# PaullyMac/routest

Hardware: AMD Instinct MI355X
Metric: ETA preds/sec (whole node) + p50 /predict latency, 3-layer MLP bf16 (higher is better)
Workload: dtype bf16

## Files before the change

csrc/cch.hip:

```cpp
#include <chrono>
#include <cstdio>
#include <cstdlib>
#include <cstring>
#include <string>

#include "cch_dev.h"
#include "cch_gpu.h"

namespace rt {

using namespace cchd;

CchMetricDev::~CchMetricDev() {
  int cur = 0;
  (void)hipGetDevice(&cur);
  (void)hipSetDevice(device);
  dfree(cost);
  dfree(sub_up);
  dfree(sub_dn);
  dfree(len_up);
  dfree(len_dn);
  dfree(cnt_up);
  dfree(cnt_dn);
  dfree(f_ptr);
  dfree(b_ptr);
  dfree(f_rec);
  dfree(b_rec);
  (void)hipSetDevice(cur);
}

CchGpu::CchGpu(rcch::Topology T, const float* length, const uint8_t* road_class, const uint8_t* base_traffic,
               int device)
    : T_(std::move(T)), dev_(device) {
  int cur = 0;
  (void)hipGetDevice(&cur);
  if (hipSetDevice(dev_) != hipSuccess) throw std::runtime_error("CchGpu: bad device");
  const int N = T_.N;
  const int64_t M = T_.M, E = T_.E;
  if (M >= (int64_t)1 << 31 || E >= (int64_t)1 << 31) throw std::runtime_error("CchGpu: graph too large");
  std::vector<int32_t> up_ptr32(N + 1);
  for (int r = 0; r <= N; ++r) up_ptr32[r] = (int32_t)T_.up_ptr[r];
  bofs_.assign(N + 1, 0);
  pofs_.assign(N + 1, 0);
  aofs_.assign(N + 1, 0);
  for (int i = 0; i < N; ++i) {
    const int64_t kb = T_.up_ptr[T_.hlev_nodes[i] + 1] - T_.up_ptr[T_.hlev_nodes[i]];
    bofs_[i + 1] = bofs_[i] + kb * (kb + 1) / 2;
    const int64_t kp = T_.up_ptr[T_.dlev_nodes[i] + 1] - T_.up_ptr[T_.dlev_nodes[i]];
    pofs_[i + 1] = pofs_[i] + kp * (kp - 1);
    aofs_[i + 1] = aofs_[i] + kp;
  }
  plev_kmax_.assign((size_t)T_.max_depth + 1, 0);
  for (int d = 0; d <= T_.max_depth; ++d)
    for (int64_t i = T_.dlev_ptr[d]; i < T_.dlev_ptr[d + 1]; ++i) {
      const int x = T_.dlev_nodes[i];
      plev_kmax_[d] = std::max(plev_kmax_[d], (int)(T_.up_ptr[x + 1] - T_.up_ptr[x]));
    }
  hipError_t e = hipSuccess;
  auto ck = [&](hipError_t x) {
    if (x != hipSuccess && e == hipSuccess) e = x;
  };
  ck(up_copy(d_up_ptr, up_ptr32.data(), N + 1));
  ck(up_copy(d_up_head, T_.up_head.data(), M));
  ck(up_copy(d_arc_lo, T_.arc_lo.data(), M));
  ck(up_copy(d_parent, T_.parent.data(), N));
  ck(up_copy(d_depth, T_.depth.data(), N));
  ck(up_copy(d_rank, T_.rank.data(), N));
  ck(up_copy(d_node, T_.node.data(), N));
  ck(up_copy(d_edge_arc, T_.edge_arc.data(), E));
  ck(up_copy(d_edge_dir, T_.edge_dir.data(), E));
  ck(up_copy(d_length, length, E));
  if (road_class) ck(up_copy(d_class, road_class, E));
  if (base_traffic) ck(up_copy(d_base_traffic, base_traffic, E));
  ck(up_copy(d_hnodes, T_.hlev_nodes.data(), N));
  ck(up_copy(d_dnodes, T_.dlev_nodes.data(), N));
  {
    std::vector<int32_t> dlev32(T_.dlev_ptr.begin(), T_.dlev_ptr.end());
    ck(up_copy(d_dlev_ptr, dlev32.data(), dlev32.size()));
  }
  ck(up_copy(d_bofs, bofs_.data(), N + 1));
  ck(up_copy(d_pofs, pofs_.data(), N + 1));

  ck(alloc_scratch(cs0_));
  if (builder_max_wg_.load() < 0) builder_max_wg_.store(M >= 20000000LL ? 512 : 0);
  if (e == hipSuccess) build_tables();
  (void)hipSetDevice(cur);
  if (e != hipSuccess) throw std::runtime_error(std::string("CchGpu: ") + hipGetErrorString(e));
  if (const char* gb = std::getenv("ROUTEST_CCH_CACHE_GB")) cache_gb_ = std::atof(gb);
}

CchGpu::~CchGpu() {
  {
    std::lock_guard<std::mutex> lk(bmu_);
    bstop_ = true;
    bq_.clear();
  }
  bcv_.notify_all();
  for (auto& t : bths_)
    if (t.joinable()) t.join();
  for (auto& x : bscr_) free_scratch(*x);
  {
    std::lock_guard<std::mutex> lk(mu_);
    cache_.clear();
  }
  int cur = 0;
  (void)hipGetDevice(&cur);
  (void)hipSetDevice(dev_);
  dfree(d_up_ptr);
  dfree(d_up_head);
  dfree(d_arc_lo);
  dfree(d_parent);
  dfree(d_depth);
  dfree(d_rank);
  dfree(d_node);
  dfree(d_edge_arc);
  dfree(d_edge_dir);
  dfree(d_length);
  dfree(d_class);
  dfree(d_base_traffic);
  dfree(d_hnodes);
  dfree(d_dnodes);
  dfree(d_dlev_ptr);
  dfree(d_bofs);
  dfree(d_pofs);
  free_tables();
  free_geometry();
  free_scratch(cs0_);
  (void)hipSetDevice(cur);
}

void CchGpu::set_eta(const void* blob, int H, const NormParams& np, int variant, int num_cus) {
  std::lock_guard<std::mutex> lk(mu_cust_);
  eta_blob_ = blob;
  eta_H_ = H;
  eta_np_ = np;
  eta_variant_ = variant;
  eta_cus_ = num_cus;
}

hipError_t CchGpu::metric_from_costs(uint64_t key, const float* d_cost, hipStream_t s,
                                     std::shared_ptr<CchMetricDev>& out) {
  auto m = std::make_shared<CchMetricDev>();
  m->key = key;
  hipError_t e = customize(d_cost, *m, s);
  if (e != hipSuccess) return e;
  {
    std::lock_guard<std::mutex> lk(mu_);
    for (auto it = cache_.begin(); it != cache_.end(); ++it)
      if ((*it)->key == key) {
        cache_.erase(it);
        break;
      }
  }
  insert_cached(m);
  out = m;
  return hipSuccess;
}

static int64_t metric_device_bytes(const CchMetricDev& m, int64_t N, int64_t M, int64_t E) {
  return E * 4 + M * (8 + 8 + 4 + 4 + 4 + 4) + (N + 1) * 8 + (m.kept_f + m.kept_b) * 16;
}

void CchGpu::insert_cached(const std::shared_ptr<CchMetricDev>& m) {
  const int64_t b = metric_device_bytes(*m, T_.N, T_.M, T_.E);
  metric_bytes_.store(b);
  std::lock_guard<std::mutex> lk(mu_);
  if (cache_gb_ > 0.0 && b > 0) capacity_ = (int)std::max<int64_t>(4, (int64_t)(cache_gb_ * 1073741824.0 / (double)b));
  cache_.push_front(m);
  if (m->avoid) {
    const int cap = std::max(1, capacity_ / 4);
    int n = 0;
    for (const auto& x : cache_) n += x->avoid != nullptr;
    for (auto it = cache_.end(); n > cap && it != cache_.begin();) {
      --it;
      if ((*it)->avoid) {
        it = cache_.erase(it);
        --n;
      }
    }
  }
  while ((int)cache_.size() > capacity_) cache_.pop_back();
}

static bool same_avoid(const std::shared_ptr<const std::vector<int32_t>>& a,
                       const std::shared_ptr<const std::vector<int32_t>>& b) {
  return a == b || (a && b && *a == *b);
}

bool CchGpu::avoid_clash(const CchContext& c) {
  const uint64_t key = c.key();
  std::lock_guard<std::mutex> lk(mu_);
  for (const auto& m : cache_)
    if (m->key == key) return !same_avoid(m->avoid, c.avoid);
  return false;
}

void CchGpu::set_cache_gb(double gb) {
  std::lock_guard<std::mutex> lk(mu_);
  cache_gb_ = gb > 0.0 ? gb : 0.0;
  const int64_t b = metric_bytes_.load();
  if (cache_gb_ > 0.0 && b > 0) capacity_ = (int)std::max<int64_t>(4, (int64_t)(cache_gb_ * 1073741824.0 / (double)b));
  while ((int)cache_.size() > capacity_) cache_.pop_back();
}

void CchGpu::request_build(const CchContext& c, bool urgent) {
  const uint64_t key = c.key();
  std::shared_ptr<CchMetricDev> m;
  if (cached_metric(key, m)) {
    notify_built(key, same_avoid(m->avoid, c.avoid));
    return;
  }
  {
    std::lock_guard<std::mutex> lk(bmu_);
    if (bstop_ || !bpending_.insert(key).second) return;
    if (urgent) bq_.push_front(c);
    else bq_.push_back(c);
    start_builders_locked();
  }
  n_bqueued_.fetch_add(1, std::memory_order_relaxed);
  bcv_.notify_one();
}

void CchGpu::start_builders_locked() {
  if (!bths_.empty() || bstop_) return;
  static const int nb = [] {
    const char* v = std::getenv("ROUTEST_CCH_BUILDERS");
    const int k = v ? std::atoi(v) : 3;
    return k < 1 ? 1 : (k > 8 ? 8 : k);
  }();
  for (int i = 0; i < nb; ++i) bths_.emplace_back([this, i] { builder_loop(i); });
}

void CchGpu::start_builders() {
  std::lock_guard<std::mutex> lk(bmu_);
  start_builders_locked();
}

int CchGpu::add_build_listener(std::function<void(uint64_t, bool)> cb) {
  std::lock_guard<std::mutex> lk(lmu_);
  listeners_.emplace_back(next_listener_, std::move(cb));
  return next_listener_++;
}

void CchGpu::remove_build_listener(int id) {
  std::lock_guard<std::mutex> lk(lmu_);
  for (auto it = listeners_.begin(); it != listeners_.end(); ++it)
    if (it->first == id) {
      listeners_.erase(it);
      break;
    }
}

void CchGpu::notify_built(uint64_t key, bool ok) {
  std::lock_guard<std::mutex> lk(lmu_);
  for (auto& l : listeners_) l.second(key, ok);
}

CchGpu::AsyncStats CchGpu::async_stats() {
  AsyncStats a;
  a.queued = n_bqueued_.load();
  a.built = n_bbuilt_.load();
  a.failed = n_bfailed_.load();
  a.build_ms = us_build_.load() / 1e3;
  a.alloc_ms = us_alloc_.load() / 1e3;
  a.hostcopy_ms = us_hostcopy_.load() / 1e3;
  a.paced = n_paced_.load();
  std::lock_guard<std::mutex> lk(bmu_);
  a.pending = (int)bpending_.size();
  return a;
}

void CchGpu::builder_loop(int idx) {
  (void)idx;
  if (hipSetDevice(dev_) != hipSuccess) return;
  CustScratch* xs = nullptr;
  {
    auto x = std::make_unique<CustScratch>();
    if (alloc_scratch(*x) == hipSuccess) {
      xs = x.get();
      std::lock_guard<std::mutex> lk(bmu_);
      bscr_.push_back(std::move(x));
    } else {
      free_scratch(*x);
      (void)hipGetLastError();
    }
  }
  hipStream_t s = nullptr;
  static const int share = [] {
    const char* v = std::getenv("ROUTEST_CCH_BUILDER_CU_SHARE");
    const int k = v ? std::atoi(v) : 4;
    return k < 1 ? 1 : k;
  }();
  if (share > 1) {
    int cus = 0;
    if (hipDeviceGetAttribute(&cus, hipDeviceAttributeMultiprocessorCount, dev_) != hipSuccess || cus <= 0) cus = 256;
    std::vector<uint32_t> mask((size_t)(cus + 31) / 32, 0u);
    for (int c = share - 1; c < cus; c += share) mask[(size_t)c / 32] |= 1u << (c % 32);
    if (hipExtStreamCreateWithCUMask(&s, (uint32_t)mask.size(), mask.data()) != hipSuccess) {
      (void)hipGetLastError();
      s = nullptr;
    }
  }
  if (s == nullptr) {
    int least = 0, greatest = 0;
    if (hipDeviceGetStreamPriorityRange(&least, &greatest) != hipSuccess ||
        hipStreamCreateWithPriority(&s, hipStreamNonBlocking, least) != hipSuccess) {
      (void)hipGetLastError();
      if (hipStreamCreateWithFlags(&s, hipStreamNonBlocking) != hipSuccess) s = nullptr;
    }
  }
  while (true) {
    CchContext c;
    {
      std::unique_lock<std::mutex> lk(bmu_);
      bcv_.wait(lk, [&] { return bstop_ || !bq_.empty(); });
      if (bstop_) break;
      c = bq_.front();
      bq_.pop_front();
    }
    std::shared_ptr<CchMetricDev> m;
    bool fresh = false;
    const auto tb = std::chrono::steady_clock::now();
    const bool ok = s != nullptr && metric_for(c, s, m, &fresh, xs) == hipSuccess;
    if (ok && fresh && m) {
      us_build_.fetch_add((long long)(std::chrono::duration<double, std::micro>(std::chrono::steady_clock::now() - tb).count()));
      us_alloc_.fetch_add((long long)(m->alloc_ms * 1e3));
      us_hostcopy_.fetch_add((long long)(m->hostcopy_ms * 1e3));
    }
    if (!ok) (void)hipGetLastError();
    (ok ? n_bbuilt_ : n_bfailed_).fetch_add(1, std::memory_order_relaxed);
    {
      std::lock_guard<std::mutex> lk(bmu_);
      bpending_.erase(c.key());
    }
    notify_built(c.key(), ok);
  }
  if (s) (void)hipStreamDestroy(s);
}

bool CchGpu::cached_metric(uint64_t key, std::shared_ptr<CchMetricDev>& out) {
  std::lock_guard<std::mutex> lk(mu_);
  for (auto it = cache_.begin(); it != cache_.end(); ++it)
    if ((*it)->key == key) {
      out = *it;
      cache_.splice(cache_.begin(), cache_, it);
      return true;
    }
  return false;
}

hipError_t CchGpu::metric_for(const CchContext& c, hipStream_t s, std::shared_ptr<CchMetricDev>& out, bool* fresh,
                              CustScratch* cs) {
  const uint64_t key = c.key();
  if (fresh) *fresh = false;
  auto lookup = [&]() -> bool { return cached_metric(key, out); };
  auto checked = [&]() -> hipError_t {
    if (same_avoid(out->avoid, c.avoid)) return hipSuccess;
    out.reset();
    return hipErrorInvalidValue;
  };
  if (lookup()) return checked();
  {
    std::unique_lock<std::mutex> lk(mu_inflight_);
    cv_inflight_.wait(lk, [&] { return inflight_.count(key) == 0; });
    if (lookup()) return checked();
    inflight_.insert(key);
  }
  struct Done {
    CchGpu* g;
    uint64_t k;
    ~Done() {
      {
        std::lock_guard<std::mutex> lk(g->mu_inflight_);
        g->inflight_.erase(k);
      }
      g->cv_inflight_.notify_all();
    }
  } done{this, key};
  auto m = std::make_shared<CchMetricDev>();
  m->key = key;
  m->device = dev_;
  m->avoid = c.avoid;
  const auto ta = std::chrono::steady_clock::now();
  hipError_t e = dmalloc(m->cost, T_.E);
  m->alloc_ms = std::chrono::duration<double, std::milli>(std::chrono::steady_clock::now() - ta).count();
  if (e != hipSuccess) return e;
  auto t0 = std::chrono::steady_clock::now();
  e = context_costs(c, m->cost, s, cs);
  if (e == hipSuccess) e = hipStreamSynchronize(s);
  if (e != hipSuccess) return e;
  m->cost_ms = std::chrono::duration<double, std::milli>(std::chrono::steady_clock::now() - t0).count();
  e = customize(m->cost, *m, s, cs);
  if (e != hipSuccess) return e;
  insert_cached(m);
  out = m;
  if (fresh) *fresh = true;
  return hipSuccess;
}

}
```

csrc/cch_all.hip:

```cpp
#include <algorithm>
#include <cstdlib>

#include "cch_dev.h"
#include "cch_gpu.h"

namespace rt {

using namespace cchd;

namespace {

constexpr int ALL_FUSED_THREADS = 1024;
constexpr int ALL_FUSE_MAX = ALL_FUSED_THREADS / 64;
constexpr int ALL_ROWS = 16;
constexpr int ALL_PRE = 64 / ALL_ROWS;

__device__ __forceinline__ bool label_less(float s1, float m1, float s0, float m0) {
  return s1 < s0 || (s1 == s0 && m1 < m0);
}

__global__ __launch_bounds__(256) void cch_all_fill_kernel(float4* __restrict__ sec, float4* __restrict__ met,
                                                           long long n4) {
  const long long g = blockIdx.x * (long long)blockDim.x + threadIdx.x;
  if (g >= n4) return;
  const float4 v = make_float4(F_INF, F_INF, F_INF, F_INF);
  sec[g] = v;
  met[g] = v;
}

__global__ __launch_bounds__(64) void cch_all_up_kernel(const int* __restrict__ src, int cnt,
                                                        const int32_t* __restrict__ rank,
                                                        const int32_t* __restrict__ parent,
                                                        const int32_t* __restrict__ depth,
                                                        const int32_t* __restrict__ ptr, const int4* __restrict__ rec,
                                                        const float* __restrict__ len, int N, int stride,
                                                        float* __restrict__ wsec, float* __restrict__ wmet) {
  extern __shared__ unsigned char smem[];
  float* sd = reinterpret_cast<float*>(smem);
  float* sm = sd + stride;
  int32_t* sn = reinterpret_cast<int32_t*>(sm + stride);
  const int j = blockIdx.x;
  if (j >= cnt) return;
  const int lane = threadIdx.x;
  const int node = src[j];
  if (node < 0 || node >= N) return;
  const int r = rank[node];
  const int D = depth[r];
  if (D >= stride) return;
  for (int d = lane; d <= D; d += 64) {
    sd[d] = F_INF;
    sm[d] = F_INF;
    sn[d] = -1;
  }
  __syncthreads();
  if (lane == 0) {
    sd[D] = 0.f;
    sm[D] = 0.f;
  }
  __syncthreads();
  int x = r;
  for (int d = D; d >= 0 && x >= 0; --d) {
    const int par = parent[x];
    const int kb = ptr[x], ke = ptr[x + 1];
    if (lane == 0) sn[d] = x;
    const float dx = sd[d], mx = sm[d];
    if (dx < F_INF) {
      for (int k = kb + lane; k < ke; k += 64) {
        const int4 rc = rec[k];
        const int hd = rc.y;
        const float cs = dx + __int_as_float(rc.x);
        const float cm = mx + len[rc.z];
        if (hd >= 0 && hd < d && label_less(cs, cm, sd[hd], sm[hd])) {
          sd[hd] = cs;
          sm[hd] = cm;
        }
      }
    }
    __syncthreads();
    x = par;
  }
  const size_t base = (size_t)(j >> 6) * (size_t)N * 64 + (size_t)(j & 63);
  for (int d = lane; d <= D; d += 64) {
    const int y = sn[d];
    if (y < 0) continue;
    wsec[base + (size_t)y * 64] = sd[d];
    wmet[base + (size_t)y * 64] = sm[d];
  }
}

__device__ __forceinline__ void pull_rows(int n, int l0, int w_l, int u_l, int m_l, size_t base, const float* wsec,
                                          const float* wmet, float& bs, float& bm) {
  float ls[ALL_ROWS], lm[ALL_ROWS];
#pragma unroll
  for (int q = 0; q < ALL_ROWS; ++q) {
    const int u = __builtin_amdgcn_readlane(u_l, l0 + (q < n ? q : n - 1));
    ls[q] = wsec[base + (size_t)u * 64];
    lm[q] = wmet[base + (size_t)u * 64];
  }
#pragma unroll
  for (int q = 0; q < ALL_ROWS; ++q) {
    const int ii = l0 + (q < n ? q : n - 1);
    const float cs = ls[q] + __int_as_float(__builtin_amdgcn_readlane(w_l, ii));
    const float cm = lm[q] + __int_as_float(__builtin_amdgcn_readlane(m_l, ii));
    if (ls[q] < F_INF && label_less(cs, cm, bs, bm)) {
      bs = cs;
      bm = cm;
    }
  }
}

__device__ __forceinline__ int chunk_record(int kb, int part, int parts, int t0, int lane) {
  return kb + ALL_ROWS * (part + parts * (t0 + lane / ALL_ROWS)) + lane % ALL_ROWS;
}

__device__ __forceinline__ void pull_chunks(int kb, int ke, int part, int parts, int t0, int w_l, int u_l, int m_l,
                                            size_t base, const float* wsec, const float* wmet, float& bs, float& bm) {
#pragma unroll
  for (int t = 0; t < ALL_PRE; ++t) {
    const int left = ke - (kb + ALL_ROWS * (part + parts * (t0 + t)));
    if (left > 0) pull_rows(left < ALL_ROWS ? left : ALL_ROWS, ALL_ROWS * t, w_l, u_l, m_l, base, wsec, wmet, bs, bm);
  }
}

__device__ __forceinline__ void pull_part(int kb, int ke, int part, int parts, int t0, size_t base, int lane,
                                          const int4* __restrict__ rec, const int32_t* __restrict__ up_head,
                                          const float* __restrict__ len, const float* wsec, const float* wmet,
                                          float& bs, float& bm) {
  for (; kb + ALL_ROWS * (part + parts * t0) < ke; t0 += ALL_PRE) {
    const int k = chunk_record(kb, part, parts, t0, lane);
    int w_l = 0, u_l = 0, m_l = 0;
    if (k < ke) {
      const int4 rc = rec[k];
      w_l = rc.x;
      u_l = up_head[rc.z];
      m_l = __float_as_int(len[rc.z]);
    }
    pull_chunks(kb, ke, part, parts, t0, w_l, u_l, m_l, base, wsec, wmet, bs, bm);
  }
}

template <int WAVES>
__global__ __launch_bounds__(64 * WAVES) void cch_all_pull_kernel(
    const int32_t* __restrict__ dnodes, int lb, int cnt, int nblk, int N, const int32_t* __restrict__ ptr,
    const int4* __restrict__ rec, const int32_t* __restrict__ up_head, const float* __restrict__ len, float* wsec,
    float* wmet) {
  __shared__ float red_s[WAVES][64], red_m[WAVES][64];
  const int wave = __builtin_amdgcn_readfirstlane(threadIdx.x >> 6), lane = threadIdx.x & 63;
  const int ni = blockIdx.x / nblk, b = blockIdx.x % nblk;
  if (ni >= cnt) return;
  const int v = dnodes[lb + ni];
  const int kb = ptr[v], ke = ptr[v + 1];
  if (ke <= kb) return;
  const size_t base = (size_t)b * (size_t)N * 64 + (size_t)lane;
  const size_t row = base + (size_t)v * 64;
  float bs = F_INF, bm = F_INF;
  if (wave == 0) {
    bs = wsec[row];
    bm = wmet[row];
  }
  pull_part(kb, ke, wave, WAVES, 0, base, lane, rec, up_head, len, wsec, wmet, bs, bm);
  if (WAVES > 1) {
    red_s[wave][lane] = bs;
    red_m[wave][lane] = bm;
    __syncthreads();
    if (wave != 0) return;
#pragma unroll
    for (int p = 1; p < WAVES; ++p)
      if (label_less(red_s[p][lane], red_m[p][lane], bs, bm)) {
        bs = red_s[p][lane];
        bm = red_m[p][lane];
      }
  }
  wsec[row] = bs;
  wmet[row] = bm;
}

__global__ __launch_bounds__(ALL_FUSED_THREADS) void cch_all_pull_fused_kernel(
    const int32_t* __restrict__ dlev_ptr, const int32_t* __restrict__ dnodes, int d0, int d1, int N,
    const int32_t* __restrict__ ptr, const int4* __restrict__ rec, const int32_t* __restrict__ up_head,
    const float* __restrict__ len, float* wsec, float* wmet) {
  constexpr int NW = ALL_FUSED_THREADS / 64;
  __shared__ float red_s[NW][64], red_m[NW][64];
  const int wave = __builtin_amdgcn_readfirstlane(threadIdx.x >> 6), lane = threadIdx.x & 63;
  const size_t base = (size_t)blockIdx.x * (size_t)N * 64 + (size_t)lane;
  int lb1 = 0, width1 = 0;
  int act2 = 0, part2 = 0, parts2 = 1, v2 = 0;
  int act3 = 0, part3 = 0, parts3 = 1, v3 = 0, kb3 = 0, ke3 = 0;
  int act4 = 0, part4 = 0, parts4 = 1, v4 = 0, kb4 = 0, ke4 = 0, n4 = 0;
  int4 rc4 = make_int4(0, 0, 0, 0);
  int act5 = 0, part5 = 0, parts5 = 1, v5 = 0, kb5 = 0, ke5 = 0;
  int w5 = 0, u5 = 0, m5 = 0;
  for (int d = d0 - 5; d < d1; ++d) {
    const int act = act5, part = part5, parts = parts5, v = v5, kb = kb5, ke = ke5;
    const int w_l = w5, u_l = u5, m_l = m5;
    act5 = act4, part5 = part4, parts5 = parts4, v5 = v4, kb5 = kb4, ke5 = ke4;
    w5 = rc4.x;
    u5 = m5 = 0;
    if (n4) {
      u5 = up_head[rc4.z];
      m5 = __float_as_int(len[rc4.z]);
    }
    act4 = act3, part4 = part3, parts4 = parts3, v4 = v3, kb4 = kb3, ke4 = ke3;
    {
      const int k = chunk_record(kb3, part3, parts3, 0, lane);
      n4 = act3 && k < ke3;
      rc4 = make_int4(0, 0, 0, 0);
      if (n4) rc4 = rec[k];
    }
    act3 = act2, part3 = part2, parts3 = parts2, v3 = v2;
    kb3 = ke3 = 0;
    if (act2) {
      kb3 = ptr[v2];
      ke3 = ptr[v2 + 1];
    }
    act2 = 0, part2 = 0, parts2 = 1, v2 = 0;
    if (width1 > 0 && width1 <= NW) {
      parts2 = NW / width1;
      part2 = wave % parts2;
      const int ni = wave / parts2;
      if (ni < width1) {
        act2 = 1;
        v2 = dnodes[lb1 + ni];
      }
    }
    lb1 = width1 = 0;
    if (d + 5 >= d0 && d + 5 < d1) {
      lb1 = dlev_ptr[d + 5];
      width1 = dlev_ptr[d + 6] - lb1;
    }
    if (d < d0) continue;
    size_t row = 0;
    float bs = F_INF, bm = F_INF;
    if (act) {
      row = base + (size_t)v * 64;
      if (part == 0) {
        bs = wsec[row];
        bm = wmet[row];
      }
      pull_chunks(kb, ke, part, parts, 0, w_l, u_l, m_l, base, wsec, wmet, bs, bm);
      pull_part(kb, ke, part, parts, ALL_PRE, base, lane, rec, up_head, len, wsec, wmet, bs, bm);
      red_s[wave][lane] = bs;
      red_m[wave][lane] = bm;
    }
    __syncthreads();
    if (act && part == 0) {
      for (int p = 1; p < parts; ++p)
        if (label_less(red_s[wave + p][lane], red_m[wave + p][lane], bs, bm)) {
          bs = red_s[wave + p][lane];
          bm = red_m[wave + p][lane];
        }
      wsec[row] = bs;
      wmet[row] = bm;
    }
    __syncthreads();
  }
}

__global__ __launch_bounds__(256) void cch_all_out_kernel(const int32_t* __restrict__ rank, int N, int cnt,
                                                          const float* __restrict__ wsec,
                                                          const float* __restrict__ wmet, float* __restrict__ osec,
                                                          float* __restrict__ omet) {
  __shared__ float tile[64][65];
  const float* __restrict__ w = blockIdx.z == 0 ? wsec : wmet;
  float* __restrict__ o = blockIdx.z == 0 ? osec : omet;
  const int b = blockIdx.y;
  const int n0 = blockIdx.x * 64;
  const int lane = threadIdx.x & 63, wave = threadIdx.x >> 6;
  const size_t base = (size_t)b * (size_t)N * 64;
  for (int i = wave; i < 64; i += 4) {
    const int n = n0 + i;
    if (n < N) tile[i][lane] = w[base + (size_t)rank[n] * 64 + lane];
  }
  __syncthreads();
  const int nl = cnt - b * 64 < 64 ? cnt - b * 64 : 64;
  if (n0 + lane < N)
    for (int l = wave; l < nl; l += 4) o[(size_t)(b * 64 + l) * (size_t)N + n0 + lane] = tile[lane][l];
}

}

CchAllScratch::~CchAllScratch() {
  int cur = 0;
  (void)hipGetDevice(&cur);
  (void)hipSetDevice(device);
  dfree(sec);
  dfree(met);
  for (void* p : old) (void)hipFree(p);
  (void)hipSetDevice(cur);
}

hipError_t CchAllScratch::ensure(size_t blocks, size_t N) {
  if (blocks <= blocks_cap) return hipSuccess;
  if (sec) old.push_back((void*)sec);
  if (met) old.push_back((void*)met);
  sec = met = nullptr;
  blocks_cap = 0;
  hipError_t e;
  if ((e = dmalloc(sec, blocks * N * 64)) != hipSuccess) return e;
  if ((e = dmalloc(met, blocks * N * 64)) != hipSuccess) return e;
  blocks_cap = blocks;
  return hipSuccess;
}

hipError_t CchGpu::one_to_all(const CchMetricDev& m, const int* d_src, int S, bool reverse, float* d_sec, float* d_met,
                              CchAllScratch& sc, hipStream_t s, int fuse) {
  if (S <= 0) return hipSuccess;
  if (d_src == nullptr || d_sec == nullptr || d_met == nullptr) return hipErrorInvalidValue;
  static const int fuse_default = [] {
    const char* v = std::getenv("ROUTEST_CCH_ALL_FUSE");
    return v ? std::max(0, std::atoi(v)) : ALL_FUSE_WIDTH;
  }();
  if (fuse < 0) fuse = fuse_default;
  fuse = std::min(fuse, ALL_FUSE_MAX);
  const int N = T_.N, ST = stride();
  const size_t up_lds = (size_t)ST * 12;
  if (up_lds > 64 * 1024) return hipErrorInvalidValue;
  const int32_t* u_ptr = reverse ? m.b_ptr : m.f_ptr;
  const int4* u_rec = reverse ? m.b_rec : m.f_rec;
  const float* u_len = reverse ? m.len_dn : m.len_up;
  const int32_t* p_ptr = reverse ? m.f_ptr : m.b_ptr;
  const int4* p_rec = reverse ? m.f_rec : m.b_rec;
  const float* p_len = reverse ? m.len_up : m.len_dn;
  const size_t block_bytes = (size_t)N * 64 * 4 * 2;
  const int total_blocks = (S + 63) / 64;
  const int chunk_blocks = (int)std::min<size_t>((size_t)total_blocks, std::max<size_t>(1, ALL_SCRATCH_BYTES / block_bytes));
  sc.device = dev_;
  hipError_t e = sc.ensure((size_t)chunk_blocks, (size_t)N);
  if (e != hipSuccess) return e;
  for (int c0 = 0; c0 < total_blocks; c0 += chunk_blocks) {
    const int nb = std::min(chunk_blocks, total_blocks - c0);
    const int s0 = c0 * 64;
    const int cnt = std::min(S - s0, nb * 64);
    const long long n4 = (long long)nb * N * 16;
    hipLaunchKernelGGL(cch_all_fill_kernel, dim3(blocks_for(n4, 256)), dim3(256), 0, s,
                       reinterpret_cast<float4*>(sc.sec), reinterpret_cast<float4*>(sc.met), n4);
    hipLaunchKernelGGL(cch_all_up_kernel, dim3(cnt), dim3(64), up_lds, s, d_src + s0, cnt, d_rank, d_parent, d_depth,
                       u_ptr, u_rec, u_len, N, ST, sc.sec, sc.met);
    if ((e = hipGetLastError()) != hipSuccess) return e;
    for (int d = 1; d <= T_.max_depth;) {
      int d1 = d;
      while (fuse > 0 && d1 <= T_.max_depth && T_.dlev_ptr[d1 + 1] - T_.dlev_ptr[d1] <= fuse) ++d1;
      if (d1 - d >= 2) {
        hipLaunchKernelGGL(cch_all_pull_fused_kernel, dim3(nb), dim3(ALL_FUSED_THREADS), 0, s, d_dlev_ptr, d_dnodes, d,
                           d1, N, p_ptr, p_rec, d_up_head, p_len, sc.sec, sc.met);
        d = d1;
      } else {
        const int lb = (int)T_.dlev_ptr[d], lc = (int)(T_.dlev_ptr[d + 1] - T_.dlev_ptr[d]);
        const int kmax = plev_kmax_[d];
        const dim3 grid((unsigned)((long long)lc * nb));
        auto launch = [&](auto kernel, int waves) {
          hipLaunchKernelGGL(kernel, grid, dim3(64 * waves), 0, s, d_dnodes, lb, lc, nb, N, p_ptr, p_rec, d_up_head, p_len,
                             sc.sec, sc.met);
        };
        if (kmax <= ALL_ROWS) launch(cch_all_pull_kernel<1>, 1);
        else if (kmax <= 2 * ALL_ROWS) launch(cch_all_pull_kernel<2>, 2);
        else if (kmax <= 4 * ALL_ROWS) launch(cch_all_pull_kernel<4>, 4);
        else launch(cch_all_pull_kernel<8>, 8);
        ++d;
      }
    }
    if ((e = hipGetLastError()) != hipSuccess) return e;
    hipLaunchKernelGGL(cch_all_out_kernel, dim3(blocks_for(N, 64), nb, 2), dim3(256), 0, s, d_rank, N, cnt, sc.sec,
                       sc.met, d_sec + (size_t)s0 * N, d_met + (size_t)s0 * N);
    if ((e = hipGetLastError()) != hipSuccess) return e;
  }
  return hipSuccess;
}

}
```

csrc/cch_bindings.cpp:

```cpp
#include <torch/extension.h>
#include <ATen/hip/impl/HIPStreamMasqueradingAsCUDA.h>
#include <c10/core/DeviceGuard.h>

#include <chrono>
#include <cmath>
#include <memory>
#include <mutex>
#include <unordered_map>

#include "cch_gpu.h"
#include "ops.h"

namespace py = pybind11;

namespace {

#define CCH_CHECK_HIP(expr)                                                            \
  do {                                                                                 \
    hipError_t _e = (expr);                                                            \
    TORCH_CHECK(_e == hipSuccess, "HIP error in ", #expr, ": ", hipGetErrorString(_e)); \
  } while (0)

hipStream_t stream_of(int dev) { return c10::hip::getCurrentHIPStreamMasqueradingAsCUDA(dev).stream(); }

template <class T>
const T* host_ptr(const torch::Tensor& t, int64_t n, const char* name) {
  TORCH_CHECK(!t.is_cuda() && t.is_contiguous() && t.numel() == n, name, ": contiguous CPU tensor of ", n);
  return t.data_ptr<T>();
}

class PyCchGpu {
 public:
  PyCchGpu(torch::Tensor indptr, torch::Tensor indices, torch::Tensor lat, torch::Tensor lon, torch::Tensor length,
           torch::Tensor road_class, torch::Tensor base_traffic, int64_t device) {
    TORCH_CHECK(indptr.scalar_type() == torch::kInt32 && indices.scalar_type() == torch::kInt32 &&
                    lat.scalar_type() == torch::kFloat64 && lon.scalar_type() == torch::kFloat64 &&
                    length.scalar_type() == torch::kFloat32 && road_class.scalar_type() == torch::kUInt8 &&
                    base_traffic.scalar_type() == torch::kUInt8,
                "CchGpu: indptr/indices int32, lat/lon float64, length float32, road_class/base_traffic uint8");
    const int64_t N = lat.numel();
    const int32_t* ip = host_ptr<int32_t>(indptr, N + 1, "indptr");
    const int64_t E = ip[N];
    const int32_t* ix = host_ptr<int32_t>(indices, E, "indices");
    for (int64_t e = 0; e < E; ++e) TORCH_CHECK(ix[e] >= 0 && ix[e] < N, "edge target out of range");
    for (int64_t v = 0; v < N; ++v) TORCH_CHECK(ip[v] <= ip[v + 1], "indptr not monotone");
    auto t0 = std::chrono::steady_clock::now();
    rcch::Topology T;
    {
      py::gil_scoped_release nogil;
      T = rcch::build_topology((int)N, ip, ix, host_ptr<double>(lat, N, "lat"), host_ptr<double>(lon, N, "lon"));
    }
    build_ms_ = std::chrono::duration<double, std::milli>(std::chrono::steady_clock::now() - t0).count();
    dev_ = (int)device;
    g_ = std::make_unique<rt::CchGpu>(std::move(T), host_ptr<float>(length, E, "length"),
                                      host_ptr<uint8_t>(road_class, E, "road_class"),
                                      host_ptr<uint8_t>(base_traffic, E, "base_traffic"), dev_);
    sc_ = std::make_unique<rt::CchScratch>();
    asc_ = std::make_unique<rt::CchAllScratch>();
    std::vector<int32_t> qx((size_t)N), qy((size_t)N);
    const double* la = lat.data_ptr<double>();
    const double* lo = lon.data_ptr<double>();
    for (int64_t v = 0; v < N; ++v) {
      TORCH_CHECK(std::fabs(la[v]) <= 90.0 && std::fabs(lo[v]) <= 180.0, "node coordinate out of range");
      qx[v] = (int32_t)std::nearbyint(lo[v] * 1e6);
      qy[v] = (int32_t)std::nearbyint(la[v] * 1e6);
    }
    g_->set_geometry(ip, ix, qx.data(), qy.data());
  }

  rt::CchContext context(int64_t weather, int64_t congestion, int64_t weekhour, double age,
                         const c10::optional<torch::Tensor>& avoid, int64_t digest) const {
    rt::CchContext c;
    c.weather = (int)weather;
    c.congestion = (int)congestion;
    c.weekhour = (int)weekhour;
    c.driver_age = (float)age;
    if (avoid.has_value()) {
      c.avoid = blob_of(*avoid);
      TORCH_CHECK(digest > 0 && digest < ((int64_t)1 << 31), "avoid_digest: 1 .. 2^31 - 1");
      c.avoid_digest = (uint32_t)digest;
    }
    return c;
  }
  static std::shared_ptr<const std::vector<int32_t>> blob_of(const torch::Tensor& t) {
    TORCH_CHECK(!t.is_cuda() && t.scalar_type() == torch::kInt32 && t.dim() == 1 && t.is_contiguous(),
                "avoid: int32 [n] CPU tensor");
    return std::make_shared<const std::vector<int32_t>>(t.data_ptr<int32_t>(), t.data_ptr<int32_t>() + t.numel());
  }

  torch::Tensor avoid_mask(torch::Tensor blob) {
    auto b = blob_of(blob);
    auto out = torch::empty({(int64_t)g_->topo().E}, torch::TensorOptions().dtype(torch::kUInt8).device(torch::kCUDA, dev_));
    const c10::DeviceGuard guard(out.device());
    hipError_t e;
    {
      py::gil_scoped_release nogil;
      e = g_->avoid_mask(*b, out.data_ptr<uint8_t>(), stream_of(dev_));
    }
    if (e == hipErrorInvalidValue) throw py::value_error("avoid: not a valid avoid-set blob");
    CCH_CHECK_HIP(e);
    return out;
  }

  void set_eta(torch::Tensor blob, int64_t H, std::vector<double> norm, int64_t variant) {
    TORCH_CHECK(blob.is_cuda() && blob.device().index() == dev_ && blob.scalar_type() == torch::kUInt8,
                "blob: uint8 on the router's GPU");
    TORCH_CHECK((size_t)blob.numel() == rt::eta_mlp3_blob_bytes((int)H), "blob size for H=", H);
    TORCH_CHECK(norm.size() == 8, "norm: 4 scales + 4 shifts");
    rt::NormParams np;
    for (int i = 0; i < 4; ++i) {
      np.scale[i] = (float)norm[i];
      np.shift[i] = (float)norm[4 + i];
    }
    int cus = 256;
    (void)hipDeviceGetAttribute(&cus, hipDeviceAttributeMultiprocessorCount, dev_);
    blob_ = blob;
    g_->set_eta(blob_.data_ptr(), (int)H, np, (int)variant, cus);
  }

  py::dict stats() const {
    const rcch::Topology& T = g_->topo();
    py::dict d;
    d["nodes"] = T.N;
    d["arcs"] = T.M;
    d["edges"] = T.E;
    d["max_depth"] = T.max_depth;
    d["max_height"] = T.max_height;
    d["top_separator"] = T.separator_top;
    d["build_ms"] = build_ms_;
    d["cached_metrics"] = g_->cached();
    d["triangle_table"] = g_->has_triangle_table();
    d["triangles"] = g_->triangles();
    d["basic_tasks"] = g_->basic_tasks();
    d["supernodal"] = g_->supernodal();
    d["sup_fronts"] = g_->sup_fronts();
    d["sup_nodes"] = g_->sup_nodes();
    d["sup_levels"] = g_->sup_levels();
    d["sup_blocks"] = g_->sup_blocks();
    d["sparse_heights"] = g_->sparse_heights();
    d["sparse_depths"] = g_->sparse_depths();
    d["cache_capacity"] = g_->capacity();
    d["cache_gb"] = g_->cache_gb();
    d["metric_bytes"] = g_->metric_bytes();
    const auto a = g_->async_stats();
    d["async_queued"] = a.queued;
    d["async_built"] = a.built;
    d["async_failed"] = a.failed;
    d["async_pending"] = a.pending;
    d["async_build_ms"] = a.build_ms;
    d["async_alloc_ms"] = a.alloc_ms;
    d["async_hostcopy_ms"] = a.hostcopy_ms;
    d["builder_max_wg"] = g_->builder_pacing();
    d["async_paced"] = a.paced;
    return d;
  }

  void request_build(int64_t weather, int64_t congestion, int64_t weekhour, double age, bool urgent,
                     c10::optional<torch::Tensor> avoid, int64_t avoid_digest) {
    TORCH_CHECK(g_->has_eta(), "CchGpu: set_eta first");
    const rt::CchContext c = context(weather, congestion, weekhour, age, avoid, avoid_digest);
    g_->request_build(c, urgent);
  }
  bool is_cached(int64_t key) {
    std::shared_ptr<rt::CchMetricDev> m;
    return g_->cached_metric((uint64_t)key, m);
  }
  void set_cache_gb(double gb) { g_->set_cache_gb(gb); }
  void set_builder_pacing(int n, bool always) { g_->set_builder_pacing(n, always); }
  void set_unpack_serial(bool on) { g_->set_unpack_serial(on); }
  bool unpack_serial() const { return g_->unpack_serial(); }

  py::dict info(const rt::CchMetricDev& m, bool fresh) const {
    py::dict d;
    d["key"] = m.key;
    d["fresh"] = fresh;
    d["cost_ms"] = m.cost_ms;
    d["customize_ms"] = m.customize_ms;
    d["basic_ms"] = m.basic_ms;
    d["perfect_ms"] = m.perfect_ms;
    d["prune_ms"] = m.prune_ms;
    d["kept_f"] = m.kept_f;
    d["kept_b"] = m.kept_b;
    return d;
  }

  py::dict metric_for(int64_t weather, int64_t congestion, int64_t weekhour, double age, bool pin,
                      c10::optional<torch::Tensor> avoid, int64_t avoid_digest) {
    TORCH_CHECK(g_->has_eta(), "CchGpu: set_eta first");
    const rt::CchContext c = context(weather, congestion, weekhour, age, avoid, avoid_digest);
    const c10::DeviceGuard guard(c10::Device(c10::DeviceType::CUDA, dev_));
    std::shared_ptr<rt::CchMetricDev> m;
    bool fresh = false;
    hipError_t e;
    {
      py::gil_scoped_release nogil;
      e = g_->metric_for(c, stream_of(dev_), m, &fresh);
    }
    if (e == hipErrorInvalidValue && g_->avoid_clash(c))
      throw py::value_error("avoid set: its digest is cached for a different set (a 2^-31 collision); "
                            "change a vertex by a microdegree or retry once that metric is evicted");
    if (e == hipErrorInvalidValue && c.avoid) throw py::value_error("avoid: not a valid avoid-set blob");
    CCH_CHECK_HIP(e);
    if (pin) pin_ptr(m);
    return info(*m, fresh);
  }

  void unpin(int64_t key) {
    std::lock_guard<std::mutex> lk(pin_mu_);
    auto it = pins_.find((uint64_t)key);
    if (it != pins_.end() && --it->second.second <= 0) pins_.erase(it);
  }
  int64_t pinned() {
    std::lock_guard<std::mutex> lk(pin_mu_);
    return (int64_t)pins_.size();
  }

  py::dict metric_from_costs(int64_t key, torch::Tensor cost) {
    TORCH_CHECK(cost.is_cuda() && cost.device().index() == dev_ && cost.scalar_type() == torch::kFloat32 &&
                    cost.is_contiguous() && cost.numel() == g_->topo().E,
                "cost: float32 [E] on the router's GPU");
    TORCH_CHECK((cost >= 0).all().item<bool>(), "edge costs must be >= 0 (+inf: edge absent), not NaN");
    cost = cost.add(0.0);
    const c10::DeviceGuard guard(cost.device());
    std::shared_ptr<rt::CchMetricDev> m;
    hipError_t e;
    {
      py::gil_scoped_release nogil;
      e = g_->metric_from_costs((uint64_t)key, cost.data_ptr<float>(), stream_of(dev_), m);
    }
    CCH_CHECK_HIP(e);
    return info(*m, true);
  }

  py::dict metric_dump(int64_t key) {
    auto m = get(key);
    const int64_t M = g_->topo().M, N = g_->topo().N;
    const auto opt = torch::TensorOptions().device(torch::kCUDA, dev_);
    const c10::DeviceGuard guard(opt.device());
    py::dict d;
    auto put = [&](const char* name, const void* src, int64_t n, torch::ScalarType t) {
      auto out = torch::empty({n}, opt.dtype(t));
      if (n > 0)
        CCH_CHECK_HIP(hipMemcpyAsync(out.data_ptr(), src, n * out.element_size(), hipMemcpyDeviceToDevice, stream_of(dev_)));
      d[name] = out;
    };
    put("sub_up", m->sub_up, 2 * M, torch::kInt32);
    put("sub_dn", m->sub_dn, 2 * M, torch::kInt32);
    put("len_up", m->len_up, M, torch::kFloat32);
    put("len_dn", m->len_dn, M, torch::kFloat32);
    put("cnt_up", m->cnt_up, M, torch::kInt32);
    put("cnt_dn", m->cnt_dn, M, torch::kInt32);
    put("f_ptr", m->f_ptr, N + 1, torch::kInt32);
    put("b_ptr", m->b_ptr, N + 1, torch::kInt32);
    put("f_rec", m->f_rec, 4 * m->kept_f, torch::kInt32);
    put("b_rec", m->b_rec, 4 * m->kept_b, torch::kInt32);
    return d;
  }

  torch::Tensor costs(int64_t key) {
    auto m = get(key);
    auto out = torch::empty({(int64_t)g_->topo().E},
                            torch::TensorOptions().dtype(torch::kFloat32).device(torch::kCUDA, dev_));
    const c10::DeviceGuard guard(out.device());
    CCH_CHECK_HIP(hipMemcpyAsync(out.data_ptr<float>(), m->cost, g_->topo().E * 4, hipMemcpyDeviceToDevice,
                                 stream_of(dev_)));
    return out;
  }

  py::tuple route(int64_t key, torch::Tensor src, torch::Tensor dst, int64_t max_path, bool want_path) {
    auto m = get(key);
    TORCH_CHECK(src.is_cuda() && dst.is_cuda() && src.device().index() == dev_ && dst.device().index() == dev_ &&
                    src.scalar_type() == torch::kInt32 && dst.scalar_type() == torch::kInt32 &&
                    src.is_contiguous() && dst.is_contiguous() && src.numel() == dst.numel(),
                "src/dst: int32 [Q] on the router's GPU");
    const int64_t Q = src.numel();
    const int N = g_->topo().N;
    if (Q > 0) {
      const auto mn = torch::minimum(src.min(), dst.min()).item<int>();
      const auto mx = torch::maximum(src.max(), dst.max()).item<int>();
      TORCH_CHECK(mn >= 0 && mx < N, "node id out of range");
    }
    auto o32 = torch::TensorOptions().dtype(torch::kInt32).device(torch::kCUDA, dev_);
    auto of = torch::TensorOptions().dtype(torch::kFloat32).device(torch::kCUDA, dev_);
    auto sec = torch::empty({Q}, of), met = torch::empty({Q}, of);
    auto st = torch::empty({Q}, o32), len = torch::zeros({Q}, o32);
    auto path = want_path ? torch::empty({Q, max_path}, o32) : torch::empty({0, max_path}, o32);
    rt::CchRouteOut o;
    o.sec = sec.data_ptr<float>();
    o.metres = met.data_ptr<float>();
    o.status = st.data_ptr<int>();
    o.len = len.data_ptr<int>();
    o.path = want_path ? path.data_ptr<int>() : nullptr;
    o.max_path = (int)max_path;
    const c10::DeviceGuard guard(src.device());
    std::lock_guard<std::mutex> lk(mu_);
    CCH_CHECK_HIP(g_->route(*m, src.data_ptr<int>(), dst.data_ptr<int>(), (int)Q, o, *sc_, stream_of(dev_)));
    return py::make_tuple(sec, met, st, len, path);
  }

  py::tuple matrix(int64_t key, torch::Tensor pts, torch::Tensor npts) {
    auto m = get(key);
    TORCH_CHECK(pts.is_cuda() && npts.is_cuda() && pts.dim() == 2 && pts.scalar_type() == torch::kInt32 &&
                    npts.scalar_type() == torch::kInt32 && npts.numel() == pts.size(0) && pts.is_contiguous(),
                "pts int32 [R, NM], npts int32 [R] on the router's GPU");
    const int R = (int)pts.size(0), NM = (int)pts.size(1);
    auto of = torch::TensorOptions().dtype(torch::kFloat32).device(torch::kCUDA, dev_);
    auto sec = torch::empty({R, NM, NM}, of), met = torch::empty({R, NM, NM}, of);
    const c10::DeviceGuard guard(pts.device());
    std::lock_guard<std::mutex> lk(mu_);
    CCH_CHECK_HIP(g_->matrix(*m, pts.data_ptr<int>(), npts.data_ptr<int>(), R, NM, sec.data_ptr<float>(),
                             met.data_ptr<float>(), nullptr, *sc_, stream_of(dev_)));
    return py::make_tuple(sec, met);
  }

  py::tuple matrix_rect(int64_t key, torch::Tensor src, torch::Tensor nsrc, torch::Tensor dst, torch::Tensor ndst,
                        int64_t meet) {
    auto m = get(key);
    for (const torch::Tensor* t : {&src, &nsrc, &dst, &ndst})
      TORCH_CHECK(t->is_cuda() && t->device().index() == dev_ && t->scalar_type() == torch::kInt32 && t->is_contiguous(),
                  "src / nsrc / dst / ndst: int32 on the router's GPU");
    TORCH_CHECK(src.dim() == 2 && dst.dim() == 2 && dst.size(0) == src.size(0) && nsrc.numel() == src.size(0) &&
                    ndst.numel() == src.size(0),
                "src [R, SM], dst [R, DM], nsrc [R], ndst [R]");
    const int64_t R = src.size(0), SM = src.size(1), DM = dst.size(1);
    TORCH_CHECK(R * (SM + DM) <= INT32_MAX && R * SM * DM <= INT32_MAX, "matrix_rect: too many chains or cells for one call");
    auto of = torch::TensorOptions().dtype(torch::kFloat32).device(torch::kCUDA, dev_);
    auto sec = torch::empty({R, SM, DM}, of), met = torch::empty({R, SM, DM}, of);
    const c10::DeviceGuard guard(src.device());
    std::lock_guard<std::mutex> lk(mu_);
    CCH_CHECK_HIP(g_->matrix_rect(*m, src.data_ptr<int>(), nsrc.data_ptr<int>(), dst.data_ptr<int>(),
                                  ndst.data_ptr<int>(), (int)R, (int)SM, (int)DM, sec.data_ptr<float>(),
                                  met.data_ptr<float>(), *sc_, stream_of(dev_), (int)meet));
    return py::make_tuple(sec, met);
  }

  py::tuple matrix_keep(int64_t key, torch::Tensor pts, torch::Tensor npts) {
    auto sm = matrix(key, pts, npts);
    std::lock_guard<std::mutex> lk(mu_);
    return py::make_tuple(sm[0], sm[1], (uint64_t)sc_->chain_tag);
  }

  py::tuple legs_from_matrix(int64_t key, uint64_t tag, torch::Tensor pts, torch::Tensor r, torch::Tensor i,
                             torch::Tensor j, int64_t max_path, bool want_path) {
    auto m = get(key);
    for (const torch::Tensor* t : {&pts, &r, &i, &j})
      TORCH_CHECK(t->is_cuda() && t->device().index() == dev_ && t->scalar_type() == torch::kInt32 && t->is_contiguous(),
                  "pts / r / i / j: int32 on the router's GPU");
    TORCH_CHECK(pts.dim() == 2 && r.numel() == i.numel() && r.numel() == j.numel(), "pts [R, NM]; r, i, j [Q]");
    const int64_t Q = r.numel();
    const int R = (int)pts.size(0), NM = (int)pts.size(1);
    if (Q > 0) {
      TORCH_CHECK(r.min().item<int>() >= 0 && r.max().item<int>() < R, "leg request index out of range");
      TORCH_CHECK(torch::minimum(i.min(), j.min()).item<int>() >= 0 && torch::maximum(i.max(), j.max()).item<int>() < NM,
                  "leg point index out of range");
    }
    auto o32 = torch::TensorOptions().dtype(torch::kInt32).device(torch::kCUDA, dev_);
    auto of = torch::TensorOptions().dtype(torch::kFloat32).device(torch::kCUDA, dev_);
    auto sec = torch::empty({Q}, of), met = torch::empty({Q}, of);
    auto st = torch::empty({Q}, o32), len = torch::zeros({Q}, o32);
    auto path = want_path ? torch::empty({Q, max_path}, o32) : torch::empty({0, max_path}, o32);
    rt::CchRouteOut o;
    o.sec = sec.data_ptr<float>();
    o.metres = met.data_ptr<float>();
    o.status = st.data_ptr<int>();
    o.len = len.data_ptr<int>();
    o.path = want_path ? path.data_ptr<int>() : nullptr;
    o.max_path = (int)max_path;
    const c10::DeviceGuard guard(pts.device());
    auto src = Q > 0 ? pts.index({r.to(torch::kLong), i.to(torch::kLong)}).contiguous() : torch::empty({0}, o32);
    std::lock_guard<std::mutex> lk(mu_);
    TORCH_CHECK(tag != 0 && tag == sc_->chain_tag && sc_->chain_nm == NM && sc_->chain_r == R,
                "legs_from_matrix: the matrix chains of this tag are gone (another call ran since)");
    CCH_CHECK_HIP(g_->legs_from_matrix(*m, src.data_ptr<int>(), r.data_ptr<int>(), i.data_ptr<int>(), j.data_ptr<int>(),
                                       (int)Q, tag, o, *sc_, stream_of(dev_)));
    return py::make_tuple(sec, met, st, len, path);
  }

  py::tuple one_to_all(int64_t key, torch::Tensor src, bool reverse, int64_t fuse) {
    auto m = get(key);
    TORCH_CHECK(src.is_cuda() && src.device().index() == dev_ && src.scalar_type() == torch::kInt32 &&
                    src.is_contiguous() && src.dim() == 1,
                "src: int32 [S] on the router's GPU");
    const int64_t S = src.numel();
    const int64_t N = g_->topo().N;
    TORCH_CHECK(S < ((int64_t)1 << 31) - 64, "too many sources");
    if (S > 0) TORCH_CHECK(src.min().item<int>() >= 0 && src.max().item<int>() < N, "node id out of range");
    auto of = torch::TensorOptions().dtype(torch::kFloat32).device(torch::kCUDA, dev_);
    auto sec = torch::empty({S, N}, of), met = torch::empty({S, N}, of);
    const c10::DeviceGuard guard(src.device());
    std::lock_guard<std::mutex> lk(mu_);
    CCH_CHECK_HIP(g_->one_to_all(*m, src.data_ptr<int>(), (int)S, reverse, sec.data_ptr<float>(), met.data_ptr<float>(),
                                 *asc_, stream_of(dev_), (int)fuse));
    return py::make_tuple(sec, met);
  }

  void set_capacity(int64_t n) { g_->set_capacity((int)n); }
  uintptr_t ptr() const { return reinterpret_cast<uintptr_t>(g_.get()); }
  py::dict topology_arrays() const {
    const rcch::Topology& T = g_->topo();
    py::dict d;
    auto i32 = [](const std::vector<int32_t>& v) {
      auto t = torch::empty({(int64_t)v.size()}, torch::kInt32);
      if (!v.empty()) std::memcpy(t.data_ptr<int32_t>(), v.data(), v.size() * 4);
      return t;
    };
    d["rank"] = i32(T.rank);
    d["node"] = i32(T.node);
    d["parent"] = i32(T.parent);
    d["depth"] = i32(T.depth);
    d["up_head"] = i32(T.up_head);
    return d;
  }

 private:
  void pin_ptr(const std::shared_ptr<rt::CchMetricDev>& m) {
    std::lock_guard<std::mutex> lk(pin_mu_);
    auto& p = pins_[m->key];
    p.first = m;
    ++p.second;
  }

  std::shared_ptr<rt::CchMetricDev> get(int64_t key) {
    std::shared_ptr<rt::CchMetricDev> m;
    if (g_->cached_metric((uint64_t)key, m)) return m;
    {
      std::lock_guard<std::mutex> lk(pin_mu_);
      auto it = pins_.find((uint64_t)key);
      if (it != pins_.end()) return it->second.first;
    }
    TORCH_CHECK(false, "CchGpu: no cached metric for key ", key, " (evicted or never built)");
    return m;
  }

  std::mutex pin_mu_;
  std::unordered_map<uint64_t, std::pair<std::shared_ptr<rt::CchMetricDev>, int>> pins_;

  std::unique_ptr<rt::CchGpu> g_;
  std::unique_ptr<rt::CchScratch> sc_;
  std::unique_ptr<rt::CchAllScratch> asc_;
  std::mutex mu_;
  torch::Tensor blob_;
  int dev_ = 0;
  double build_ms_ = 0.0;
};

}

void bind_cch_gpu(py::module& m) {
  py::class_<PyCchGpu>(m, "CchGpu")
      .def(py::init<torch::Tensor, torch::Tensor, torch::Tensor, torch::Tensor, torch::Tensor, torch::Tensor,
                    torch::Tensor, int64_t>(),
           py::arg("indptr"), py::arg("indices"), py::arg("lat"), py::arg("lon"), py::arg("length"),
           py::arg("road_class"), py::arg("base_traffic"), py::arg("device"))
      .def("set_eta", &PyCchGpu::set_eta, py::arg("blob"), py::arg("H"), py::arg("norm"), py::arg("variant") = -1)
      .def("stats", &PyCchGpu::stats)
      .def("metric_for", &PyCchGpu::metric_for, py::arg("weather"), py::arg("congestion"), py::arg("weekhour"),
           py::arg("driver_age") = 35.0, py::arg("pin") = false, py::arg("avoid") = py::none(),
           py::arg("avoid_digest") = 0)
      .def("avoid_mask", &PyCchGpu::avoid_mask, py::arg("blob"))
      .def("unpin", &PyCchGpu::unpin, py::arg("key"))
      .def("pinned", &PyCchGpu::pinned)
      .def("metric_from_costs", &PyCchGpu::metric_from_costs, py::arg("key"), py::arg("cost"))
      .def("costs", &PyCchGpu::costs, py::arg("key"))
      .def("metric_dump", &PyCchGpu::metric_dump, py::arg("key"))
      .def("route", &PyCchGpu::route, py::arg("key"), py::arg("src"), py::arg("dst"), py::arg("max_path") = 4096,
           py::arg("want_path") = true)
      .def("matrix", &PyCchGpu::matrix, py::arg("key"), py::arg("pts"), py::arg("npts"))
      .def("matrix_rect", &PyCchGpu::matrix_rect, py::arg("key"), py::arg("src"), py::arg("nsrc"), py::arg("dst"),
           py::arg("ndst"), py::arg("meet") = 0)
      .def("matrix_keep", &PyCchGpu::matrix_keep, py::arg("key"), py::arg("pts"), py::arg("npts"))
      .def("legs_from_matrix", &PyCchGpu::legs_from_matrix, py::arg("key"), py::arg("tag"), py::arg("pts"), py::arg("r"),
           py::arg("i"), py::arg("j"), py::arg("max_path") = 4096, py::arg("want_path") = true)
      .def("one_to_all", &PyCchGpu::one_to_all, py::arg("key"), py::arg("src"), py::arg("reverse") = false,
           py::arg("fuse") = -1)
      .def("set_capacity", &PyCchGpu::set_capacity)
      .def("set_cache_gb", &PyCchGpu::set_cache_gb, py::arg("gb"))
      .def("set_builder_pacing", &PyCchGpu::set_builder_pacing, py::arg("max_workgroups"), py::arg("always") = false)
      .def("set_unpack_serial", &PyCchGpu::set_unpack_serial, py::arg("on"))
      .def("unpack_serial", &PyCchGpu::unpack_serial)
      .def("request_build", &PyCchGpu::request_build, py::arg("weather"), py::arg("congestion"), py::arg("weekhour"),
           py::arg("driver_age") = 35.0, py::arg("urgent") = true, py::arg("avoid") = py::none(),
           py::arg("avoid_digest") = 0)
      .def("is_cached", &PyCchGpu::is_cached, py::arg("key"))
      .def("ptr", &PyCchGpu::ptr)
      .def("topology_arrays", &PyCchGpu::topology_arrays);
}
```

csrc/cch_customize.hip:

```cpp
#include <hipcub/hipcub.hpp>

#include <chrono>
#include <cstdio>
#include <cstdlib>
#include <cstring>
#include <string>

#include "cch_dev.h"
#include "cch_gpu.h"
#include "ops.h"
#include "runtime/rt_core.h"

namespace rt {

using namespace cchd;

namespace {

using EtaRecordDev = rtc::EtaRecord;

__device__ __forceinline__ int item_owner(const int64_t* __restrict__ ofs, int lo, int hi, long long g) {
  while (hi - lo > 1) {
    const int mid = (lo + hi) >> 1;
    if (ofs[mid] <= g) lo = mid;
// ... 73 lines not shown
      sub[1] = e;
      len[a] = length[e];
      cnt[a] = 1;
      continue;
    }
    const int zz = (int)pl;
    const int azu = find_arc_d(up_ptr, up_head, zz, z), azv = find_arc_d(up_ptr, up_head, zz, v);
    const int s0 = dir ? azv : azu, s1 = dir ? azu : azv;
    sub[0] = s0;
    sub[1] = s1;
    len[a] = len_dn[s0] + len_up[s1];
    cnt[a] = cnt_dn[s0] + cnt_up[s1];
  }
}

__device__ __forceinline__ void basic_relax_pair(int z, int ai, int aj, int t, unsigned long long* __restrict__ up,
                                                 unsigned long long* __restrict__ dn) {
  const float wu = wof(dn[ai]) + wof(up[aj]);
  const float wd = wof(dn[aj]) + wof(up[ai]);
  if (wu < F_INF) {
    const unsigned long long pu = packw(wu, (uint32_t)z);
    if (pu < up[t]) atomicMin(up + t, pu);
  }
  if (wd < F_INF) {
    const unsigned long long pd = packw(wd, (uint32_t)z);
    if (pd < dn[t]) atomicMin(dn + t, pd);
  }
}

__global__ __launch_bounds__(256) void basic_level_kernel(LevelArgs L, unsigned long long* __restrict__ up,
                                                          unsigned long long* __restrict__ dn,
                                                          int32_t* __restrict__ sub_up, int32_t* __restrict__ sub_dn,
                                                          float* __restrict__ len_up, float* __restrict__ len_dn,
                                                          int32_t* __restrict__ cnt_up, int32_t* __restrict__ cnt_dn,
                                                          const float* __restrict__ length) {
  const long long gi = blockIdx.x * (long long)blockDim.x + threadIdx.x;
  if (gi >= L.items) return;
  const long long g = L.base + gi;
  const int ni = item_owner(L.ofs, L.lo, L.hi, g);
  const int z = L.nodes[ni];
  const long long p = g - L.ofs[ni];
  const int a0 = L.up_ptr[z];
  const int k = L.up_ptr[z + 1] - a0;
  if (p < k) {
    const int a = a0 + (int)p;
    basic_finalize_arc(a, z, L.up_head[a], L.up_ptr, L.up_head, up, dn, sub_up, sub_dn, len_up, len_dn, cnt_up, cnt_dn,
                       length);
    return;
  }
  const long long q = p - k;
  const double kk = (double)(2 * k - 1);
  int i = (int)((kk - sqrt(kk * kk - 8.0 * (double)q)) * 0.5);
  if (i < 0) i = 0;
  auto row0 = [&](int r) { return (long long)r * (2 * k - r - 1) / 2; };
  while (i > 0 && row0(i) > q) --i;
  while (i + 1 < k && row0(i + 1) <= q) ++i;
  const int j = (int)(q - row0(i)) + i + 1;
  const int ai = a0 + i, aj = a0 + j;
  const int t = find_arc_d(L.up_ptr, L.up_head, L.up_head[ai], L.up_head[aj]);
  if (t < 0) return;
  basic_relax_pair(z, ai, aj, t, up, dn);
}

struct BasicTask {
  int64_t rowbase;
  int32_t node;
  int32_t a0;
  uint16_t k;
  uint16_t row;
  uint16_t col0;
  uint16_t pad;
};
static_assert(sizeof(BasicTask) == 24, "basic task layout");
constexpr uint16_t ROW_FINAL = 0xFFFF;

__global__ __launch_bounds__(256) void basic_task_kernel(const BasicTask* __restrict__ tasks, long long ntask,
                                                         const int32_t* __restrict__ up_ptr,
                                                         const int32_t* __restrict__ up_head,
                                                         const int32_t* __restrict__ tri,
                                                         unsigned long long* __restrict__ up,
                                                         unsigned long long* __restrict__ dn, int32_t* __restrict__ sub_up,
                                                         int32_t* __restrict__ sub_dn, float* __restrict__ len_up,
                                                         float* __restrict__ len_dn, int32_t* __restrict__ cnt_up,
                                                         int32_t* __restrict__ cnt_dn, const float* __restrict__ length) {
  const long long ti = (long long)blockIdx.x * 4 + (threadIdx.x >> 6);
  if (ti >= ntask) return;
  const BasicTask& T = tasks[ti];
  const int lane = threadIdx.x & 63;
  const int z = T.node;
  const int a0 = T.a0;
  const int k = T.k;
  if (T.row == ROW_FINAL) {
    const int p = T.col0 + lane;
    if (p >= k) return;
    const int a = a0 + p;
    basic_finalize_arc(a, z, up_head[a], up_ptr, up_head, up, dn, sub_up, sub_dn, len_up, len_dn, cnt_up, cnt_dn,
                       length);
    return;
  }
  const int i = T.row;
  const int j = T.col0 + lane;
  if (j >= k) return;
  const int t = tri[T.rowbase + j];
  if (t < 0) return;
  basic_relax_pair(z, a0 + i, a0 + j, t, up, dn);
}

__global__ void perfect_init_kernel(const unsigned long long* __restrict__ up, const unsigned long long* __restrict__ dn,
                                    uint32_t* __restrict__ pup, uint32_t* __restrict__ pdn, long long M) {
  for (long long a = blockIdx.x * (long long)blockDim.x + threadIdx.x; a < M; a += (long long)gridDim.x * blockDim.x) {
    pup[a] = (uint32_t)(up[a] >> 32);
    pdn[a] = (uint32_t)(dn[a] >> 32);
  }
}

__global__ __launch_bounds__(256) void perfect_level_kernel(LevelArgs L, const unsigned long long* __restrict__ up,
                                                            const unsigned long long* __restrict__ dn,
                                                            uint32_t* __restrict__ pup, uint32_t* __restrict__ pdn) {
  const long long gi = blockIdx.x * (long long)blockDim.x + threadIdx.x;
  if (gi >= L.items) return;
  const long long g = L.base + gi;
  const int ni = item_owner(L.ofs, L.lo, L.hi, g);
  const int x = L.nodes[ni];
  const long long p = g - L.ofs[ni];
  const int a0 = L.up_ptr[x];
  const int k = L.up_ptr[x + 1] - a0;
  const int c = (int)(p / (k - 1));
  const int r = (int)(p % (k - 1));
  const int a = r < c ? r : r + 1;
  const int ac = a0 + c, aa = a0 + a;
  const int y = L.up_head[aa], z = L.up_head[ac];
  const int azy = find_arc_d(L.up_ptr, L.up_head, z < y ? z : y, z < y ? y : z);
  if (azy < 0) return;
  const float xz = wof(up[ac]), zx = wof(dn[ac]);
  const float zy = __uint_as_float(z < y ? pup[azy] : pdn[azy]);
  const float yz = __uint_as_float(z < y ? pdn[azy] : pup[azy]);
  const float cu = xz + zy, cd = yz + zx;
  if (cu < F_INF && __float_as_uint(cu) < pup[aa]) atomicMin(pup + aa, __float_as_uint(cu));
  if (cd < F_INF && __float_as_uint(cd) < pdn[aa]) atomicMin(pdn + aa, __float_as_uint(cd));
}

struct PArc {
  int64_t tb;
  int32_t a0;
  int32_t y;
  uint16_t k;
  uint16_t ia;
  int32_t pad;
};
static_assert(sizeof(PArc) == 24, "pull arc record");

struct PullArgs {
  const int32_t* up_head;
  const int32_t* tri;
  const PArc* parc;
  long long base, arcs;
};

__device__ __forceinline__ void pull_cand(const PullArgs& P, long long tb, int k, int a0, int ia, int ic, float xz_c,
                                          float zx_c, const uint32_t* __restrict__ pup, const uint32_t* __restrict__ pdn,
                                          int y, int z, float& bu, float& bd) {
  const int i = ic < ia ? ic : ia, j = ic < ia ? ia : ic;
  const int azy = P.tri[tb + (long long)i * (2 * k - i - 1) / 2 + (j - i - 1)];
  const float zy = __uint_as_float(z < y ? pup[azy] : pdn[azy]);
  const float yz = __uint_as_float(z < y ? pdn[azy] : pup[azy]);
  const float cu = xz_c + zy, cd = yz + zx_c;
  bu = cu < bu ? cu : bu;
  bd = cd < bd ? cd : bd;
}

__device__ __forceinline__ void pull_arc_min(const PullArgs& P, long long tb, int a0, int k, int ia, int y, int c_begin,
                                             int c_step, int lane, const unsigned long long* __restrict__ up,
                                             const unsigned long long* __restrict__ dn, const uint32_t* __restrict__ pup,
                                             const uint32_t* __restrict__ pdn, float& bu, float& bd) {
  for (int c0 = c_begin; c0 < k; c0 += c_step) {
    int azy[4], z[4];
    unsigned long long wu[4], wd[4];
    bool ok[4];
#pragma unroll
    for (int u = 0; u < 4; ++u) {
      const int ic = c0 + 64 * u + lane;
      ok[u] = ic < k && ic != ia;
      const int i = ic < ia ? ic : ia, j = ic < ia ? ia : ic;
      azy[u] = ok[u] ? P.tri[tb + (long long)i * (2 * k - i - 1) / 2 + (j - i - 1)] : 0;
      z[u] = ok[u] ? P.up_head[a0 + ic] : 0;
      wu[u] = ok[u] ? up[a0 + ic] : 0ull;
      wd[u] = ok[u] ? dn[a0 + ic] : 0ull;
    }
    uint32_t gu[4], gd[4];
#pragma unroll
    for (int u = 0; u < 4; ++u) {
      gu[u] = ok[u] ? pup[azy[u]] : 0u;
      gd[u] = ok[u] ? pdn[azy[u]] : 0u;
    }
#pragma unroll
    for (int u = 0; u < 4; ++u) {
      if (!ok[u]) continue;
      const float zy = __uint_as_float(z[u] < y ? gu[u] : gd[u]);
      const float yz = __uint_as_float(z[u] < y ? gd[u] : gu[u]);
      const float cu = wof(wu[u]) + zy, cd = yz + wof(wd[u]);
      bu = cu < bu ? cu : bu;
      bd = cd < bd ? cd : bd;
    }
  }
#pragma unroll
  for (int o = 32; o >= 1; o >>= 1) {
    const float ou = __shfl_xor(bu, o), od = __shfl_xor(bd, o);
    bu = ou < bu ? ou : bu;
    bd = od < bd ? od : bd;
  }
}

template <int S>
__global__ __launch_bounds__(256) void perfect_pull_wave_kernel(PullArgs P, const unsigned long long* __restrict__ up,
                                                                const unsigned long long* __restrict__ dn,
                                                                uint32_t* __restrict__ pup, uint32_t* __restrict__ pdn) {
  static_assert(S == 1 || S == 2 || S == 4, "waves per arc");
  constexpr int APB = 4 / S;
  __shared__ float red[2][4];
  const int w = threadIdx.x >> 6, lane = threadIdx.x & 63;
  const long long g = (long long)blockIdx.x * APB + w / S;
  const int part = w % S;
  const bool active = g < P.arcs;
  float bu = F_INF, bd = F_INF;
  int aa = 0;
  if (active) {
    const PArc pa = P.parc[P.base + g];
    aa = pa.a0 + pa.ia;
    pull_arc_min(P, pa.tb, pa.a0, pa.k, pa.ia, pa.y, 256 * part, 256 * S, lane, up, dn, pup, pdn, bu, bd);
  }
  if constexpr (S > 1) {
    if (lane == 0) {
      red[0][w] = bu;
      red[1][w] = bd;
    }
    __syncthreads();
    if (part != 0) return;
#pragma unroll
    for (int q = 1; q < S; ++q) {
      const float ou = red[0][w + q], od = red[1][w + q];
      bu = ou < bu ? ou : bu;
      bd = od < bd ? od : bd;
    }
  }
  if (active && lane == 0) {
    const float cu = __uint_as_float(pup[aa]), cd = __uint_as_float(pdn[aa]);
    if (bu < cu) pup[aa] = __float_as_uint(bu);
    if (bd < cd) pdn[aa] = __float_as_uint(bd);
  }
}

__global__ __launch_bounds__(256) void perfect_pull_lane_kernel(PullArgs P, const unsigned long long* __restrict__ up,
                                                                const unsigned long long* __restrict__ dn,
                                                                uint32_t* __restrict__ pup, uint32_t* __restrict__ pdn) {
  const long long g = (long long)blockIdx.x * blockDim.x + threadIdx.x;
  if (g >= P.arcs) return;
  const PArc pa = P.parc[P.base + g];
  const long long tb = pa.tb;
  const int a0 = pa.a0, k = pa.k, ia = pa.ia, y = pa.y;
  const int aa = a0 + ia;
  float bu = __uint_as_float(pup[aa]), bd = __uint_as_float(pdn[aa]);
  for (int ic = 0; ic < k; ++ic) {
    if (ic == ia) continue;
    const int ac = a0 + ic;
    pull_cand(P, tb, k, a0, ia, ic, wof(up[ac]), wof(dn[ac]), pup, pdn, y, P.up_head[ac], bu, bd);
  }
  pup[aa] = __float_as_uint(bu);
  pdn[aa] = __float_as_uint(bd);
}

__device__ __forceinline__ bool kept(uint32_t p, unsigned long long b) {
  return __uint_as_float(p) < F_INF && p == (uint32_t)(b >> 32);
}

__global__ __launch_bounds__(256) void prune_count_wave_kernel(const int32_t* __restrict__ up_ptr,
                                                               const uint32_t* __restrict__ pup,
                                                               const uint32_t* __restrict__ pdn,
                                                               const unsigned long long* __restrict__ up,
                                                               const unsigned long long* __restrict__ dn, int N,
                                                               int32_t* __restrict__ fcnt, int32_t* __restrict__ bcnt) {
  const int x = blockIdx.x * 4 + (threadIdx.x >> 6);
  const int lane = threadIdx.x & 63;
  if (x >= N) return;
  int kf = 0, kb = 0;
  for (int a = up_ptr[x] + lane; a < up_ptr[x + 1]; a += 64) {
    kf += kept(pup[a], up[a]);
    kb += kept(pdn[a], dn[a]);
  }
#pragma unroll
  for (int o = 32; o >= 1; o >>= 1) {
    kf += __shfl_xor(kf, o);
    kb += __shfl_xor(kb, o);
  }
  if (lane == 0) {
    fcnt[x] = kf;
    bcnt[x] = kb;
  }
}

__global__ __launch_bounds__(256) void prune_scatter_wave_kernel(
    const int32_t* __restrict__ up_ptr, const int32_t* __restrict__ up_head, const int32_t* __restrict__ depth,
    const uint32_t* __restrict__ pup, const uint32_t* __restrict__ pdn, const unsigned long long* __restrict__ up,
    const unsigned long long* __restrict__ dn, int N, const int32_t* __restrict__ f_ptr, const int32_t* __restrict__ b_ptr,
    int4* __restrict__ f_rec, int4* __restrict__ b_rec) {
  const int x = blockIdx.x * 4 + (threadIdx.x >> 6);
  const int lane = threadIdx.x & 63;
  if (x >= N) return;
  int kf = f_ptr[x], kb = b_ptr[x];
  const unsigned long long below = (1ull << lane) - 1ull;
  for (int a0 = up_ptr[x]; a0 < up_ptr[x + 1]; a0 += 64) {
    const int a = a0 + lane;
    const bool in = a < up_ptr[x + 1];
    const bool f = in && kept(pup[a], up[a]);
    const bool b = in && kept(pdn[a], dn[a]);
    const unsigned long long mf = __ballot(f), mb = __ballot(b);
    if (f || b) {
      const int hd = depth[up_head[a]];
      if (f) f_rec[kf + __popcll(mf & below)] = make_int4((int)pup[a], hd, a, 0);
      if (b) b_rec[kb + __popcll(mb & below)] = make_int4((int)pdn[a], hd, a, 0);
    }
    kf += __popcll(mf);
    kb += __popcll(mb);
  }
}

struct SupNode {
  int64_t dofs;
  int64_t foff;
  int32_t c0, m, n;
  int32_t fnode;
};
struct SupWork {
  int32_t s, b, t0, t1;
  SupNode sn;
};
constexpr int SUP_B = 32;
constexpr int SUP_PJ = 32;
constexpr int SUP_TT = 64;
constexpr int SUP_G1Y = 32;
constexpr int SUP_G1Z = 128;
constexpr int SUP_SJ = 64;

__device__ __forceinline__ unsigned long long sup_cand(unsigned long long a, unsigned long long b, uint32_t z) {
  const float w = wof(a) + wof(b);
  return w < F_INF ? packw(w, z) : PACK_INF_D;
}
__device__ __forceinline__ unsigned long long umin64(unsigned long long a, unsigned long long b) { return b < a ? b : a; }

__global__ __launch_bounds__(256) void sup_farc_kernel(const SupNode* __restrict__ sn, const SupWork* __restrict__ w,
                                                       long long nw, const int32_t* __restrict__ fnode,
                                                       const int32_t* __restrict__ up_ptr,
                                                       const int32_t* __restrict__ up_head, int32_t* __restrict__ farc) {
  const long long wi = (long long)blockIdx.x * 4 + (threadIdx.x >> 6);
  if (wi >= nw) return;
  const SupWork W = w[wi];
  const SupNode S = W.sn;
  const int i = W.b, n = S.n;
  const int fi = fnode[S.fnode + i];
  for (int j = threadIdx.x & 63; j < n; j += 64) {
    const int fj = fnode[S.fnode + j];
    farc[S.foff + (long long)i * n + j] = i == j ? -1 : find_arc_d(up_ptr, up_head, fi < fj ? fi : fj, fi < fj ? fj : fi);
  }
}

__global__ __launch_bounds__(256) void sup_gather_basic_kernel(
    const SupNode* __restrict__ sn, const SupWork* __restrict__ w, const int32_t* __restrict__ fnode,
    const int32_t* __restrict__ farc, const unsigned long long* __restrict__ up, const unsigned long long* __restrict__ dn,
    const int32_t* __restrict__ up_ptr, const int32_t* __restrict__ up_head, const float* __restrict__ len_up,
    const float* __restrict__ len_dn, const int32_t* __restrict__ cnt_up, const int32_t* __restrict__ cnt_dn,
    unsigned long long* __restrict__ D, int2* __restrict__ SS, int2* __restrict__ SL) {
  const SupWork W = w[blockIdx.x];
  const SupNode S = W.sn;
  const int i = W.b, n = S.n;
  const long long r0 = S.dofs + (long long)i * n;
  const int32_t* fr = farc + S.foff + (long long)i * n;
  const int fi = fnode[S.fnode + i];
  for (int j = threadIdx.x; j < n; j += 256) {
    unsigned long long v = PACK_INF_D;
    if (i != j && (i < S.m || j < S.m)) {
      const int a = fr[j];
      if (a >= 0) {
        v = i < j ? up[a] : dn[a];
        const uint32_t pl = (uint32_t)v;
        if (wof(v) < F_INF && !(pl & EDGE_FLAG_D)) {
          const int zz = (int)pl, fj = fnode[S.fnode + j];
          const int lo = i < j ? fi : fj, hi = i < j ? fj : fi;
          const int azx = find_arc_d(up_ptr, up_head, zz, lo), azv = find_arc_d(up_ptr, up_head, zz, hi);
          const int s0 = i < j ? azx : azv, s1 = i < j ? azv : azx;
          SS[r0 + j] = make_int2(s0, s1);
          SL[r0 + j] = make_int2(__float_as_int(len_dn[s0] + len_up[s1]), cnt_dn[s0] + cnt_up[s1]);
        }
      }
    }
    D[r0 + j] = v;
  }
}

__device__ __forceinline__ void sup_panel_body(
    const SupWork& W, const int32_t* __restrict__ farc, unsigned long long* __restrict__ D, const int2* __restrict__ SS,
    const int2* __restrict__ SL, unsigned long long* __restrict__ up, unsigned long long* __restrict__ dn,
    int32_t* __restrict__ sub_up, int32_t* __restrict__ sub_dn, float* __restrict__ len_up, float* __restrict__ len_dn,
    int32_t* __restrict__ cnt_up, int32_t* __restrict__ cnt_dn, const float* __restrict__ length) {
  constexpr int B = SUP_B, J = SUP_PJ, W2 = SUP_B + SUP_PJ;
  static_assert(B == 32 && J == 32, "one entry of each matrix per thread");
  __shared__ unsigned long long Dk[B][B + 1];
  __shared__ unsigned long long R[B][J + 1];
  __shared__ unsigned long long C[J][B + 1];
  __shared__ int32_t FK[B][W2];
  __shared__ float lu[B][W2], ld[B][W2];
  __shared__ int32_t cu[B][W2], cd[B][W2];
  const SupNode S = W.sn;
  const int n = S.n, tid = threadIdx.x;
  const int k0 = W.b * B, k1 = min(k0 + B, S.m), kb = k1 - k0;
  const int j0 = k1 + W.t0 * J, nj = max(0, min(J, n - j0));
  const bool diag_writer = W.t0 == 0;
  unsigned long long* Df = D + S.dofs;
  const int32_t* F = farc + S.foff;
  const int ty = tid >> 5, tx = tid & 31;
  Dk[ty][tx] = (ty < kb && tx < kb) ? Df[(long long)(k0 + ty) * n + k0 + tx] : PACK_INF_D;
  R[ty][tx] = (ty < kb && tx < nj) ? Df[(long long)(k0 + ty) * n + j0 + tx] : PACK_INF_D;
  C[ty][tx] = (tx < kb && ty < nj) ? Df[(long long)(j0 + ty) * n + k0 + tx] : PACK_INF_D;
  FK[ty][tx] = (ty < kb && tx < kb && tx > ty) ? F[(long long)(k0 + ty) * n + k0 + tx] : -1;
  FK[ty][B + tx] = (ty < kb && tx < nj) ? F[(long long)(k0 + ty) * n + j0 + tx] : -1;
  __syncthreads();
  if (W.b > 0) {
    const int km = k0 - B;
    __shared__ unsigned long long Ay[B][B + 1];
    __shared__ unsigned long long Aj[J][B + 1];
    __shared__ unsigned long long Bx[B][B + 1];
    __shared__ unsigned long long Bj[B][J + 1];
    Ay[ty][tx] = ty < kb ? Df[(long long)(k0 + ty) * n + km + tx] : PACK_INF_D;
    Aj[ty][tx] = ty < nj ? Df[(long long)(j0 + ty) * n + km + tx] : PACK_INF_D;
    Bx[ty][tx] = tx < kb ? Df[(long long)(km + ty) * n + k0 + tx] : PACK_INF_D;
    Bj[ty][tx] = tx < nj ? Df[(long long)(km + ty) * n + j0 + tx] : PACK_INF_D;
    __syncthreads();
    unsigned long long dk = Dk[ty][tx], rr = R[ty][tx], cc = C[ty][tx];
    const bool odk = ty < kb && tx < kb && ty != tx, orr = ty < kb && tx < nj, occ = ty < nj && tx < kb;
    for (int p = 0; p < B; ++p) {
      const uint32_t z = (uint32_t)(S.c0 + km + p);
      if (odk) dk = umin64(dk, sup_cand(Ay[ty][p], Bx[p][tx], z));
      if (orr) rr = umin64(rr, sup_cand(Ay[ty][p], Bj[p][tx], z));
      if (occ) cc = umin64(cc, sup_cand(Aj[ty][p], Bx[p][tx], z));
    }
    Dk[ty][tx] = dk;
    R[ty][tx] = rr;
    C[ty][tx] = cc;
    __syncthreads();
  }
  for (int p = 0; p < kb; ++p) {
    const uint32_t z = (uint32_t)(S.c0 + k0 + p);
    if (ty > p && tx > p && ty < kb && tx < kb && ty != tx) Dk[ty][tx] = umin64(Dk[ty][tx], sup_cand(Dk[ty][p], Dk[p][tx], z));
    if (ty > p && ty < kb && tx < nj) R[ty][tx] = umin64(R[ty][tx], sup_cand(Dk[ty][p], R[p][tx], z));
    if (tx > p && tx < kb && ty < nj) C[ty][tx] = umin64(C[ty][tx], sup_cand(C[ty][p], Dk[p][tx], z));
    __syncthreads();
  }
  if (ty < kb && tx < nj) {
    Df[(long long)(k0 + ty) * n + j0 + tx] = R[ty][tx];
    Df[(long long)(j0 + tx) * n + k0 + ty] = C[tx][ty];
    const int a = FK[ty][B + tx];
    if (a >= 0) {
      up[a] = R[ty][tx];
      dn[a] = C[tx][ty];
    }
  }
  if (diag_writer && ty < kb && tx < kb) {
    Df[(long long)(k0 + ty) * n + k0 + tx] = Dk[ty][tx];
    const int a = FK[ty][tx];
    if (a >= 0) {
      up[a] = Dk[ty][tx];
      dn[a] = Dk[tx][ty];
    }
  }
  const int zK = S.c0 + k0;
  auto vfront = [&](int col) { return col < B ? k0 + col : j0 + col - B; };
  auto weight = [&](int x, int col, int dir) -> unsigned long long {
    if (col < B) return dir ? Dk[col][x] : Dk[x][col];
    return dir ? C[col - B][x] : R[x][col - B];
  };
  auto put = [&](int x, int col, int a, int dir, int s0, int s1, float L, int32_t Cn) {
    (dir ? ld : lu)[x][col] = L;
    (dir ? cd : cu)[x][col] = Cn;
    if (col >= B || diag_writer) {
      int32_t* sub = (dir ? sub_dn : sub_up) + 2 * (long long)a;
      sub[0] = s0;
      sub[1] = s1;
      (dir ? len_dn : len_up)[a] = L;
      (dir ? cnt_dn : cnt_up)[a] = Cn;
    }
  };
  {
    constexpr int Q = B * W2 / 1024;
    int kind[Q][2], s0[Q][2], s1[Q][2];
    float L[Q][2];
    int32_t Cn[Q][2];
#pragma unroll
    for (int q = 0; q < Q; ++q) {
      const int e = tid + 1024 * q, x = e / W2, col = e % W2;
      const int a = FK[x][col];
#pragma unroll
      for (int dir = 0; dir < 2; ++dir) {
        kind[q][dir] = 0;
        if (a < 0) continue;
        const unsigned long long wt = weight(x, col, dir);
        const uint32_t pl = (uint32_t)wt;
        const int vf = vfront(col);
        if (!(wof(wt) < F_INF)) {
          kind[q][dir] = 1;
          s0[q][dir] = -1;
          s1[q][dir] = -1;
          L[q][dir] = F_INF;
          Cn[q][dir] = 0;
        } else if (pl & EDGE_FLAG_D) {
          const int ed = (int)(pl & ~EDGE_FLAG_D);
          kind[q][dir] = 1;
          s0[q][dir] = -1;
          s1[q][dir] = ed;
          L[q][dir] = length[ed];
          Cn[q][dir] = 1;
        } else if ((int)pl < S.c0) {
          const long long idx = dir ? (long long)vf * n + k0 + x : (long long)(k0 + x) * n + vf;
          const int2 ss = SS[S.dofs + idx], sl = SL[S.dofs + idx];
          kind[q][dir] = 1;
          s0[q][dir] = ss.x;
          s1[q][dir] = ss.y;
          L[q][dir] = __int_as_float(sl.x);
          Cn[q][dir] = sl.y;
        } else if ((int)pl < zK) {
          const long long fz = (int)pl - S.c0;
          const int azx = F[fz * n + k0 + x], azv = F[fz * n + vf];
          kind[q][dir] = 2;
          s0[q][dir] = dir ? azv : azx;
          s1[q][dir] = dir ? azx : azv;
        }
      }
    }
#pragma unroll
    for (int q = 0; q < Q; ++q)
#pragma unroll
      for (int dir = 0; dir < 2; ++dir)
        if (kind[q][dir] == 2) {
          L[q][dir] = len_dn[s0[q][dir]] + len_up[s1[q][dir]];
          Cn[q][dir] = cnt_dn[s0[q][dir]] + cnt_up[s1[q][dir]];
        }
#pragma unroll
    for (int q = 0; q < Q; ++q) {
      const int e = tid + 1024 * q, x = e / W2, col = e % W2;
#pragma unroll
      for (int dir = 0; dir < 2; ++dir)
        if (kind[q][dir]) put(x, col, FK[x][col], dir, s0[q][dir], s1[q][dir], L[q][dir], Cn[q][dir]);
    }
  }
  __syncthreads();
  for (int x = 1; x < kb; ++x) {
    if (tid < 2 * W2) {
      const int dir = tid / W2, col = tid % W2;
      const int a = FK[x][col];
      const unsigned long long wt = a >= 0 ? weight(x, col, dir) : PACK_INF_D;
      const uint32_t pl = (uint32_t)wt;
      const int zl = (int)pl - zK;
      if (wof(wt) < F_INF && !(pl & EDGE_FLAG_D) && zl >= 0) {
        const int azx = FK[zl][x], azv = FK[zl][col];
        if (dir == 0)
          put(x, col, a, 0, azx, azv, ld[zl][x] + lu[zl][col], cd[zl][x] + cu[zl][col]);
        else
          put(x, col, a, 1, azv, azx, ld[zl][col] + lu[zl][x], cd[zl][col] + cu[zl][x]);
      }
    }
    __syncthreads();
  }
}

__device__ __forceinline__ void sup_trailing_body(const SupWork& W, const int32_t* __restrict__ farc,
                                                  unsigned long long* __restrict__ D, unsigned long long* __restrict__ up,
                                                  unsigned long long* __restrict__ dn) {
  constexpr int B = SUP_B, T = SUP_TT;
  __shared__ float A[T][B + 1];
  __shared__ float Bm[B][T + 1];
  const SupNode S = W.sn;
  const int n = S.n, m = S.m, tid = threadIdx.x;
  const int nb = (m + B - 1) / B;
  const int k0 = W.b * B, k1 = min(k0 + B, m), kb = k1 - k0;
  const int zr0 = W.b + 1 < nb ? min(k1 + B, m) : k1;
  const int y0 = zr0 + W.t0 * T, z0 = zr0 + W.t1 * T;
  unsigned long long* Df = D + S.dofs;
#pragma unroll
  for (int h = 0; h < 2; ++h) {
    const int e = tid + 1024 * h;
    {
      const int r = e / B, p = e % B;
      A[r][p] = (y0 + r < n && p < kb) ? wof(Df[(long long)(y0 + r) * n + k0 + p]) : F_INF;
    }
    {
      const int p = e / T, c = e % T;
      Bm[p][c] = (p < kb && z0 + c < n) ? wof(Df[(long long)(k0 + p) * n + z0 + c]) : F_INF;
    }
  }
  const int ty = tid >> 4, tz = tid & 15;
  const int y = y0 + ty;
  unsigned long long old[4];
#pragma unroll
  for (int j = 0; j < 4; ++j) {
    const int z = z0 + tz + 16 * j;
    old[j] = (y < n && z < n && y != z) ? Df[(long long)y * n + z] : PACK_INF_D;
  }
  __syncthreads();
  float bw[4];
  int bp[4];
#pragma unroll
  for (int j = 0; j < 4; ++j) {
    bw[j] = F_INF;
    bp[j] = 0;
  }
  for (int p = 0; p < kb; ++p) {
    const float a = A[ty][p];
#pragma unroll
    for (int j = 0; j < 4; ++j) {
      const float sum = a + Bm[p][tz + 16 * j];
      if (sum < bw[j]) {
        bw[j] = sum;
        bp[j] = p;
      }
    }
  }
  const bool last = k1 == m;
  const int32_t* F = farc + S.foff;
// ... 670 lines not shown
  SupWork* dwk = nullptr;
  int32_t *dfn = nullptr, *dfa = nullptr;
  PArc* dpa = nullptr;
  bool ok = up_copy(dsn, sn.data(), sn.size()) == hipSuccess && up_copy(dwk, work.data(), work.size()) == hipSuccess &&
            up_copy(dfn, fnode.data(), fnode.size()) == hipSuccess && dmalloc(dfa, (size_t)foff) == hipSuccess &&
            up_copy(dpa, parc.data(), parc.size()) == hipSuccess && dmalloc(cs0_.sup_buf, 3 * (size_t)buf) == hipSuccess;
  if (ok) {
    hipLaunchKernelGGL(sup_farc_kernel, dim3((unsigned)cdiv(all_rows.cnt, 4)), dim3(256), 0, 0, dsn, dwk + all_rows.off,
                       (long long)all_rows.cnt, dfn, d_up_ptr, d_up_head, dfa);
    ok = hipGetLastError() == hipSuccess && hipDeviceSynchronize() == hipSuccess;
  }
  if (!ok) {
    (void)hipGetLastError();
    dfree(dsn);
    dfree(dwk);
    dfree(dfn);
    dfree(dfa);
    dfree(dpa);
    dfree(cs0_.sup_buf);
    std::fprintf(stderr, "[cch] supernodal plan: device allocation failed; per-level customization\n");
    return;
  }
  d_sup_sn = dsn;
  d_sup_work = dwk;
  d_sup_fnode = dfn;
  d_sup_farc = dfa;
  d_parc2 = dpa;
  sup_buf_entries_ = buf;
  sup_lev_ = std::move(levs);
  sup_node_ = std::move(node_in);
  rlev_aofs_ = std::move(raofs);
  rlev_nodes_ = std::move(rnodes);
  rlev_kmax_ = std::move(rkmax);
  rlev_multi_ = std::move(rmulti);
  sup_fronts_ = (int)sn.size();
  sup_nodes_ = nodes_in;
  sup_blocks_ = blocks;
  sparse_heights_ = hmax + 1;
  sup_on_ = true;
}

bool CchGpu::build_pull_records(const std::vector<int64_t>& tofs) {
  if (sup_on_) return true;
  const int N = T_.N;
  std::vector<PArc> parc((size_t)aofs_[N]);
  for (int i = 0; i < N; ++i) {
    const int x = T_.dlev_nodes[i];
    const int a0 = (int)T_.up_ptr[x], k = (int)(T_.up_ptr[x + 1] - T_.up_ptr[x]);
    if (k > 0xFFFF) return false;
    for (int ia = 0; ia < k; ++ia)
      parc[(size_t)aofs_[i] + ia] = PArc{tofs[x], a0, (int32_t)T_.up_head[a0 + ia], (uint16_t)k, (uint16_t)ia, 0};
  }
  PArc* dp = nullptr;
  const bool ok = up_copy(dp, parc.data(), parc.size()) == hipSuccess;
  d_parc = dp;
  return ok;
}

bool CchGpu::build_tasks(const std::vector<int64_t>& tofs) {
  std::vector<BasicTask> bt;
  btask_ptr_.assign(T_.max_height + 2, 0);
  for (int h = 0; h <= T_.max_height; ++h) {
    for (int64_t q = T_.hlev_ptr[h]; q < T_.hlev_ptr[h + 1]; ++q) {
      const int z = T_.hlev_nodes[q];
      if (sup_on_ && sup_node_[z]) continue;
      const int k = (int)(T_.up_ptr[z + 1] - T_.up_ptr[z]);
      if (k > 0xFFFE) return false;
      const int a0 = (int)T_.up_ptr[z];
      for (int j0 = 0; j0 < k; j0 += 64)
        bt.push_back(BasicTask{0, z, a0, (uint16_t)k, ROW_FINAL, (uint16_t)j0, 0});
      for (int i = 0; i + 1 < k; ++i) {
        const int64_t rb = tofs[z] + (int64_t)i * (2 * k - i - 1) / 2 - i - 1;
        for (int j0 = i + 1; j0 < k; j0 += 64)
          bt.push_back(BasicTask{rb, z, a0, (uint16_t)k, (uint16_t)i, (uint16_t)j0, 0});
      }
    }
    btask_ptr_[h + 1] = (int64_t)bt.size();
  }
  BasicTask* db = nullptr;
  const bool ok = up_copy(db, bt.data(), bt.size()) == hipSuccess;
  d_btask = db;
  if (ok) n_btask_ = (int64_t)bt.size();
  return ok;
}

hipError_t CchGpu::alloc_scratch(CustScratch& x) {
  const int N = T_.N;
  const int64_t M = T_.M;
  hipError_t e = hipSuccess;
  auto ck = [&](hipError_t r) {
    if (r != hipSuccess && e == hipSuccess) e = r;
  };
  ck(dmalloc(x.up64, M));
  ck(dmalloc(x.dn64, M));
  ck(dmalloc(x.pup, M));
  ck(dmalloc(x.pdn, M));
  ck(dmalloc(x.fcnt, N));
  ck(dmalloc(x.bcnt, N));
  size_t tb = 0;
  ck(hipcub::DeviceScan::InclusiveSum(nullptr, tb, x.fcnt, x.fcnt, N));
  x.cub_bytes = tb;
  ck(hipMalloc(&x.cub, x.cub_bytes ? x.cub_bytes : 1));
  ck(hipHostMalloc((void**)&x.h_stage, (size_t)std::max<int64_t>(1, T_.E) * sizeof(float), hipHostMallocDefault));
  if (sup_on_) ck(dmalloc(x.sup_buf, 3 * (size_t)sup_buf_entries_));
  return e;
}

void CchGpu::free_scratch(CustScratch& x) {
  dfree(x.up64);
  dfree(x.dn64);
  dfree(x.pup);
  dfree(x.pdn);
  dfree(x.fcnt);
  dfree(x.bcnt);
  if (x.cub) (void)hipFree(x.cub);
  x.cub = nullptr;
  if (x.rec_buf) (void)hipFree(x.rec_buf);
  x.rec_buf = nullptr;
  dfree(x.min_buf);
  if (x.h_stage) (void)hipHostFree(x.h_stage);
  x.h_stage = nullptr;
  dfree(x.sup_buf);
  dfree(x.avoid_dev);
  if (x.avoid_host) (void)hipHostFree(x.avoid_host);
  x.avoid_host = nullptr;
}

hipError_t CchGpu::context_costs(const CchContext& c, float* d_cost, hipStream_t s, CustScratch* cs) {
  if (eta_blob_ == nullptr || d_class == nullptr || d_base_traffic == nullptr) return hipErrorInvalidValue;
  const int E = (int)T_.E;
  hipError_t e = hipSuccess;
  std::unique_lock<std::mutex> lk(mu_cust_, std::defer_lock);
  if (cs == nullptr) lk.lock();
  CustScratch& X = cs ? *cs : cs0_;
  void*& rec_buf = X.rec_buf;
  float*& min_buf = X.min_buf;
  if (rec_buf == nullptr) {
    if ((e = hipMalloc(&rec_buf, (size_t)2 * E * sizeof(EtaRecordDev))) != hipSuccess) return e;
    if ((e = dmalloc(min_buf, (size_t)2 * E)) != hipSuccess) return e;
  }
  hipLaunchKernelGGL(ctx_records_kernel, dim3(blocks_for(E, 256)), dim3(256), 0, s, d_base_traffic, E, c.weather,
                     c.congestion, c.weekhour, c.driver_age, (EtaRecordDev*)rec_buf);
  if ((e = hipGetLastError()) != hipSuccess) return e;
  e = launch_eta_mlp3_fwd(rec_buf, min_buf, 2 * E, eta_blob_, eta_H_, eta_np_, eta_variant_, eta_cus_, s, 16);
  if (e != hipSuccess) return e;
  hipLaunchKernelGGL(ctx_cost_kernel, dim3(blocks_for(E, 256)), dim3(256), 0, s, min_buf, d_length, d_class, E, d_cost);
  e = hipGetLastError();
  if (e == hipSuccess && c.avoid) e = apply_avoid(*c.avoid, d_cost, nullptr, s, X);
  if (e == hipSuccess && cs == nullptr) e = hipStreamSynchronize(s);
  return e;
}

namespace {

inline long long wave_cap(int max_wg) { return max_wg > 0 ? 4LL * max_wg : (1LL << 40); }

template <class F>
hipError_t launch_pieces(long long total, long long cap, F&& launch) {
  for (long long i0 = 0; i0 < total; i0 += cap) {
    launch(i0, std::min(cap, total - i0));
    const hipError_t e = hipGetLastError();
    if (e != hipSuccess) return e;
  }
  return hipSuccess;
}

constexpr int PULL_WAVE_K = 64;

hipError_t pull_level(hipStream_t s, const CustScratch& X, PullArgs P, long long nodes, int km, int wave_km, int max_wg) {
  const bool wave = P.arcs >= 24 * nodes || km >= wave_km;
  const int S = P.arcs >= 8192 ? 1 : (km > 768 ? 4 : (km > 256 ? 2 : 1));
  const long long cap = wave ? std::max(1LL, wave_cap(max_wg) / S) : 64 * wave_cap(max_wg);
  const long long base = P.base;
  return launch_pieces(P.arcs, cap, [&](long long a0, long long n) {
    P.base = base + a0;
    P.arcs = n;
    if (wave && S == 4)
      hipLaunchKernelGGL(perfect_pull_wave_kernel<4>, dim3((unsigned)P.arcs), dim3(256), 0, s, P, X.up64, X.dn64,
                         X.pup, X.pdn);
    else if (wave && S == 2)
      hipLaunchKernelGGL(perfect_pull_wave_kernel<2>, dim3((unsigned)((P.arcs + 1) / 2)), dim3(256), 0, s, P,
                         X.up64, X.dn64, X.pup, X.pdn);
    else if (wave)
      hipLaunchKernelGGL(perfect_pull_wave_kernel<1>, dim3((unsigned)((P.arcs + 3) / 4)), dim3(256), 0, s, P,
                         X.up64, X.dn64, X.pup, X.pdn);
    else
      hipLaunchKernelGGL(perfect_pull_lane_kernel, dim3(blocks_for(P.arcs, 256)), dim3(256), 0, s, P, X.up64,
                         X.dn64, X.pup, X.pdn);
  });
}

}

hipError_t CchGpu::reset_weights(hipStream_t s, CustScratch& X, CchMetricDev& m) {
  const int64_t M = T_.M, E = T_.E;
  const int fill_blocks = (int)std::min<int64_t>(4096, (M + 255) / 256 + 1);
  hipLaunchKernelGGL(fill_u64_kernel, dim3(fill_blocks), dim3(256), 0, s, X.up64, (long long)M, PACK_INF_D);
  hipLaunchKernelGGL(fill_u64_kernel, dim3(fill_blocks), dim3(256), 0, s, X.dn64, (long long)M, PACK_INF_D);
  hipLaunchKernelGGL(edge_scatter_kernel, dim3(blocks_for(E, 256)), dim3(256), 0, s, m.cost, d_edge_arc, d_edge_dir,
                     (int)E, X.up64, X.dn64);
  return hipGetLastError();
}

hipError_t CchGpu::basic_phase(hipStream_t s, CustScratch& X, CchMetricDev& m, int max_wg) {
  hipError_t e = hipSuccess;
  if (!accel_) {
    for (int h = 0; h <= T_.max_height && e == hipSuccess; ++h) {
      LevelArgs L{d_up_ptr, d_up_head, d_hnodes, d_bofs, (int)T_.hlev_ptr[h], (int)T_.hlev_ptr[h + 1], 0, 0};
      if (L.lo >= L.hi) continue;
      L.base = bofs_[L.lo];
      L.items = bofs_[L.hi] - bofs_[L.lo];
      if (L.items <= 0) continue;
      hipLaunchKernelGGL(basic_level_kernel, dim3(blocks_for(L.items, 256)), dim3(256), 0, s, L, X.up64, X.dn64,
                         m.sub_up, m.sub_dn, m.len_up, m.len_dn, m.cnt_up, m.cnt_dn, d_length);
      e = hipGetLastError();
    }
    return e;
  }
  for (int h = 0; h <= T_.max_height && e == hipSuccess; ++h) {
    const BasicTask* level = (const BasicTask*)d_btask + btask_ptr_[h];
    e = launch_pieces(btask_ptr_[h + 1] - btask_ptr_[h], wave_cap(max_wg), [&](long long t0, long long nt) {
      hipLaunchKernelGGL(basic_task_kernel, dim3((unsigned)((nt + 3) / 4)), dim3(256), 0, s, level + t0, nt, d_up_ptr,
                         d_up_head, d_tri, X.up64, X.dn64, m.sub_up, m.sub_dn, m.len_up, m.len_dn, m.cnt_up, m.cnt_dn,
                         d_length);
    });
  }
  if (!sup_on_ || e != hipSuccess) return e;
  if (X.sup_buf == nullptr) return hipErrorOutOfMemory;
  const SupNode* sup_sn = (const SupNode*)d_sup_sn;
  const SupWork* sup_wk = (const SupWork*)d_sup_work;
  int2* sup_ss = (int2*)(X.sup_buf + sup_buf_entries_);
  int2* sup_sl = (int2*)(X.sup_buf + 2 * sup_buf_entries_);
  for (size_t l = 0; l < sup_lev_.size() && e == hipSuccess; ++l) {
    const SupLevel& SL = sup_lev_[l];
    hipLaunchKernelGGL(sup_gather_basic_kernel, dim3((unsigned)SL.gather.cnt), dim3(256), 0, s, sup_sn,
                       sup_wk + SL.gather.off, d_sup_fnode, d_sup_farc, X.up64, X.dn64, d_up_ptr, d_up_head, m.len_up,
                       m.len_dn, m.cnt_up, m.cnt_dn, X.sup_buf, sup_ss, sup_sl);
    for (size_t r = 0; r < SL.panel.size(); ++r)
      if (SL.panel[r].cnt > 0)
        hipLaunchKernelGGL(sup_step_basic_kernel, dim3((unsigned)SL.panel[r].cnt), dim3(1024), 0, s,
                           sup_wk + SL.panel[r].off, d_sup_farc, X.sup_buf, sup_ss, sup_sl, X.up64, X.dn64, m.sub_up,
                           m.sub_dn, m.len_up, m.len_dn, m.cnt_up, m.cnt_dn, d_length);
    e = hipGetLastError();
  }
  return e;
}

hipError_t CchGpu::perfect_phase(hipStream_t s, CustScratch& X, CchMetricDev& m, int max_wg) {
  (void)m;
  const int64_t M = T_.M;
  const int fill_blocks = (int)std::min<int64_t>(4096, (M + 255) / 256 + 1);
  hipLaunchKernelGGL(perfect_init_kernel, dim3(fill_blocks), dim3(256), 0, s, X.up64, X.dn64, X.pup, X.pdn, (long long)M);
  hipError_t e = hipGetLastError();
  if (!accel_) {
    for (int d = 0; d <= T_.max_depth && e == hipSuccess; ++d) {
      LevelArgs L{d_up_ptr, d_up_head, d_dnodes, d_pofs, (int)T_.dlev_ptr[d], (int)T_.dlev_ptr[d + 1], 0, 0};
      if (L.lo >= L.hi) continue;
      L.base = pofs_[L.lo];
      L.items = pofs_[L.hi] - pofs_[L.lo];
      if (L.items <= 0) continue;
      hipLaunchKernelGGL(perfect_level_kernel, dim3(blocks_for(L.items, 256)), dim3(256), 0, s, L, X.up64, X.dn64, X.pup,
                         X.pdn);
      e = hipGetLastError();
    }
    return e;
  }
  if (!sup_on_) {
    for (int d = 0; d <= T_.max_depth && e == hipSuccess; ++d) {
      const int lo = (int)T_.dlev_ptr[d], hi = (int)T_.dlev_ptr[d + 1];
      if (lo >= hi) continue;
      const PullArgs P{d_up_head, d_tri, (const PArc*)d_parc, aofs_[lo], aofs_[hi] - aofs_[lo]};
      if (P.arcs <= 0 || pofs_[hi] == pofs_[lo]) continue;
      e = pull_level(s, X, P, hi - lo, plev_kmax_[d], 1 << 30, max_wg);
    }
    return e;
  }
  const SupNode* sup_sn = (const SupNode*)d_sup_sn;
  const SupWork* sup_wk = (const SupWork*)d_sup_work;
  for (int l = (int)sup_lev_.size() - 1; l >= 0 && e == hipSuccess; --l) {
    const SupLevel& SL = sup_lev_[l];
    float* Dp = (float*)X.sup_buf;
    hipLaunchKernelGGL(sup_gather_perfect_kernel, dim3(blocks_for(SL.gather.cnt, 4)), dim3(256), 0, s, sup_sn,
                       sup_wk + SL.gather.off, (long long)SL.gather.cnt, d_sup_farc, X.up64, X.dn64, X.pup, X.pdn, Dp);
    for (size_t r = 0; r < SL.px.size(); ++r) {
      if (SL.px[r].cnt > 0)
        hipLaunchKernelGGL(sup_kk_gemm_perfect_kernel, dim3((unsigned)SL.px[r].cnt), dim3(1024), 0, s,
                           sup_wk + SL.px[r].off, d_sup_farc, Dp, X.pup, X.pdn);
      if (r < SL.py.size() && SL.py[r].cnt > 0)
        hipLaunchKernelGGL(sup_solve_perfect_kernel, dim3((unsigned)SL.py[r].cnt), dim3(1024), 0, s, sup_sn,
                           sup_wk + SL.py[r].off, d_sup_farc, Dp, X.pup, X.pdn);
    }
    e = hipGetLastError();
  }
  for (size_t d = 0; d < rlev_nodes_.size() && e == hipSuccess; ++d) {
    if (!rlev_multi_[d]) continue;
    const PullArgs P{d_up_head, d_tri, (const PArc*)d_parc2, rlev_aofs_[d], rlev_aofs_[d + 1] - rlev_aofs_[d]};
    e = pull_level(s, X, P, rlev_nodes_[d], rlev_kmax_[d], PULL_WAVE_K, max_wg);
  }
  return e;
}

hipError_t CchGpu::prune_phase(hipStream_t s, CustScratch& X, CchMetricDev& m) {
  const int N = T_.N;
  hipError_t e = hipSuccess;
  auto ck = [&](hipError_t x) {
    if (x != hipSuccess && e == hipSuccess) e = x;
  };
  hipLaunchKernelGGL(prune_count_wave_kernel, dim3((unsigned)((N + 3) / 4)), dim3(256), 0, s, d_up_ptr, X.pup, X.pdn,
                     X.up64, X.dn64, N, X.fcnt, X.bcnt);
  ck(hipGetLastError());
  ck(hipMemsetAsync(m.f_ptr, 0, sizeof(int32_t), s));
  ck(hipMemsetAsync(m.b_ptr, 0, sizeof(int32_t), s));
  size_t tb = X.cub_bytes;
  ck(hipcub::DeviceScan::InclusiveSum(X.cub, tb, X.fcnt, m.f_ptr + 1, N, s));
  tb = X.cub_bytes;
  ck(hipcub::DeviceScan::InclusiveSum(X.cub, tb, X.bcnt, m.b_ptr + 1, N, s));
  int32_t tot[2] = {0, 0};
  ck(hipMemcpyAsync(&tot[0], m.f_ptr + N, 4, hipMemcpyDeviceToHost, s));
  ck(hipMemcpyAsync(&tot[1], m.b_ptr + N, 4, hipMemcpyDeviceToHost, s));
  ck(hipStreamSynchronize(s));
  if (e != hipSuccess) return e;
  if (tot[0] > m.kept_f || m.f_rec == nullptr) {
    dfree(m.f_rec);
    ck(dmalloc(m.f_rec, tot[0]));
  }
  if (tot[1] > m.kept_b || m.b_rec == nullptr) {
    dfree(m.b_rec);
    ck(dmalloc(m.b_rec, tot[1]));
  }
  m.kept_f = tot[0];
  m.kept_b = tot[1];
  if (e != hipSuccess) return e;
  hipLaunchKernelGGL(prune_scatter_wave_kernel, dim3((unsigned)((N + 3) / 4)), dim3(256), 0, s, d_up_ptr, d_up_head,
                     d_depth, X.pup, X.pdn, X.up64, X.dn64, N, m.f_ptr, m.b_ptr, m.f_rec, m.b_rec);
  return hipGetLastError();
}

hipError_t CchGpu::customize(const float* d_cost, CchMetricDev& m, hipStream_t s, CustScratch* cs) {
  std::unique_lock<std::mutex> lk(mu_cust_, std::defer_lock);
  if (cs == nullptr) lk.lock();
  CustScratch& X = cs ? *cs : cs0_;
  const bool paced = cs != nullptr && builder_max_wg_.load() > 0 && (pace_always_.load() || serving_now());
  if (paced) n_paced_.fetch_add(1, std::memory_order_relaxed);
  const int max_wg = paced ? std::max(0, builder_max_wg_.load(std::memory_order_relaxed)) : 0;
  auto t0 = std::chrono::steady_clock::now();
  const int N = T_.N;
  const int64_t M = T_.M, E = T_.E;
  m.device = dev_;
  hipError_t e = hipSuccess;
  auto ck = [&](hipError_t x) {
    if (x != hipSuccess && e == hipSuccess) e = x;
  };
  const auto ta = std::chrono::steady_clock::now();
  if (m.cost == nullptr) ck(dmalloc(m.cost, E));
  if (m.sub_up == nullptr) {
    ck(dmalloc(m.sub_up, 2 * M));
    ck(dmalloc(m.sub_dn, 2 * M));
    ck(dmalloc(m.len_up, M));
    ck(dmalloc(m.len_dn, M));
    ck(dmalloc(m.cnt_up, M));
    ck(dmalloc(m.cnt_dn, M));
    ck(dmalloc(m.f_ptr, N + 1));
    ck(dmalloc(m.b_ptr, N + 1));
  }
  m.alloc_ms += std::chrono::duration<double, std::milli>(std::chrono::steady_clock::now() - ta).count();
  if (e != hipSuccess) return e;
  if (d_cost != m.cost) ck(hipMemcpyAsync(m.cost, d_cost, E * sizeof(float), hipMemcpyDeviceToDevice, s));
  struct Events {
    hipEvent_t e[4] = {};
    Events() {
      for (auto& x : e)
        if (hipEventCreate(&x) != hipSuccess) x = nullptr;
    }
    ~Events() {
      for (auto& x : e)
        if (x) (void)hipEventDestroy(x);
    }
  } evs;
  hipEvent_t* ev = evs.e;
  ck(reset_weights(s, X, m));
  if (ev[0]) (void)hipEventRecord(ev[0], s);
  if (e == hipSuccess) ck(basic_phase(s, X, m, max_wg));
  if (ev[1]) (void)hipEventRecord(ev[1], s);
  if (e == hipSuccess) ck(perfect_phase(s, X, m, max_wg));
  if (ev[2]) (void)hipEventRecord(ev[2], s);
  if (e == hipSuccess) ck(prune_phase(s, X, m));
  if (ev[3]) (void)hipEventRecord(ev[3], s);
  ck(hipStreamSynchronize(s));
  if (e != hipSuccess) return e;
  m.customize_ms = std::chrono::duration<double, std::milli>(std::chrono::steady_clock::now() - t0).count();
  float ms = 0.f;
  if (ev[0] && ev[1] && hipEventElapsedTime(&ms, ev[0], ev[1]) == hipSuccess) m.basic_ms = ms;
  if (ev[1] && ev[2] && hipEventElapsedTime(&ms, ev[1], ev[2]) == hipSuccess) m.perfect_ms = ms;
  if (ev[2] && ev[3] && hipEventElapsedTime(&ms, ev[2], ev[3]) == hipSuccess) m.prune_ms = ms;
  const auto th = std::chrono::steady_clock::now();
  m.host_cost.resize((size_t)E);
  if (X.h_stage != nullptr) {
    ck(hipMemcpyAsync(X.h_stage, m.cost, (size_t)E * sizeof(float), hipMemcpyDeviceToHost, s));
    ck(hipStreamSynchronize(s));
    if (e == hipSuccess) std::memcpy(m.host_cost.data(), X.h_stage, (size_t)E * sizeof(float));
  } else {
    ck(hipMemcpyAsync(m.host_cost.data(), m.cost, (size_t)E * sizeof(float), hipMemcpyDeviceToHost, s));
    ck(hipStreamSynchronize(s));
  }
  if (e != hipSuccess) m.host_cost.clear();
  m.hostcopy_ms = std::chrono::duration<double, std::milli>(std::chrono::steady_clock::now() - th).count();
  return e;
}

}
```

csrc/cch_gpu.h:

```cpp
#pragma once
#include <hip/hip_runtime.h>

#include <cstdint>
#include <cstdlib>
#include <cstring>
#include <atomic>
#include <chrono>
#include <condition_variable>
#include <deque>
#include <functional>
#include <list>
#include <memory>
#include <mutex>
#include <thread>
#include <unordered_set>
#include <vector>

#include "common.h"
#include "runtime/cch.h"

namespace rt {

struct CchContext {
  int weather = 2, congestion = 1, weekhour = 9;
  float driver_age = 35.f;
  std::shared_ptr<const std::vector<int32_t>> avoid;
  uint32_t avoid_digest = 0;
  uint64_t key() const {
    return (uint64_t)(weather & 0xFF) | ((uint64_t)(congestion & 0xFF) << 8) | ((uint64_t)(weekhour & 0xFFFF) << 16) |
           (avoid ? (uint64_t)(avoid_digest & 0x7FFFFFFFu) << 32 : 0);
  }
};

struct CchMetricDev {
  uint64_t key = 0;
  int device = 0;
  float* cost = nullptr;
  int32_t* sub_up = nullptr;
  int32_t* sub_dn = nullptr;
  float* len_up = nullptr;
  float* len_dn = nullptr;
  int32_t* cnt_up = nullptr;
  int32_t* cnt_dn = nullptr;
  int32_t* f_ptr = nullptr;
  int32_t* b_ptr = nullptr;
  int4* f_rec = nullptr;
  int4* b_rec = nullptr;
  int64_t kept_f = 0, kept_b = 0;
  double customize_ms = 0.0, cost_ms = 0.0;
  double basic_ms = 0.0, perfect_ms = 0.0, prune_ms = 0.0;
  double alloc_ms = 0.0, hostcopy_ms = 0.0;
  std::vector<float> host_cost;
  std::shared_ptr<const std::vector<int32_t>> avoid;
  ~CchMetricDev();
};

struct CchScratch {
  float* dist = nullptr;
  int32_t* pred = nullptr;
  int32_t* node = nullptr;
  size_t jobs_cap = 0;
  int32_t* jobs = nullptr;
  int32_t* arcs = nullptr;
  int32_t* narcs = nullptr;
  size_t pairs_cap = 0;
  int32_t* pj = nullptr;
  size_t pj_cap = 0;
  uint64_t chain_tag = 0;
  int chain_nm = 0, chain_r = 0;
  int device = 0;
  std::vector<void*> old;
  ~CchScratch();
  hipError_t ensure(size_t jobs, size_t pairs, int stride, int max_arcs);
};

struct CchAllScratch {
  float* sec = nullptr;
  float* met = nullptr;
  size_t blocks_cap = 0;
  int device = 0;
  std::vector<void*> old;
  ~CchAllScratch();
  hipError_t ensure(size_t blocks, size_t N);
};

struct CustScratch {
  unsigned long long *up64 = nullptr, *dn64 = nullptr;
  uint32_t *pup = nullptr, *pdn = nullptr;
  int32_t *fcnt = nullptr, *bcnt = nullptr;
  void* cub = nullptr;
  size_t cub_bytes = 0;
  void* rec_buf = nullptr;
  float* min_buf = nullptr;
  float* h_stage = nullptr;
  unsigned long long* sup_buf = nullptr;
  int32_t* avoid_dev = nullptr;
  int32_t* avoid_host = nullptr;
};

struct CchMView {
  const int32_t* f_ptr;
  const int32_t* b_ptr;
  const int4* f_rec;
  const int4* b_rec;
  const float* len_up;
  const float* len_dn;
  const int32_t* sub_up;
  const int32_t* sub_dn;
  const int32_t* cnt_up;
  const int32_t* cnt_dn;
};

struct CchRouteOut {
  float* sec = nullptr;
  float* metres = nullptr;
  int* status = nullptr;
  int* len = nullptr;
  int* path = nullptr;
  int* edges = nullptr;
  int max_path = 0;
};

class CchGpu {
 public:
  CchGpu(rcch::Topology T, const float* length, const uint8_t* road_class, const uint8_t* base_traffic, int device);
  ~CchGpu();
  const rcch::Topology& topo() const { return T_; }
  int device() const { return dev_; }
  int stride() const { return T_.max_depth + 1; }
  bool has_triangle_table() const { return accel_; }
  int64_t triangles() const { return n_tri; }
  int64_t basic_tasks() const { return n_btask_; }
  bool supernodal() const { return sup_on_; }
  int sup_fronts() const { return sup_fronts_; }
  int sup_nodes() const { return sup_nodes_; }
  int sup_levels() const { return (int)sup_lev_.size(); }
  int sup_blocks() const { return sup_blocks_; }
  int sparse_heights() const { return sparse_heights_; }
  int sparse_depths() const { return (int)rlev_nodes_.size(); }

  void set_eta(const void* blob, int H, const NormParams& np, int variant, int num_cus);
  bool has_eta() const { return eta_blob_ != nullptr; }
  hipError_t context_costs(const CchContext& c, float* d_cost, hipStream_t s, CustScratch* cs = nullptr);

  void set_geometry(const int32_t* indptr, const int32_t* indices, const int32_t* qx, const int32_t* qy);
  hipError_t avoid_mask(const std::vector<int32_t>& blob, uint8_t* d_mask, hipStream_t s);
  bool avoid_clash(const CchContext& c);

  hipError_t customize(const float* d_cost, CchMetricDev& m, hipStream_t s, CustScratch* cs = nullptr);

  hipError_t metric_for(const CchContext& c, hipStream_t s, std::shared_ptr<CchMetricDev>& out, bool* fresh = nullptr,
                        CustScratch* cs = nullptr);
  hipError_t metric_from_costs(uint64_t key, const float* d_cost, hipStream_t s, std::shared_ptr<CchMetricDev>& out);
  bool cached_metric(uint64_t key, std::shared_ptr<CchMetricDev>& out);
  void set_capacity(int n) {
    std::lock_guard<std::mutex> lk(mu_);
    capacity_ = n < 1 ? 1 : n;
    cache_gb_ = 0.0;
  }
  void set_cache_gb(double gb);
  double cache_gb() { std::lock_guard<std::mutex> lk(mu_); return cache_gb_; }
  int capacity() { std::lock_guard<std::mutex> lk(mu_); return capacity_; }
  int64_t metric_bytes() const { return metric_bytes_.load(); }
  int cached() { std::lock_guard<std::mutex> lk(mu_); return (int)cache_.size(); }

  void request_build(const CchContext& c, bool urgent = true);
  void start_builders();
  int add_build_listener(std::function<void(uint64_t, bool)> cb);
  void remove_build_listener(int id);
  struct AsyncStats {
    long long queued = 0, built = 0, failed = 0;
    int pending = 0;
    double build_ms = 0.0, alloc_ms = 0.0, hostcopy_ms = 0.0;
    long long paced = 0;
  };
  AsyncStats async_stats();
  void set_builder_pacing(int n, bool always = false) {
    builder_max_wg_.store(n < 0 ? 0 : n);
    pace_always_.store(always);
  }
  int builder_pacing() const { return builder_max_wg_.load(); }
  void set_unpack_serial(bool on) { unpack_serial_.store(on); }
  bool unpack_serial() const { return unpack_serial_.load(); }
  void note_queries() {
    query_us_.store(std::chrono::duration_cast<std::chrono::microseconds>(
                        std::chrono::steady_clock::now().time_since_epoch()).count(),
                    std::memory_order_relaxed);
  }
  bool serving_now() const {
    const long long now = std::chrono::duration_cast<std::chrono::microseconds>(
                              std::chrono::steady_clock::now().time_since_epoch()).count();
    return now - query_us_.load(std::memory_order_relaxed) < 250000;
  }

  hipError_t route(const CchMetricDev& m, const int* d_src, const int* d_dst, int Q, const CchRouteOut& o,
                   CchScratch& sc, hipStream_t s);
  hipError_t matrix(const CchMetricDev& m, const int* d_pts, const int* d_npts, int R, int NM, float* d_sec,
                    float* d_met, double* d_D64, CchScratch& sc, hipStream_t s);
  hipError_t legs_from_matrix(const CchMetricDev& m, const int* d_src, const int* d_r, const int* d_i, const int* d_j,
                              int Q, uint64_t tag, const CchRouteOut& o, CchScratch& sc, hipStream_t s);
  static constexpr int MAX_ARCS = 1024;
  enum { MEET_AUTO = 0, MEET_RECT = 1, MEET_PAIRS = 2, MEET_NONE = 3 };
  hipError_t matrix_rect(const CchMetricDev& m, const int* d_src, const int* d_nsrc, const int* d_dst,
                         const int* d_ndst, int R, int SM, int DM, float* d_sec, float* d_met, CchScratch& sc,
                         hipStream_t s, int meet = MEET_AUTO);

  hipError_t one_to_all(const CchMetricDev& m, const int* d_src, int S, bool reverse, float* d_sec, float* d_met,
                        CchAllScratch& sc, hipStream_t s, int fuse = -1);
  static constexpr size_t ALL_SCRATCH_BYTES = 1ull << 30;
  static constexpr int ALL_FUSE_WIDTH = 4;

  static CchMView view(const CchMetricDev& m) {
    return CchMView{m.f_ptr, m.b_ptr, m.f_rec, m.b_rec, m.len_up, m.len_dn, m.sub_up, m.sub_dn, m.cnt_up, m.cnt_dn};
  }
  hipError_t route_multi(const CchMView* d_mv, const int* d_grp, const int* d_src, const int* d_dst, int Q,
                         const CchRouteOut& o, CchScratch& sc, hipStream_t s);
  hipError_t matrix_multi(const CchMView* d_mv, const int* d_row_grp, const int* d_pts, const int* d_npts, int R, int NM,
                          float* d_sec, float* d_met, double* d_D64, CchScratch& sc, hipStream_t s);
  hipError_t legs_from_matrix_multi(const CchMView* d_mv, const int* d_grp, const int* d_src, const int* d_r,
                                    const int* d_i, const int* d_j, int Q, uint64_t tag, const CchRouteOut& o,
                                    CchScratch& sc, hipStream_t s);

 private:
  hipError_t route_impl(const CchMetricDev* m, const CchMView* mv, const int* grp, const int* d_src, const int* d_dst,
                        int Q, const CchRouteOut& o, CchScratch& sc, hipStream_t s);
  hipError_t matrix_impl(const CchMetricDev* m, const CchMView* mv, const int* grp, const int* d_pts, const int* d_npts,
                         int R, int NM, float* d_sec, float* d_met, double* d_D64, CchScratch& sc, hipStream_t s);
  hipError_t legs_impl(const CchMetricDev* m, const CchMView* mv, const int* grp, const int* d_src, const int* d_r,
                       const int* d_i, const int* d_j, int Q, uint64_t tag, const CchRouteOut& o, CchScratch& sc,
                       hipStream_t s);
  hipError_t launch_unpack(const CchMetricDev* m, const CchMView* mv, const int* grp, int Q, const int* d_src,
                           CchScratch& sc, const CchRouteOut& o, hipStream_t s);
  rcch::Topology T_;
  int dev_ = 0;
  int32_t *d_up_ptr = nullptr, *d_up_head = nullptr, *d_arc_lo = nullptr, *d_parent = nullptr, *d_depth = nullptr;
  int32_t *d_rank = nullptr, *d_node = nullptr, *d_edge_arc = nullptr;
  uint8_t* d_edge_dir = nullptr;
  float* d_length = nullptr;
  uint8_t *d_class = nullptr, *d_base_traffic = nullptr;
  int32_t *d_hnodes = nullptr, *d_dnodes = nullptr;
  int32_t* d_dlev_ptr = nullptr;
  int64_t *d_bofs = nullptr, *d_pofs = nullptr;
  std::vector<int64_t> bofs_, pofs_, aofs_;
  std::vector<int> plev_kmax_;
  bool accel_ = false;
  void build_tables();
  void free_tables();
  bool build_triangles(const std::vector<int64_t>& tofs);
  int32_t* d_tri = nullptr;
  int64_t n_tri = 0;
  bool build_tasks(const std::vector<int64_t>& tofs);
  bool build_pull_records(const std::vector<int64_t>& tofs);
  void* d_btask = nullptr;
  std::vector<int64_t> btask_ptr_;
  int64_t n_btask_ = 0;
  void* d_parc = nullptr;
  void build_supernodes(const std::vector<int64_t>& tofs);
  struct SupRange {
    int64_t off = 0, cnt = 0;
  };
  struct SupLevel {
    SupRange gather;
    std::vector<SupRange> panel;
    std::vector<SupRange> px, py;
  };
  bool sup_on_ = false;
  std::vector<uint8_t> sup_node_;
  std::vector<SupLevel> sup_lev_;
  void* d_sup_sn = nullptr;
  void* d_sup_work = nullptr;
  int32_t* d_sup_fnode = nullptr;
  int32_t* d_sup_farc = nullptr;
  int64_t sup_buf_entries_ = 0;
  int sup_fronts_ = 0, sup_nodes_ = 0, sup_blocks_ = 0, sparse_heights_ = 0;
  void* d_parc2 = nullptr;
  std::vector<int64_t> rlev_aofs_;
  std::vector<int> rlev_nodes_, rlev_kmax_;
  std::vector<uint8_t> rlev_multi_;
  hipError_t alloc_scratch(CustScratch& x);
  void free_scratch(CustScratch& x);
  hipError_t reset_weights(hipStream_t s, CustScratch& x, CchMetricDev& m);
  hipError_t basic_phase(hipStream_t s, CustScratch& x, CchMetricDev& m, int max_wg);
  hipError_t perfect_phase(hipStream_t s, CustScratch& x, CchMetricDev& m, int max_wg);
  hipError_t prune_phase(hipStream_t s, CustScratch& x, CchMetricDev& m);
  CustScratch cs0_;
  std::vector<std::unique_ptr<CustScratch>> bscr_;
  std::mutex mu_cust_;
  std::mutex mu_inflight_;
  std::condition_variable cv_inflight_;
  std::unordered_set<uint64_t> inflight_;
  const void* eta_blob_ = nullptr;
  int eta_H_ = 0, eta_variant_ = -1, eta_cus_ = 256;
  NormParams eta_np_{};
  std::mutex mu_;
  std::list<std::shared_ptr<CchMetricDev>> cache_;
  int capacity_ = 32;
  double cache_gb_ = 48.0;
  std::atomic<int64_t> metric_bytes_{0};
  void insert_cached(const std::shared_ptr<CchMetricDev>& m);
  hipError_t ensure_geometry();
  void free_geometry();
  hipError_t apply_avoid(const std::vector<int32_t>& blob, float* d_cost, uint8_t* d_mask, hipStream_t s, CustScratch& X);
  std::mutex mu_geom_;
  std::vector<int32_t> h_esrc_, h_edst_, h_qx_, h_qy_;
  int32_t *d_esrc = nullptr, *d_edst = nullptr, *d_qx = nullptr, *d_qy = nullptr;
  std::atomic<uint64_t> tag_ctr_{0};
  void builder_loop(int idx);
  void start_builders_locked();
  void notify_built(uint64_t key, bool ok);
  std::vector<std::thread> bths_;
  std::mutex bmu_;
  std::condition_variable bcv_;
  std::deque<CchContext> bq_;
  std::unordered_set<uint64_t> bpending_;
  bool bstop_ = false;
  std::mutex lmu_;
  std::vector<std::pair<int, std::function<void(uint64_t, bool)>>> listeners_;
  int next_listener_ = 1;
  std::atomic<long long> n_bqueued_{0}, n_bbuilt_{0}, n_bfailed_{0};
  std::atomic<long long> us_build_{0}, us_alloc_{0}, us_hostcopy_{0};
  std::atomic<long long> query_us_{-(1LL << 40)};
  std::atomic<bool> pace_always_{false};
  std::atomic<long long> n_paced_{0};
  std::atomic<int> builder_max_wg_{[] {
    const char* v = std::getenv("ROUTEST_CCH_BUILDER_MAX_WG");
    return v ? std::max(0, std::atoi(v)) : -1;
  }()};
  std::atomic<bool> unpack_serial_{[] {
    const char* v = std::getenv("ROUTEST_CCH_UNPACK");
    return v != nullptr && std::strcmp(v, "serial") == 0;
  }()};
};

}
```

csrc/cch_query.hip:

```cpp
#include "cch_dev.h"
#include "cch_gpu.h"

namespace rt {

using namespace cchd;

namespace {

constexpr int SWEEP_AHEAD = 3;
constexpr int SWEEP_RECS = 4;

typedef int sweep_v4i __attribute__((ext_vector_type(4)));

struct SweepRecs {
  sweep_v4i r[SWEEP_RECS];
};

__device__ __forceinline__ SweepRecs sweep_fetch(const int4* __restrict__ rec, int pb, int pe, int i, int L, int lane) {
  SweepRecs v;
  const int ii = i < 63 ? i : 63;
  const int b = __shfl(pb, ii);
  const int e = i < L ? __shfl(pe, ii) : b;
#pragma unroll
  for (int k = 0; k < SWEEP_RECS; ++k) {
    const int idx = b + lane + 64 * k;
    const int4* p = rec + (idx < e ? idx : 0);
    asm volatile("global_load_dwordx4 %0, %1, off" : "=v"(v.r[k]) : "v"(p));
  }
  return v;
}

template <int NEWER>
__device__ __forceinline__ void sweep_wait(SweepRecs& q) {
  static_assert(NEWER * SWEEP_RECS <= 63, "vmcnt range");
  asm volatile("s_waitcnt vmcnt(%4)" : "+v"(q.r[0]), "+v"(q.r[1]), "+v"(q.r[2]), "+v"(q.r[3]) : "n"(NEWER * SWEEP_RECS));
}

__device__ __forceinline__ void sweep_relax(float* sd, int32_t* sp, float dx, int w, int hd, int arc) {
  const float nd = dx + __int_as_float(w);
  if (nd < sd[hd]) {
    sd[hd] = nd;
    sp[hd] = arc;
  }
}

__global__ __launch_bounds__(64) void sweep_kernel(const int32_t* __restrict__ jobs, int J,
                                                   const int32_t* __restrict__ parent,
                                                   const int32_t* __restrict__ depth, int N,
                                                   const int32_t* __restrict__ f_ptr, const int4* __restrict__ f_rec,
                                                   const int32_t* __restrict__ b_ptr, const int4* __restrict__ b_rec,
                                                   int stride, float* __restrict__ out_dist,
                                                   int32_t* __restrict__ out_pred, int32_t* __restrict__ out_node,
                                                   const CchMView* __restrict__ mv, const int32_t* __restrict__ grp,
                                                   int gdiv) {
  extern __shared__ unsigned char smem[];
  float* sd = reinterpret_cast<float*>(smem);
  int32_t* sp = reinterpret_cast<int32_t*>(smem + (size_t)stride * 4);
  const int j = blockIdx.x;
  if (j >= J) return;
  const int lane = threadIdx.x;
  const int code = jobs[j];
  if (code < 0) return;
  const int r = code >> 1;
  const bool fwd = (code & 1) == 0;
  if (mv != nullptr) {
    const CchMView& v = mv[grp[j / gdiv]];
    f_ptr = v.f_ptr;
    f_rec = v.f_rec;
    b_ptr = v.b_ptr;
    b_rec = v.b_rec;
  }
  const int32_t* __restrict__ ptr = fwd ? f_ptr : b_ptr;
  const int4* __restrict__ rec = fwd ? f_rec : b_rec;
  const int D = depth[r];
  for (int d = lane; d <= D; d += 64) {
    sd[d] = F_INF;
    sp[d] = -1;
  }
  __syncthreads();
  if (lane == 0) sd[D] = 0.f;
  __syncthreads();
  const size_t base = (size_t)j * stride;
  int x = r, d = D;
  int cand = x + lane;
  int par = cand < N ? parent[cand] : -2;
  int pb = cand < N ? ptr[cand] : 0;
  int pe = cand < N ? ptr[cand + 1] : 0;
  while (x >= 0 && d >= 0) {
    const unsigned long long cont = __ballot(cand < N && par == cand + 1);
    int L = (~cont == 0ull) ? 64 : (__builtin_ctzll(~cont) + 1);
    if (L > d + 1) L = d + 1;
    const int next = __shfl(par, L - 1);
    if (lane < L) out_node[base + (d - lane)] = x + lane;
    const int ncand = next + lane;
    const bool nin = next >= 0 && ncand < N;
    const int npar = nin ? parent[ncand] : -2;
    const int npb = nin ? ptr[ncand] : 0;
    const int npe = nin ? ptr[ncand + 1] : 0;
    auto node = [&](int i, const SweepRecs& q) {
      if (i >= L) return;
      const float dx = sd[d - i];
      if (dx < F_INF) {
        const int b = __shfl(pb, i), e = __shfl(pe, i);
#pragma unroll
        for (int k = 0; k < SWEEP_RECS; ++k)
          if (b + lane + 64 * k < e) sweep_relax(sd, sp, dx, q.r[k].x, q.r[k].y, q.r[k].z);
        for (int k = b + 64 * SWEEP_RECS + lane; k < e; k += 64) {
          const int4 rc = rec[k];
          sweep_relax(sd, sp, dx, rc.x, rc.y, rc.z);
        }
        __syncthreads();
      }
    };
    SweepRecs qa = sweep_fetch(rec, pb, pe, 0, L, lane);
    SweepRecs qb = sweep_fetch(rec, pb, pe, 1, L, lane);
    SweepRecs qc = sweep_fetch(rec, pb, pe, 2, L, lane);
    for (int i = 0; i < L; i += 4) {
      SweepRecs qd = sweep_fetch(rec, pb, pe, i + 3, L, lane);
      sweep_wait<3>(qa);
      node(i, qa);
      qa = sweep_fetch(rec, pb, pe, i + 4, L, lane);
      sweep_wait<3>(qb);
      node(i + 1, qb);
      qb = sweep_fetch(rec, pb, pe, i + 5, L, lane);
      sweep_wait<3>(qc);
      node(i + 2, qc);
      qc = sweep_fetch(rec, pb, pe, i + 6, L, lane);
      sweep_wait<3>(qd);
      node(i + 3, qd);
    }
    sweep_wait<0>(qa);
    sweep_wait<0>(qb);
    sweep_wait<0>(qc);
    x = next;
    d -= L;
    cand = ncand;
    par = npar;
    pb = npb;
    pe = npe;
  }
  __syncthreads();
  for (int dd = lane; dd <= D; dd += 64) {
    out_dist[base + dd] = sd[dd];
    out_pred[base + dd] = sp[dd];
  }
}

__global__ __launch_bounds__(64) void meet_kernel(int P, const int32_t* __restrict__ pjf, const int32_t* __restrict__ pjb,
                                                  int jf0, int jb0, const int32_t* __restrict__ jobs, int stride,
                                                  const float* __restrict__ sdist, const int32_t* __restrict__ spred,
                                                  const int32_t* __restrict__ snode, const int32_t* __restrict__ depth,
                                                  const int32_t* __restrict__ arc_lo, const float* __restrict__ len_up,
                                                  const float* __restrict__ len_dn, float* __restrict__ out_sec,
                                                  float* __restrict__ out_met, int* __restrict__ out_status,
                                                  int32_t* __restrict__ arcs, int32_t* __restrict__ narcs, int max_arcs,
                                                  const CchMView* __restrict__ mv, const int32_t* __restrict__ grp,
                                                  int gdiv) {
  __shared__ int32_t fw[4096];
  const int q = blockIdx.x;
  if (q >= P) return;
  const int lane = threadIdx.x;
  if (mv != nullptr) {
    const CchMView& v = mv[grp[q / gdiv]];
    len_up = v.len_up;
    len_dn = v.len_dn;
  }
  const int jf = pjf ? pjf[q] : jf0 + 2 * q;
  const int jb = pjb ? pjb[q] : jb0 + 2 * q;
  if (jobs[jf] < 0 || jobs[jb] < 0) {
    if (threadIdx.x == 0) {
      if (out_sec) out_sec[q] = -1.f;
      if (out_met) out_met[q] = -1.f;
      if (out_status) out_status[q] = 1;
      if (narcs) narcs[q] = 0;
    }
    return;
  }
  const int s = jobs[jf] >> 1, t = jobs[jb] >> 1;
  const int ds = depth[s], dt = depth[t];
  const size_t bf = (size_t)jf * stride, bb = (size_t)jb * stride;
  int status = 1;
  float best = F_INF;
  int bestd = -1;
  if (snode[bf] == snode[bb]) {
    int lo = 0, hi = ds < dt ? ds : dt;
    while (lo < hi) {
      const int mid = (lo + hi + 1) >> 1;
      if (snode[bf + mid] == snode[bb + mid]) lo = mid;
      else hi = mid - 1;
    }
    const int L = lo;
    for (int d = lane; d <= L; d += 64) {
      const float v = sdist[bf + d] + sdist[bb + d];
      if (v < best || (v == best && d > bestd)) {
        best = v;
        bestd = d;
      }
    }
#pragma unroll
    for (int o = 32; o >= 1; o >>= 1) {
      const float ov = __shfl_xor(best, o);
      const int od = __shfl_xor(bestd, o);
      if (ov < best || (ov == best && od > bestd)) {
        best = ov;
        bestd = od;
      }
    }
    if (best < F_INF) status = 0;
  }
  if (lane != 0) return;
  float met = 0.f;
  int n = 0;
  if (status == 0) {
    int nf = 0;
    for (int slot = bestd; slot != ds;) {
      const int a = spred[bf + slot];
      met += len_up[a];
      if (nf < 4096) fw[nf] = a;
      ++nf;
      slot = depth[arc_lo[a]];
    }
    if (arcs != nullptr) {
      int32_t* out = arcs + (size_t)q * max_arcs;
      if (nf > 4096 || nf > max_arcs) status = 4;
      for (int i = nf - 1; i >= 0 && status == 0; --i) out[n++] = fw[i] << 1;
      for (int slot = bestd; slot != dt && status == 0;) {
        const int a = spred[bb + slot];
        met += len_dn[a];
        if (n >= max_arcs) { status = 4; break; }
        out[n++] = (a << 1) | 1;
        slot = depth[arc_lo[a]];
      }
    } else {
      for (int slot = bestd; slot != dt;) {
        const int a = spred[bb + slot];
        met += len_dn[a];
        slot = depth[arc_lo[a]];
      }
    }
  }
  if (out_sec) out_sec[q] = status == 0 ? best : -1.f;
  if (out_met) out_met[q] = status == 0 ? met : -1.f;
  if (out_status) out_status[q] = status;
  if (narcs) narcs[q] = n;
}

constexpr int UNPACK_STACK = 128;
__global__ __launch_bounds__(64) void unpack_kernel(int P, const int* __restrict__ src_node, const int32_t* __restrict__ arcs,
                                                    const int32_t* __restrict__ narcs, int max_arcs,
                                                    const int32_t* __restrict__ sub_up,
                                                    const int32_t* __restrict__ sub_dn,
                                                    const int32_t* __restrict__ arc_lo,
                                                    const int32_t* __restrict__ up_head,
                                                    const int32_t* __restrict__ node_of, int* __restrict__ status,
                                                    int* __restrict__ out_len, int* __restrict__ out_path, int max_path,
                                                    int min_arcs, int* __restrict__ out_edge,
                                                    const CchMView* __restrict__ mv, const int32_t* __restrict__ grp) {
  __shared__ int32_t stk[64 * UNPACK_STACK];
  const int q = blockIdx.x * blockDim.x + threadIdx.x;
  if (q >= P) return;
  if (mv != nullptr) {
    const CchMView& v = mv[grp[q]];
    sub_up = v.sub_up;
    sub_dn = v.sub_dn;
  }
  int32_t* st = stk + threadIdx.x * UNPACK_STACK;
  if (status[q] != 0) {
    if (min_arcs < 0) out_len[q] = 0;
    return;
  }
  if (narcs[q] <= min_arcs && out_len[q] != -1) return;
  int* out = out_path + (size_t)q * max_path;
  int n = 0;
  out[n++] = src_node[q];
  const int na = narcs[q];
  const int32_t* al = arcs + (size_t)q * max_arcs;
  bool ok = true;
  for (int k = 0; k < na && ok; ++k) {
    int sp = 0;
    st[sp++] = al[k];
    while (sp > 0) {
      const int code = st[--sp];
      const int a = code >> 1, dn = code & 1;
      const int32_t* sub = (dn ? sub_dn : sub_up) + 2 * (long long)a;
      const int s0 = sub[0];
      if (s0 < 0) {
        if (n >= max_path) { ok = false; break; }
        if (out_edge) out_edge[(size_t)q * max_path + n - 1] = sub[1];
        out[n++] = node_of[dn ? arc_lo[a] : up_head[a]];
        continue;
      }
      if (sp + 2 > UNPACK_STACK) { ok = false; break; }
      st[sp++] = sub[1] << 1;
      st[sp++] = (s0 << 1) | 1;
    }
  }
  if (!ok) {
    status[q] = 4;
    out_len[q] = 0;
    return;
  }
  out_len[q] = n;
}

constexpr int UNPACK_LANES = 16;
constexpr int UNPACK_MAX_ARCS = 256;
constexpr int UNPACK_SD = 64;
__global__ __launch_bounds__(64) void unpack_coop_kernel(int P, const int* __restrict__ src_node,
                                                         const int32_t* __restrict__ arcs,
                                                         const int32_t* __restrict__ narcs, int max_arcs,
                                                         const int32_t* __restrict__ sub_up,
                                                         const int32_t* __restrict__ sub_dn,
                                                         const int32_t* __restrict__ cnt_up,
                                                         const int32_t* __restrict__ cnt_dn,
                                                         const int32_t* __restrict__ arc_lo,
                                                         const int32_t* __restrict__ up_head,
                                                         const int32_t* __restrict__ node_of, int* __restrict__ status,
                                                         int* __restrict__ out_len, int* __restrict__ out_path,
                                                         int max_path, int* __restrict__ out_edge,
                                                         const CchMView* __restrict__ mv,
                                                         const int32_t* __restrict__ grp) {
  constexpr int G = 64 / UNPACK_LANES;
  __shared__ int32_t offs[G][UNPACK_MAX_ARCS + 1];
  __shared__ int32_t stk[64 * UNPACK_SD];
  const int lane = threadIdx.x, g = lane / UNPACK_LANES, sl = lane % UNPACK_LANES;
  const int q = blockIdx.x * G + g;
  const bool active = q < P;
  if (mv != nullptr && active) {
    const CchMView& v = mv[grp[q]];
    sub_up = v.sub_up;
    sub_dn = v.sub_dn;
    cnt_up = v.cnt_up;
    cnt_dn = v.cnt_dn;
  }
  int st = active ? status[q] : 1;
  const int na = active && st == 0 ? narcs[q] : 0;
  const bool coop = active && st == 0 && na <= UNPACK_MAX_ARCS;
  if (active && st != 0 && sl == 0) out_len[q] = 0;
  const int32_t* al = arcs + (size_t)(active ? q : 0) * max_arcs;
  int carry = 0;
  for (int b = 0; b < (coop ? na : 0); b += UNPACK_LANES) {
    const int k = b + sl;
    int c = 0;
    if (k < na) {
      const int code = al[k];
      c = (code & 1) ? cnt_dn[code >> 1] : cnt_up[code >> 1];
    }
    int incl = c;
#pragma unroll
    for (int o = 1; o < UNPACK_LANES; o <<= 1) {
      const int y = __shfl_up(incl, o, UNPACK_LANES);
      if (sl >= o) incl += y;
    }
    if (k < na) offs[g][k] = carry + incl - c;
    carry += __shfl(incl, UNPACK_LANES - 1, UNPACK_LANES);
  }
  const int E = carry;
  if (coop) {
    if (sl == 0) offs[g][na] = E;
    if (E + 1 > max_path) {
      if (sl == 0) {
        status[q] = 4;
        out_len[q] = 0;
      }
      st = 4;
    } else if (sl == 0) {
      out_len[q] = E + 1;
    }
  }
  __syncthreads();
  if (!coop || st != 0) return;
  int* out = out_path + (size_t)q * max_path;
  int* oe = out_edge ? out_edge + (size_t)q * max_path : nullptr;
  if (sl == 0) out[0] = src_node[q];
  const int per = (E + UNPACK_LANES - 1) / UNPACK_LANES;
  int e = sl * per;
  const int e1 = min(E, e + per);
  if (e >= e1) return;
  int32_t* sk = stk + lane * UNPACK_SD;
  int lo = 0, hi = na - 1;
  while (lo < hi) {
    const int mid = (lo + hi + 1) >> 1;
    if (offs[g][mid] <= e) lo = mid;
    else hi = mid - 1;
  }
  int k = lo;
  int r = e - offs[g][k];
  int sp = 0;
  bool ok = true;
  int code = al[k];
  auto descend = [&](int c, int rr) -> int {
    while (true) {
      const int a = c >> 1, dn = c & 1;
      const int32_t* sub = (dn ? sub_dn : sub_up) + 2 * (long long)a;
      const int s0 = sub[0];
      if (s0 < 0) return c;
      const int s1 = sub[1];
      const int first = (s0 << 1) | 1, second = s1 << 1;
      const int c0 = cnt_dn[s0];
      if (rr < c0) {
        if (sp >= UNPACK_SD) { ok = false; return c; }
        sk[sp++] = second;
        c = first;
      } else {
        rr -= c0;
        c = second;
      }
    }
  };
  int leaf = descend(code, r);
  while (ok) {
    const int a = leaf >> 1, dn = leaf & 1;
    out[e + 1] = node_of[dn ? arc_lo[a] : up_head[a]];
    if (oe) oe[e] = (dn ? sub_dn : sub_up)[2 * (long long)a + 1];
    if (++e >= e1) break;
    if (sp > 0) {
      leaf = descend(sk[--sp], 0);
    } else {
      ++k;
      leaf = descend(al[k], 0);
    }
  }
  if (!ok) out_len[q] = -1;
}

__global__ void route_jobs_kernel(const int* __restrict__ src, const int* __restrict__ dst, int Q,
                                  const int32_t* __restrict__ rank, int N, int32_t* __restrict__ jobs) {
  const int q = blockIdx.x * blockDim.x + threadIdx.x;
  if (q >= Q) return;
  int s = src[q], t = dst[q];
  s = (s < 0 || s >= N) ? 0 : s;
  t = (t < 0 || t >= N) ? 0 : t;
  jobs[2 * q] = rank[s] << 1;
  jobs[2 * q + 1] = (rank[t] << 1) | 1;
}

__global__ void leg_pairs_kernel(int NM, const int* __restrict__ r, const int* __restrict__ i,
                                 const int* __restrict__ j, int Q, int R, int32_t* __restrict__ pjf,
                                 int32_t* __restrict__ pjb) {
  const int q = blockIdx.x * blockDim.x + threadIdx.x;
  if (q >= Q) return;
  int rr = r[q], ii = i[q], jj = j[q];
  rr = rr < 0 ? 0 : (rr >= R ? R - 1 : rr);
  ii = ii < 0 ? 0 : (ii >= NM ? NM - 1 : ii);
  jj = jj < 0 ? 0 : (jj >= NM ? NM - 1 : jj);
  pjf[q] = 2 * (rr * NM + ii);
  pjb[q] = 2 * (rr * NM + jj) + 1;
}

__global__ void matrix_jobs_kernel(const int* __restrict__ pts, const int* __restrict__ npts, int R, int NM,
                                   const int32_t* __restrict__ rank, int N, int32_t* __restrict__ jobs) {
  const long long g = blockIdx.x * (long long)blockDim.x + threadIdx.x;
  if (g >= (long long)R * NM) return;
  const int r = (int)(g / NM), i = (int)(g % NM);
  if (i >= npts[r]) {
    jobs[2 * g] = -1;
    jobs[2 * g + 1] = -1;
    return;
  }
  int v = pts[g];
  if (v < 0 || v >= N) v = 0;
  jobs[2 * g] = rank[v] << 1;
  jobs[2 * g + 1] = (rank[v] << 1) | 1;
}

__global__ void matrix_pairs_kernel(const int* __restrict__ npts, int R, int NM, int32_t* __restrict__ pjf,
                                    int32_t* __restrict__ pjb) {
  const long long g = blockIdx.x * (long long)blockDim.x + threadIdx.x;
  if (g >= (long long)R * NM * NM) return;
  const int r = (int)(g / ((long long)NM * NM));
  const int rem = (int)(g % ((long long)NM * NM));
  const int i = rem / NM, j = rem % NM;
  pjf[g] = 2 * (r * NM + i);
  pjb[g] = 2 * (r * NM + j) + 1;
}

__global__ void matrix_out_kernel(const int* __restrict__ npts, int R, int NM, float* __restrict__ sec,
                                  float* __restrict__ met, double* __restrict__ D64) {
  const long long g = blockIdx.x * (long long)blockDim.x + threadIdx.x;
  if (g >= (long long)R * NM * NM) return;
  const int r = (int)(g / ((long long)NM * NM));
  const int rem = (int)(g % ((long long)NM * NM));
  const int i = rem / NM, j = rem % NM;
  const int n = npts[r];
  const bool diag = i == j;
  const bool out = i >= n || j >= n;
  float s = sec ? sec[g] : 0.f, m = met ? met[g] : 0.f;
  if (diag || out) s = m = 0.f;
  else {
    if (s < 0.f) s = F_INF;
    if (m < 0.f) m = F_INF;
  }
  if (sec) sec[g] = s;
  if (met) met[g] = m;
  if (D64) D64[g] = (double)m;
}

__global__ void rect_jobs_kernel(const int* __restrict__ src, const int* __restrict__ nsrc, const int* __restrict__ dst,
                                 const int* __restrict__ ndst, int R, int SM, int DM, const int32_t* __restrict__ rank,
                                 int N, int32_t* __restrict__ jobs) {
  const long long g = blockIdx.x * (long long)blockDim.x + threadIdx.x;
  const int W = SM + DM;
  if (g >= (long long)R * W) return;
  const int r = (int)(g / W), k = (int)(g % W);
  const bool fwd = k < SM;
  const int i = fwd ? k : k - SM;
  if (i >= (fwd ? nsrc[r] : ndst[r])) {
    jobs[g] = -1;
    return;
  }
  int v = fwd ? src[(size_t)r * SM + i] : dst[(size_t)r * DM + i];
  if (v < 0 || v >= N) v = 0;
  jobs[g] = (rank[v] << 1) | (fwd ? 0 : 1);
}

constexpr int MEET_TILE = 64;
constexpr int MEET_THREADS = 256;
__global__ __launch_bounds__(MEET_THREADS) void meet_rect_kernel(
    int SM, int DM, const int* __restrict__ nsrc, const int* __restrict__ ndst, const int32_t* __restrict__ jobs,
    int stride, const float* __restrict__ sdist, const int32_t* __restrict__ spred, const int32_t* __restrict__ snode,
    const int32_t* __restrict__ depth, const int32_t* __restrict__ arc_lo, const float* __restrict__ len_up,
    const float* __restrict__ len_dn, float* __restrict__ out_sec, float* __restrict__ out_met) {
  extern __shared__ unsigned char smem[];
  int32_t* fn = reinterpret_cast<int32_t*>(smem);
  float* fd = reinterpret_cast<float*>(smem + (size_t)stride * 4);
  int32_t* fp = reinterpret_cast<int32_t*>(smem + (size_t)stride * 8);
  __shared__ float s_best[MEET_TILE];
  __shared__ int s_bestd[MEET_TILE];
  const int tid = threadIdx.x;
  const int ntile = (DM + MEET_TILE - 1) / MEET_TILE;
  const int tile = blockIdx.x % ntile;
  const int i = (blockIdx.x / ntile) % SM;
  const int r = blockIdx.x / (ntile * SM);
  const int j0 = tile * MEET_TILE;
  const int nj = min(MEET_TILE, DM - j0);
  const int nv = min(nj, ndst[r] - j0);
  const size_t cell = ((size_t)r * SM + i) * DM + j0;
  if (i >= nsrc[r] || nv <= 0) {
    if (tid < nj) {
      out_sec[cell + tid] = 0.f;
      out_met[cell + tid] = 0.f;
    }
    return;
  }
  const size_t jrow = (size_t)r * (SM + DM);
  const int s = jobs[jrow + i] >> 1;
  const int ds = depth[s];
  const size_t bf = (jrow + i) * stride;
  for (int d = tid; d <= ds; d += MEET_THREADS) {
    fn[d] = snode[bf + d];
    fd[d] = sdist[bf + d];
    fp[d] = spred[bf + d];
  }
  __syncthreads();
  const int lane = tid & 63;
  for (int p = tid >> 6; p < nv; p += MEET_THREADS / 64) {
    const size_t jb = jrow + SM + j0 + p;
    const int t = jobs[jb] >> 1;
    const int dt = depth[t];
    const size_t bb = jb * stride;
    float best = F_INF;
    int bestd = -1;
    if (fn[0] == snode[bb]) {
      int lo = 0, hi = ds < dt ? ds : dt;
      while (lo < hi) {
        const int mid = (lo + hi + 1) >> 1;
        if (fn[mid] == snode[bb + mid]) lo = mid;
        else hi = mid - 1;
      }
      const int L = lo;
      for (int d = lane; d <= L; d += 64) {
        const float v = fd[d] + sdist[bb + d];
        if (v < best || (v == best && d > bestd)) {
          best = v;
          bestd = d;
        }
      }
#pragma unroll
      for (int o = 32; o >= 1; o >>= 1) {
        const float ov = __shfl_xor(best, o);
        const int od = __shfl_xor(bestd, o);
        if (ov < best || (ov == best && od > bestd)) {
          best = ov;
          bestd = od;
        }
      }
    }
    if (lane == 0) {
      s_best[p] = best;
      s_bestd[p] = bestd;
    }
  }
  __syncthreads();
  if (tid >= nj) return;
  float sec = 0.f, met = 0.f;
  if (tid < nv) {
    const size_t jb = jrow + SM + j0 + tid;
    const int t = jobs[jb] >> 1;
    if (t != s) {
      sec = s_best[tid];
      if (sec < F_INF) {
        const int dt = depth[t];
        const size_t bb = jb * stride;
        const int bestd = s_bestd[tid];
        for (int slot = bestd; slot != ds;) {
          const int a = fp[slot];
          met += len_up[a];
          slot = depth[arc_lo[a]];
        }
        for (int slot = bestd; slot != dt;) {
          const int a = spred[bb + slot];
          met += len_dn[a];
          slot = depth[arc_lo[a]];
        }
      } else {
        sec = met = F_INF;
      }
    }
  }
  out_sec[cell + tid] = sec;
  out_met[cell + tid] = met;
}

__global__ void rect_pairs_kernel(int R, int SM, int DM, int32_t* __restrict__ pjf, int32_t* __restrict__ pjb) {
  const long long g = blockIdx.x * (long long)blockDim.x + threadIdx.x;
  if (g >= (long long)R * SM * DM) return;
  const int r = (int)(g / ((long long)SM * DM));
  const int rem = (int)(g % ((long long)SM * DM));
  pjf[g] = r * (SM + DM) + rem / DM;
  pjb[g] = r * (SM + DM) + SM + rem % DM;
}

__global__ void rect_out_kernel(const int* __restrict__ nsrc, const int* __restrict__ ndst, int R, int SM, int DM,
                                const int32_t* __restrict__ jobs, float* __restrict__ sec, float* __restrict__ met) {
  const long long g = blockIdx.x * (long long)blockDim.x + threadIdx.x;
  if (g >= (long long)R * SM * DM) return;
  const int r = (int)(g / ((long long)SM * DM));
  const int rem = (int)(g % ((long long)SM * DM));
  const int i = rem / DM, j = rem % DM;
  float s = sec[g], m = met[g];
  const size_t jrow = (size_t)r * (SM + DM);
  if (i >= nsrc[r] || j >= ndst[r] || (jobs[jrow + i] >> 1) == (jobs[jrow + SM + j] >> 1)) s = m = 0.f;
  else {
    if (s < 0.f) s = F_INF;
    if (m < 0.f) m = F_INF;
  }
  sec[g] = s;
  met[g] = m;
}

}

CchScratch::~CchScratch() {
  int cur = 0;
  (void)hipGetDevice(&cur);
  (void)hipSetDevice(device);
  dfree(dist);
  dfree(pred);
  dfree(node);
  dfree(jobs);
  dfree(arcs);
  dfree(narcs);
  dfree(pj);
  for (void* p : old) (void)hipFree(p);
  (void)hipSetDevice(cur);
}

hipError_t CchScratch::ensure(size_t J, size_t P, int stride, int max_arcs) {
  hipError_t e = hipSuccess;
  auto retire = [&](auto*& p) {
    if (p) old.push_back((void*)p);
    p = nullptr;
  };
  if (J > jobs_cap) {
    retire(dist);
    retire(pred);
    retire(node);
    retire(jobs);
    const size_t cap = std::max(J, jobs_cap * 3 / 2);
    if ((e = dmalloc(dist, cap * stride)) != hipSuccess) return e;
    if ((e = dmalloc(pred, cap * stride)) != hipSuccess) return e;
    if ((e = dmalloc(node, cap * stride)) != hipSuccess) return e;
    if ((e = dmalloc(jobs, cap)) != hipSuccess) return e;
    jobs_cap = cap;
  }
  if (P > pairs_cap) {
    retire(arcs);
    retire(narcs);
    const size_t cap = std::max(P, pairs_cap * 3 / 2);
    if ((e = dmalloc(arcs, cap * (size_t)max_arcs)) != hipSuccess) return e;
    if ((e = dmalloc(narcs, cap)) != hipSuccess) return e;
    pairs_cap = cap;
  }
  return e;
}

hipError_t CchGpu::launch_unpack(const CchMetricDev* m, const CchMView* mv, const int* grp, int Q, const int* d_src,
                                 CchScratch& sc, const CchRouteOut& o, hipStream_t s) {
  const bool serial_only = unpack_serial();
  const int32_t* sub_up = m ? m->sub_up : nullptr;
  const int32_t* sub_dn = m ? m->sub_dn : nullptr;
  if (!serial_only) {
    constexpr int G = 64 / UNPACK_LANES;
    hipLaunchKernelGGL(unpack_coop_kernel, dim3((Q + G - 1) / G), dim3(64), 0, s, Q, d_src, sc.arcs, sc.narcs, MAX_ARCS,
                       sub_up, sub_dn, m ? m->cnt_up : nullptr, m ? m->cnt_dn : nullptr, d_arc_lo, d_up_head, d_node,
                       o.status, o.len, o.path, o.max_path, o.edges, mv, grp);
    hipError_t e = hipGetLastError();
    if (e != hipSuccess) return e;
  }
  hipLaunchKernelGGL(unpack_kernel, dim3(blocks_for(Q, 64)), dim3(64), 0, s, Q, d_src, sc.arcs, sc.narcs, MAX_ARCS,
                     sub_up, sub_dn, d_arc_lo, d_up_head, d_node, o.status, o.len, o.path, o.max_path,
                     serial_only ? -1 : UNPACK_MAX_ARCS, o.edges, mv, grp);
  return hipGetLastError();
}

hipError_t CchGpu::route_impl(const CchMetricDev* m, const CchMView* mv, const int* grp, const int* d_src,
                              const int* d_dst, int Q, const CchRouteOut& o, CchScratch& sc, hipStream_t s) {
  if (Q <= 0) return hipSuccess;
  const int S = stride();
  sc.device = dev_;
  sc.chain_tag = 0;
  hipError_t e = sc.ensure((size_t)2 * Q, (size_t)Q, S, MAX_ARCS);
  if (e != hipSuccess) return e;
  hipLaunchKernelGGL(route_jobs_kernel, dim3(blocks_for(Q, 256)), dim3(256), 0, s, d_src, d_dst, Q, d_rank, T_.N,
                     sc.jobs);
  hipLaunchKernelGGL(sweep_kernel, dim3(2 * Q), dim3(64), (size_t)S * 8, s, sc.jobs, 2 * Q, d_parent, d_depth, T_.N,
                     m ? m->f_ptr : nullptr, m ? m->f_rec : nullptr, m ? m->b_ptr : nullptr, m ? m->b_rec : nullptr, S,
                     sc.dist, sc.pred, sc.node, mv, grp, 2);
  if ((e = hipGetLastError()) != hipSuccess) return e;
  hipLaunchKernelGGL(meet_kernel, dim3(Q), dim3(64), 0, s, Q, nullptr, nullptr, 0, 1, sc.jobs, S, sc.dist, sc.pred,
                     sc.node, d_depth, d_arc_lo, m ? m->len_up : nullptr, m ? m->len_dn : nullptr, o.sec, o.metres,
                     o.status, o.path ? sc.arcs : nullptr, o.path ? sc.narcs : nullptr, MAX_ARCS, mv, grp, 1);
  if ((e = hipGetLastError()) != hipSuccess) return e;
  if (o.path != nullptr) e = launch_unpack(m, mv, grp, Q, d_src, sc, o, s);
  return e;
}

hipError_t CchGpu::route(const CchMetricDev& m, const int* d_src, const int* d_dst, int Q, const CchRouteOut& o,
                         CchScratch& sc, hipStream_t s) {
  return route_impl(&m, nullptr, nullptr, d_src, d_dst, Q, o, sc, s);
}

hipError_t CchGpu::route_multi(const CchMView* d_mv, const int* d_grp, const int* d_src, const int* d_dst, int Q,
                               const CchRouteOut& o, CchScratch& sc, hipStream_t s) {
  if (d_mv == nullptr || d_grp == nullptr) return hipErrorInvalidValue;
  return route_impl(nullptr, d_mv, d_grp, d_src, d_dst, Q, o, sc, s);
}

hipError_t CchGpu::matrix_impl(const CchMetricDev* m, const CchMView* mv, const int* grp, const int* d_pts,
                               const int* d_npts, int R, int NM, float* d_sec, float* d_met, double* d_D64,
                               CchScratch& sc, hipStream_t s) {
  if (R <= 0 || NM <= 0) return hipSuccess;
  if (d_sec == nullptr || d_met == nullptr) return hipErrorInvalidValue;
  const int S = stride();
  sc.device = dev_;
  const size_t J = (size_t)R * NM * 2, P = (size_t)R * NM * NM;
  hipError_t e = sc.ensure(J, (P * 2 + MAX_ARCS - 1) / MAX_ARCS + 1, S, MAX_ARCS);
  if (e != hipSuccess) return e;
  int32_t* pjf = sc.arcs;
  int32_t* pjb = sc.arcs + P;
  float* sec = d_sec;
  float* met = d_met;
  hipLaunchKernelGGL(matrix_jobs_kernel, dim3(blocks_for((long long)R * NM, 256)), dim3(256), 0, s, d_pts, d_npts, R, NM,
                     d_rank, T_.N, sc.jobs);
  hipLaunchKernelGGL(matrix_pairs_kernel, dim3(blocks_for((long long)P, 256)), dim3(256), 0, s, d_npts, R, NM, pjf, pjb);
  hipLaunchKernelGGL(sweep_kernel, dim3((unsigned)J), dim3(64), (size_t)S * 8, s, sc.jobs, (int)J, d_parent, d_depth,
                     T_.N, m ? m->f_ptr : nullptr, m ? m->f_rec : nullptr, m ? m->b_ptr : nullptr,
                     m ? m->b_rec : nullptr, S, sc.dist, sc.pred, sc.node, mv, grp, 2 * NM);
  if ((e = hipGetLastError()) != hipSuccess) return e;
  hipLaunchKernelGGL(meet_kernel, dim3((unsigned)P), dim3(64), 0, s, (int)P, pjf, pjb, 0, 0, sc.jobs, S, sc.dist,
                     sc.pred, sc.node, d_depth, d_arc_lo, m ? m->len_up : nullptr, m ? m->len_dn : nullptr, sec, met,
                     nullptr, nullptr, nullptr, MAX_ARCS, mv, grp, NM * NM);
  if ((e = hipGetLastError()) != hipSuccess) return e;
  hipLaunchKernelGGL(matrix_out_kernel, dim3(blocks_for((long long)P, 256)), dim3(256), 0, s, d_npts, R, NM, sec, met,
                     d_D64);
  e = hipGetLastError();
  sc.chain_tag = e == hipSuccess ? ++tag_ctr_ : 0;
  sc.chain_nm = NM;
  sc.chain_r = R;
  return e;
}

hipError_t CchGpu::matrix(const CchMetricDev& m, const int* d_pts, const int* d_npts, int R, int NM, float* d_sec,
                          float* d_met, double* d_D64, CchScratch& sc, hipStream_t s) {
  return matrix_impl(&m, nullptr, nullptr, d_pts, d_npts, R, NM, d_sec, d_met, d_D64, sc, s);
}

hipError_t CchGpu::matrix_multi(const CchMView* d_mv, const int* d_row_grp, const int* d_pts, const int* d_npts, int R,
                                int NM, float* d_sec, float* d_met, double* d_D64, CchScratch& sc, hipStream_t s) {
  if (d_mv == nullptr || d_row_grp == nullptr) return hipErrorInvalidValue;
  return matrix_impl(nullptr, d_mv, d_row_grp, d_pts, d_npts, R, NM, d_sec, d_met, d_D64, sc, s);
}

hipError_t CchGpu::matrix_rect(const CchMetricDev& m, const int* d_src, const int* d_nsrc, const int* d_dst,
                               const int* d_ndst, int R, int SM, int DM, float* d_sec, float* d_met, CchScratch& sc,
                               hipStream_t s, int meet) {
  if (R <= 0 || SM <= 0 || DM <= 0) return hipSuccess;
  if (d_sec == nullptr || d_met == nullptr || meet < MEET_AUTO || meet > MEET_NONE) return hipErrorInvalidValue;
  const int S = stride();
  const size_t J = (size_t)R * ((size_t)SM + DM), P = (size_t)R * SM * DM;
  if (J > (size_t)INT32_MAX || P > (size_t)INT32_MAX) return hipErrorInvalidValue;
  const size_t lds = (size_t)S * 12;
  const bool fits = lds + MEET_TILE * 8 <= 64 * 1024;
  if (meet == MEET_RECT && !fits) return hipErrorInvalidValue;
  if (meet == MEET_AUTO) meet = fits ? MEET_RECT : MEET_PAIRS;
  sc.device = dev_;
  sc.chain_tag = 0;
  hipError_t e = sc.ensure(J, meet == MEET_PAIRS ? (P * 2 + MAX_ARCS - 1) / MAX_ARCS + 1 : 0, S, MAX_ARCS);
  if (e != hipSuccess) return e;
  hipLaunchKernelGGL(rect_jobs_kernel, dim3(blocks_for((long long)J, 256)), dim3(256), 0, s, d_src, d_nsrc, d_dst,
                     d_ndst, R, SM, DM, d_rank, T_.N, sc.jobs);
  hipLaunchKernelGGL(sweep_kernel, dim3((unsigned)J), dim3(64), (size_t)S * 8, s, sc.jobs, (int)J, d_parent, d_depth,
                     T_.N, m.f_ptr, m.f_rec, m.b_ptr, m.b_rec, S, sc.dist, sc.pred, sc.node, nullptr, nullptr, 1);
  if ((e = hipGetLastError()) != hipSuccess) return e;
  if (meet == MEET_RECT) {
    const size_t blocks = (size_t)R * SM * ((DM + MEET_TILE - 1) / MEET_TILE);
    hipLaunchKernelGGL(meet_rect_kernel, dim3((unsigned)blocks), dim3(MEET_THREADS), lds, s, SM, DM, d_nsrc, d_ndst,
                       sc.jobs, S, sc.dist, sc.pred, sc.node, d_depth, d_arc_lo, m.len_up, m.len_dn, d_sec, d_met);
  } else if (meet == MEET_PAIRS) {
    int32_t* pjf = sc.arcs;
    int32_t* pjb = sc.arcs + P;
    hipLaunchKernelGGL(rect_pairs_kernel, dim3(blocks_for((long long)P, 256)), dim3(256), 0, s, R, SM, DM, pjf, pjb);
    hipLaunchKernelGGL(meet_kernel, dim3((unsigned)P), dim3(64), 0, s, (int)P, pjf, pjb, 0, 0, sc.jobs, S, sc.dist,
                       sc.pred, sc.node, d_depth, d_arc_lo, m.len_up, m.len_dn, d_sec, d_met, nullptr, nullptr, nullptr,
                       MAX_ARCS, nullptr, nullptr, 1);
    if ((e = hipGetLastError()) != hipSuccess) return e;
    hipLaunchKernelGGL(rect_out_kernel, dim3(blocks_for((long long)P, 256)), dim3(256), 0, s, d_nsrc, d_ndst, R, SM, DM,
                       sc.jobs, d_sec, d_met);
  }
  return hipGetLastError();
}

hipError_t CchGpu::legs_impl(const CchMetricDev* m, const CchMView* mv, const int* grp, const int* d_src,
                             const int* d_r, const int* d_i, const int* d_j, int Q, uint64_t tag, const CchRouteOut& o,
                             CchScratch& sc, hipStream_t s) {
  if (Q <= 0) return hipSuccess;
  if (tag == 0 || tag != sc.chain_tag) return hipErrorInvalidValue;
  const int S = stride();
  hipError_t e = sc.ensure(0, (size_t)Q, S, MAX_ARCS);
  if (e != hipSuccess) return e;
  if ((size_t)Q > sc.pj_cap) {
    if (sc.pj) sc.old.push_back((void*)sc.pj);
    sc.pj = nullptr;
    const size_t cap = std::max((size_t)Q, sc.pj_cap * 3 / 2);
    if ((e = dmalloc(sc.pj, 2 * cap)) != hipSuccess) return e;
    sc.pj_cap = cap;
  }
  int32_t* pjf = sc.pj;
  int32_t* pjb = sc.pj + sc.pj_cap;
  hipLaunchKernelGGL(leg_pairs_kernel, dim3(blocks_for(Q, 256)), dim3(256), 0, s, sc.chain_nm, d_r, d_i, d_j, Q,
                     sc.chain_r, pjf, pjb);
  if ((e = hipGetLastError()) != hipSuccess) return e;
  hipLaunchKernelGGL(meet_kernel, dim3(Q), dim3(64), 0, s, Q, pjf, pjb, 0, 0, sc.jobs, S, sc.dist, sc.pred, sc.node,
                     d_depth, d_arc_lo, m ? m->len_up : nullptr, m ? m->len_dn : nullptr, o.sec, o.metres, o.status,
                     o.path ? sc.arcs : nullptr, o.path ? sc.narcs : nullptr, MAX_ARCS, mv, grp, 1);
  if ((e = hipGetLastError()) != hipSuccess) return e;
  if (o.path != nullptr) e = launch_unpack(m, mv, grp, Q, d_src, sc, o, s);
  return e;
}

hipError_t CchGpu::legs_from_matrix(const CchMetricDev& m, const int* d_src, const int* d_r, const int* d_i,
                                    const int* d_j, int Q, uint64_t tag, const CchRouteOut& o, CchScratch& sc,
                                    hipStream_t s) {
  return legs_impl(&m, nullptr, nullptr, d_src, d_r, d_i, d_j, Q, tag, o, sc, s);
}

hipError_t CchGpu::legs_from_matrix_multi(const CchMView* d_mv, const int* d_grp, const int* d_src, const int* d_r,
                                          const int* d_i, const int* d_j, int Q, uint64_t tag, const CchRouteOut& o,
                                          CchScratch& sc, hipStream_t s) {
  if (d_mv == nullptr || d_grp == nullptr) return hipErrorInvalidValue;
  return legs_impl(nullptr, d_mv, d_grp, d_src, d_r, d_i, d_j, Q, tag, o, sc, s);
}

}
```

Measured before the change: 6.581 billion.

## Compress CCH kept-arc records from int4 to int2 with packed depth/offset

Shrinks each kept-arc record from 16 to 8 bytes by packing the head depth and the arc offset relative to up_ptr[x] into one 16/16-bit word, recovering the arc id as up_ptr[x] + offset. The sweep, up and pull kernels are changed to read the narrower records and the per-node up_ptr, and the sweep prefetch now loads two records per lane per dwordx4. This halves record bandwidth and footprint in the query sweeps, at the cost of an extra up_ptr load and an elimination-tree depth limit of 65535. Per-node arc counts must also fit in 16 bits. A debug export path expands the records back to int4.

After: 6.513 billion. 0.99x the previous value.

```diff
diff --git a/csrc/cch.hip b/csrc/cch.hip
--- a/csrc/cch.hip
+++ b/csrc/cch.hip
@@ -158,7 +158,8 @@
 }
 
 static int64_t metric_device_bytes(const CchMetricDev& m, int64_t N, int64_t M, int64_t E) {
-  return E * 4 + M * (8 + 8 + 4 + 4 + 4 + 4) + (N + 1) * 8 + (m.kept_f + m.kept_b) * 16;
+  return E * 4 + M * (8 + 8 + 4 + 4 + 4 + 4) + (N + 1) * 8 +
+         (m.kept_f + m.kept_b + 2 * CCH_REC_PAD) * (int64_t)sizeof(CchRec);
 }
 
 void CchGpu::insert_cached(const std::shared_ptr<CchMetricDev>& m) {
diff --git a/csrc/cch_all.hip b/csrc/cch_all.hip
--- a/csrc/cch_all.hip
+++ b/csrc/cch_all.hip
@@ -32,7 +32,8 @@
                                                         const int32_t* __restrict__ rank,
                                                         const int32_t* __restrict__ parent,
                                                         const int32_t* __restrict__ depth,
-                                                        const int32_t* __restrict__ ptr, const int4* __restrict__ rec,
+                                                        const int32_t* __restrict__ up_ptr,
+                                                        const int32_t* __restrict__ ptr, const CchRec* __restrict__ rec,
                                                         const float* __restrict__ len, int N, int stride,
                                                         float* __restrict__ wsec, float* __restrict__ wmet) {
   extern __shared__ unsigned char smem[];
@@ -61,15 +62,15 @@
   int x = r;
   for (int d = D; d >= 0 && x >= 0; --d) {
     const int par = parent[x];
-    const int kb = ptr[x], ke = ptr[x + 1];
+    const int kb = ptr[x], ke = ptr[x + 1], ab = up_ptr[x];
     if (lane == 0) sn[d] = x;
     const float dx = sd[d], mx = sm[d];
     if (dx < F_INF) {
       for (int k = kb + lane; k < ke; k += 64) {
-        const int4 rc = rec[k];
-        const int hd = rc.y;
+        const CchRec rc = rec[k];
+        const int hd = cch_rec_depth(rc);
         const float cs = dx + __int_as_float(rc.x);
-        const float cm = mx + len[rc.z];
+        const float cm = mx + len[ab + cch_rec_offset(rc)];
         if (hd >= 0 && hd < d && label_less(cs, cm, sd[hd], sm[hd])) {
           sd[hd] = cs;
           sm[hd] = cm;
@@ -122,18 +123,19 @@
   }
 }
 
-__device__ __forceinline__ void pull_part(int kb, int ke, int part, int parts, int t0, size_t base, int lane,
-                                          const int4* __restrict__ rec, const int32_t* __restrict__ up_head,
+__device__ __forceinline__ void pull_part(int kb, int ke, int ab, int part, int parts, int t0, size_t base, int lane,
+                                          const CchRec* __restrict__ rec, const int32_t* __restrict__ up_head,
                                           const float* __restrict__ len, const float* wsec, const float* wmet,
                                           float& bs, float& bm) {
   for (; kb + ALL_ROWS * (part + parts * t0) < ke; t0 += ALL_PRE) {
     const int k = chunk_record(kb, part, parts, t0, lane);
     int w_l = 0, u_l = 0, m_l = 0;
     if (k < ke) {
-      const int4 rc = rec[k];
+      const CchRec rc = rec[k];
+      const int a = ab + cch_rec_offset(rc);
       w_l = rc.x;
-      u_l = up_head[rc.z];
-      m_l = __float_as_int(len[rc.z]);
+      u_l = up_head[a];
+      m_l = __float_as_int(len[a]);
     }
     pull_chunks(kb, ke, part, parts, t0, w_l, u_l, m_l, base, wsec, wmet, bs, bm);
   }
@@ -141,9 +143,9 @@
 
 template <int WAVES>
 __global__ __launch_bounds__(64 * WAVES) void cch_all_pull_kernel(
-    const int32_t* __restrict__ dnodes, int lb, int cnt, int nblk, int N, const int32_t* __restrict__ ptr,
-    const int4* __restrict__ rec, const int32_t* __restrict__ up_head, const float* __restrict__ len, float* wsec,
-    float* wmet) {
+    const int32_t* __restrict__ dnodes, int lb, int cnt, int nblk, int N, const int32_t* __restrict__ up_ptr,
+    const int32_t* __restrict__ ptr, const CchRec* __restrict__ rec, const int32_t* __restrict__ up_head,
+    const float* __restrict__ len, float* wsec, float* wmet) {
   __shared__ float red_s[WAVES][64], red_m[WAVES][64];
   const int wave = __builtin_amdgcn_readfirstlane(threadIdx.x >> 6), lane = threadIdx.x & 63;
   const int ni = blockIdx.x / nblk, b = blockIdx.x % nblk;
@@ -158,7 +160,7 @@
     bs = wsec[row];
     bm = wmet[row];
   }
-  pull_part(kb, ke, wave, WAVES, 0, base, lane, rec, up_head, len, wsec, wmet, bs, bm);
+  pull_part(kb, ke, up_ptr[v], wave, WAVES, 0, base, lane, rec, up_head, len, wsec, wmet, bs, bm);
   if (WAVES > 1) {
     red_s[wave][lane] = bs;
     red_m[wave][lane] = bm;
@@ -177,41 +179,43 @@
 
 __global__ __launch_bounds__(ALL_FUSED_THREADS) void cch_all_pull_fused_kernel(
     const int32_t* __restrict__ dlev_ptr, const int32_t* __restrict__ dnodes, int d0, int d1, int N,
-    const int32_t* __restrict__ ptr, const int4* __restrict__ rec, const int32_t* __restrict__ up_head,
-    const float* __restrict__ len, float* wsec, float* wmet) {
+    const int32_t* __restrict__ up_ptr, const int32_t* __restrict__ ptr, const CchRec* __restrict__ rec,
+    const int32_t* __restrict__ up_head, const float* __restrict__ len, float* wsec, float* wmet) {
   constexpr int NW = ALL_FUSED_THREADS / 64;
   __shared__ float red_s[NW][64], red_m[NW][64];
   const int wave = __builtin_amdgcn_readfirstlane(threadIdx.x >> 6), lane = threadIdx.x & 63;
   const size_t base = (size_t)blockIdx.x * (size_t)N * 64 + (size_t)lane;
   int lb1 = 0, width1 = 0;
   int act2 = 0, part2 = 0, parts2 = 1, v2 = 0;
-  int act3 = 0, part3 = 0, parts3 = 1, v3 = 0, kb3 = 0, ke3 = 0;
-  int act4 = 0, part4 = 0, parts4 = 1, v4 = 0, kb4 = 0, ke4 = 0, n4 = 0;
-  int4 rc4 = make_int4(0, 0, 0, 0);
-  int act5 = 0, part5 = 0, parts5 = 1, v5 = 0, kb5 = 0, ke5 = 0;
+  int act3 = 0, part3 = 0, parts3 = 1, v3 = 0, kb3 = 0, ke3 = 0, ab3 = 0;
+  int act4 = 0, part4 = 0, parts4 = 1, v4 = 0, kb4 = 0, ke4 = 0, ab4 = 0, n4 = 0;
+  CchRec rc4 = make_int2(0, 0);
+  int act5 = 0, part5 = 0, parts5 = 1, v5 = 0, kb5 = 0, ke5 = 0, ab5 = 0;
   int w5 = 0, u5 = 0, m5 = 0;
   for (int d = d0 - 5; d < d1; ++d) {
-    const int act = act5, part = part5, parts = parts5, v = v5, kb = kb5, ke = ke5;
+    const int act = act5, part = part5, parts = parts5, v = v5, kb = kb5, ke = ke5, ab = ab5;
     const int w_l = w5, u_l = u5, m_l = m5;
-    act5 = act4, part5 = part4, parts5 = parts4, v5 = v4, kb5 = kb4, ke5 = ke4;
+    act5 = act4, part5 = part4, parts5 = parts4, v5 = v4, kb5 = kb4, ke5 = ke4, ab5 = ab4;
     w5 = rc4.x;
     u5 = m5 = 0;
     if (n4) {
-      u5 = up_head[rc4.z];
-      m5 = __float_as_int(len[rc4.z]);
-    }
-    act4 = act3, part4 = part3, parts4 = parts3, v4 = v3, kb4 = kb3, ke4 = ke3;
+      const int a = ab4 + cch_rec_offset(rc4);
+      u5 = up_head[a];
+      m5 = __float_as_int(len[a]);
+    }
+    act4 = act3, part4 = part3, parts4 = parts3, v4 = v3, kb4 = kb3, ke4 = ke3, ab4 = ab3;
     {
       const int k = chunk_record(kb3, part3, parts3, 0, lane);
       n4 = act3 && k < ke3;
-      rc4 = make_int4(0, 0, 0, 0);
+      rc4 = make_int2(0, 0);
       if (n4) rc4 = rec[k];
     }
     act3 = act2, part3 = part2, parts3 = parts2, v3 = v2;
-    kb3 = ke3 = 0;
+    kb3 = ke3 = ab3 = 0;
     if (act2) {
       kb3 = ptr[v2];
       ke3 = ptr[v2 + 1];
+      ab3 = up_ptr[v2];
     }
     act2 = 0, part2 = 0, parts2 = 1, v2 = 0;
     if (width1 > 0 && width1 <= NW) {
@@ -238,7 +242,7 @@
         bm = wmet[row];
       }
       pull_chunks(kb, ke, part, parts, 0, w_l, u_l, m_l, base, wsec, wmet, bs, bm);
-      pull_part(kb, ke, part, parts, ALL_PRE, base, lane, rec, up_head, len, wsec, wmet, bs, bm);
+      pull_part(kb, ke, ab, part, parts, ALL_PRE, base, lane, rec, up_head, len, wsec, wmet, bs, bm);
       red_s[wave][lane] = bs;
       red_m[wave][lane] = bm;
     }
@@ -316,10 +320,10 @@
   const size_t up_lds = (size_t)ST * 12;
   if (up_lds > 64 * 1024) return hipErrorInvalidValue;
   const int32_t* u_ptr = reverse ? m.b_ptr : m.f_ptr;
-  const int4* u_rec = reverse ? m.b_rec : m.f_rec;
+  const CchRec* u_rec = reverse ? m.b_rec : m.f_rec;
   const float* u_len = reverse ? m.len_dn : m.len_up;
   const int32_t* p_ptr = reverse ? m.f_ptr : m.b_ptr;
-  const int4* p_rec = reverse ? m.f_rec : m.b_rec;
+  const CchRec* p_rec = reverse ? m.f_rec : m.b_rec;
   const float* p_len = reverse ? m.len_up : m.len_dn;
   const size_t block_bytes = (size_t)N * 64 * 4 * 2;
   const int total_blocks = (S + 63) / 64;
@@ -335,22 +339,22 @@
     hipLaunchKernelGGL(cch_all_fill_kernel, dim3(blocks_for(n4, 256)), dim3(256), 0, s,
                        reinterpret_cast<float4*>(sc.sec), reinterpret_cast<float4*>(sc.met), n4);
     hipLaunchKernelGGL(cch_all_up_kernel, dim3(cnt), dim3(64), up_lds, s, d_src + s0, cnt, d_rank, d_parent, d_depth,
-                       u_ptr, u_rec, u_len, N, ST, sc.sec, sc.met);
+                       d_up_ptr, u_ptr, u_rec, u_len, N, ST, sc.sec, sc.met);
     if ((e = hipGetLastError()) != hipSuccess) return e;
     for (int d = 1; d <= T_.max_depth;) {
       int d1 = d;
       while (fuse > 0 && d1 <= T_.max_depth && T_.dlev_ptr[d1 + 1] - T_.dlev_ptr[d1] <= fuse) ++d1;
       if (d1 - d >= 2) {
         hipLaunchKernelGGL(cch_all_pull_fused_kernel, dim3(nb), dim3(ALL_FUSED_THREADS), 0, s, d_dlev_ptr, d_dnodes, d,
-                           d1, N, p_ptr, p_rec, d_up_head, p_len, sc.sec, sc.met);
+                           d1, N, d_up_ptr, p_ptr, p_rec, d_up_head, p_len, sc.sec, sc.met);
         d = d1;
       } else {
         const int lb = (int)T_.dlev_ptr[d], lc = (int)(T_.dlev_ptr[d + 1] - T_.dlev_ptr[d]);
         const int kmax = plev_kmax_[d];
         const dim3 grid((unsigned)((long long)lc * nb));
         auto launch = [&](auto kernel, int waves) {
-          hipLaunchKernelGGL(kernel, grid, dim3(64 * waves), 0, s, d_dnodes, lb, lc, nb, N, p_ptr, p_rec, d_up_head, p_len,
-                             sc.sec, sc.met);
+          hipLaunchKernelGGL(kernel, grid, dim3(64 * waves), 0, s, d_dnodes, lb, lc, nb, N, d_up_ptr, p_ptr, p_rec,
+                             d_up_head, p_len, sc.sec, sc.met);
         };
         if (kmax <= ALL_ROWS) launch(cch_all_pull_kernel<1>, 1);
         else if (kmax <= 2 * ALL_ROWS) launch(cch_all_pull_kernel<2>, 2);
diff --git a/csrc/cch_bindings.cpp b/csrc/cch_bindings.cpp
--- a/csrc/cch_bindings.cpp
+++ b/csrc/cch_bindings.cpp
@@ -252,8 +252,13 @@
     put("cnt_dn", m->cnt_dn, M, torch::kInt32);
     put("f_ptr", m->f_ptr, N + 1, torch::kInt32);
     put("b_ptr", m->b_ptr, N + 1, torch::kInt32);
-    put("f_rec", m->f_rec, 4 * m->kept_f, torch::kInt32);
-    put("b_rec", m->b_rec, 4 * m->kept_b, torch::kInt32);
+    auto put_rec = [&](const char* name, bool forward, int64_t kept) {
+      auto out = torch::empty({4 * kept}, opt.dtype(torch::kInt32));
+      if (kept > 0) CCH_CHECK_HIP(g_->expand_records(*m, forward, out.data_ptr<int32_t>(), stream_of(dev_)));
+      d[name] = out;
+    };
+    put_rec("f_rec", true, m->kept_f);
+    put_rec("b_rec", false, m->kept_b);
     return d;
   }
 
diff --git a/csrc/cch_customize.hip b/csrc/cch_customize.hip
--- a/csrc/cch_customize.hip
+++ b/csrc/cch_customize.hip
@@ -399,25 +399,39 @@
     const int32_t* __restrict__ up_ptr, const int32_t* __restrict__ up_head, const int32_t* __restrict__ depth,
     const uint32_t* __restrict__ pup, const uint32_t* __restrict__ pdn, const unsigned long long* __restrict__ up,
     const unsigned long long* __restrict__ dn, int N, const int32_t* __restrict__ f_ptr, const int32_t* __restrict__ b_ptr,
-    int4* __restrict__ f_rec, int4* __restrict__ b_rec) {
+    CchRec* __restrict__ f_rec, CchRec* __restrict__ b_rec) {
   const int x = blockIdx.x * 4 + (threadIdx.x >> 6);
   const int lane = threadIdx.x & 63;
   if (x >= N) return;
   int kf = f_ptr[x], kb = b_ptr[x];
   const unsigned long long below = (1ull << lane) - 1ull;
-  for (int a0 = up_ptr[x]; a0 < up_ptr[x + 1]; a0 += 64) {
+  const int ab = up_ptr[x];
+  for (int a0 = ab; a0 < up_ptr[x + 1]; a0 += 64) {
     const int a = a0 + lane;
     const bool in = a < up_ptr[x + 1];
     const bool f = in && kept(pup[a], up[a]);
     const bool b = in && kept(pdn[a], dn[a]);
     const unsigned long long mf = __ballot(f), mb = __ballot(b);
     if (f || b) {
-      const int hd = depth[up_head[a]];
-      if (f) f_rec[kf + __popcll(mf & below)] = make_int4((int)pup[a], hd, a, 0);
-      if (b) b_rec[kb + __popcll(mb & below)] = make_int4((int)pdn[a], hd, a, 0);
+      const int oh = (int)(((unsigned)(a - ab) << 16) | (unsigned)depth[up_head[a]]);
+      if (f) f_rec[kf + __popcll(mf & below)] = make_int2((int)pup[a], oh);
+      if (b) b_rec[kb + __popcll(mb & below)] = make_int2((int)pdn[a], oh);
     }
     kf += __popcll(mf);
     kb += __popcll(mb);
+  }
+}
+
+__global__ __launch_bounds__(256) void expand_records_kernel(const int32_t* __restrict__ up_ptr, int N,
+                                                             const int32_t* __restrict__ ptr,
+                                                             const CchRec* __restrict__ rec, int4* __restrict__ out) {
+  const int x = blockIdx.x * 4 + (threadIdx.x >> 6);
+  const int lane = threadIdx.x & 63;
+  if (x >= N) return;
+  const int ab = up_ptr[x];
+  for (int k = ptr[x] + lane; k < ptr[x + 1]; k += 64) {
+    const CchRec r = rec[k];
+    out[k] = make_int4(r.x, cch_rec_depth(r), ab + cch_rec_offset(r), 0);
   }
 }
 
@@ -1694,6 +1708,11 @@
 
 hipError_t CchGpu::prune_phase(hipStream_t s, CustScratch& X, CchMetricDev& m) {
   const int N = T_.N;
+  if (T_.max_depth > CCH_REC_MAX_DEPTH) {
+    std::fprintf(stderr, "CchGpu: elimination tree depth %d exceeds %d, the kept-arc records' 16-bit fields\n",
+                 T_.max_depth, CCH_REC_MAX_DEPTH);
+    return hipErrorInvalidValue;
+  }
   hipError_t e = hipSuccess;
   auto ck = [&](hipError_t x) {
     if (x != hipSuccess && e == hipSuccess) e = x;
@@ -1714,17 +1733,24 @@
   if (e != hipSuccess) return e;
   if (tot[0] > m.kept_f || m.f_rec == nullptr) {
     dfree(m.f_rec);
-    ck(dmalloc(m.f_rec, tot[0]));
+    ck(dmalloc(m.f_rec, (size_t)tot[0] + CCH_REC_PAD));
   }
   if (tot[1] > m.kept_b || m.b_rec == nullptr) {
     dfree(m.b_rec);
-    ck(dmalloc(m.b_rec, tot[1]));
+    ck(dmalloc(m.b_rec, (size_t)tot[1] + CCH_REC_PAD));
   }
   m.kept_f = tot[0];
   m.kept_b = tot[1];
   if (e != hipSuccess) return e;
   hipLaunchKernelGGL(prune_scatter_wave_kernel, dim3((unsigned)((N + 3) / 4)), dim3(256), 0, s, d_up_ptr, d_up_head,
                      d_depth, X.pup, X.pdn, X.up64, X.dn64, N, m.f_ptr, m.b_ptr, m.f_rec, m.b_rec);
+  return hipGetLastError();
+}
+
+hipError_t CchGpu::expand_records(const CchMetricDev& m, bool forward, int32_t* d_out, hipStream_t s) {
+  if (d_out == nullptr) return hipErrorInvalidValue;
+  hipLaunchKernelGGL(expand_records_kernel, dim3((unsigned)((T_.N + 3) / 4)), dim3(256), 0, s, d_up_ptr, T_.N,
+                     forward ? m.f_ptr : m.b_ptr, forward ? m.f_rec : m.b_rec, reinterpret_cast<int4*>(d_out));
   return hipGetLastError();
 }
 
diff --git a/csrc/cch_gpu.h b/csrc/cch_gpu.h
--- a/csrc/cch_gpu.h
+++ b/csrc/cch_gpu.h
@@ -32,6 +32,12 @@
   }
 };
 
+typedef int2 CchRec;
+constexpr int CCH_REC_MAX_DEPTH = 65535;
+constexpr int CCH_REC_PAD = 2;
+__host__ __device__ inline int cch_rec_depth(const CchRec& r) { return r.y & 0xFFFF; }
+__host__ __device__ inline int cch_rec_offset(const CchRec& r) { return (int)((unsigned)r.y >> 16); }
+
 struct CchMetricDev {
   uint64_t key = 0;
   int device = 0;
@@ -44,8 +50,8 @@
   int32_t* cnt_dn = nullptr;
   int32_t* f_ptr = nullptr;
   int32_t* b_ptr = nullptr;
-  int4* f_rec = nullptr;
-  int4* b_rec = nullptr;
+  CchRec* f_rec = nullptr;
+  CchRec* b_rec = nullptr;
   int64_t kept_f = 0, kept_b = 0;
   double customize_ms = 0.0, cost_ms = 0.0;
   double basic_ms = 0.0, perfect_ms = 0.0, prune_ms = 0.0;
@@ -101,8 +107,8 @@
 struct CchMView {
   const int32_t* f_ptr;
   const int32_t* b_ptr;
-  const int4* f_rec;
-  const int4* b_rec;
+  const CchRec* f_rec;
+  const CchRec* b_rec;
   const float* len_up;
   const float* len_dn;
   const int32_t* sub_up;
@@ -148,6 +154,8 @@
   bool avoid_clash(const CchContext& c);
 
   hipError_t customize(const float* d_cost, CchMetricDev& m, hipStream_t s, CustScratch* cs = nullptr);
+
+  hipError_t expand_records(const CchMetricDev& m, bool forward, int32_t* d_out, hipStream_t s);
 
   hipError_t metric_for(const CchContext& c, hipStream_t s, std::shared_ptr<CchMetricDev>& out, bool* fresh = nullptr,
                         CustScratch* cs = nullptr);
diff --git a/csrc/cch_query.hip b/csrc/cch_query.hip
--- a/csrc/cch_query.hip
+++ b/csrc/cch_query.hip
@@ -8,23 +8,27 @@
 namespace {
 
 constexpr int SWEEP_AHEAD = 3;
-constexpr int SWEEP_RECS = 4;
-
-typedef int sweep_v4i __attribute__((ext_vector_type(4)));
+constexpr int SWEEP_NBUF = SWEEP_AHEAD + 1;
+constexpr int SWEEP_RECS = 2;
+constexpr int SWEEP_PER = 2;
+constexpr int SWEEP_BLOCK = 64 * SWEEP_PER;
+
+typedef int sweep_vi __attribute__((ext_vector_type(2 * SWEEP_PER)));
 
 struct SweepRecs {
-  sweep_v4i r[SWEEP_RECS];
+  sweep_vi r[SWEEP_RECS];
 };
 
-__device__ __forceinline__ SweepRecs sweep_fetch(const int4* __restrict__ rec, int pb, int pe, int i, int L, int lane) {
+__device__ __forceinline__ SweepRecs sweep_fetch(const CchRec* __restrict__ rec, int pb, int pe, int i, int L,
+                                                 int lane) {
   SweepRecs v;
   const int ii = i < 63 ? i : 63;
   const int b = __shfl(pb, ii);
   const int e = i < L ? __shfl(pe, ii) : b;
 #pragma unroll
   for (int k = 0; k < SWEEP_RECS; ++k) {
-    const int idx = b + lane + 64 * k;
-    const int4* p = rec + (idx < e ? idx : 0);
+    const int idx = b + SWEEP_PER * lane + SWEEP_BLOCK * k;
+    const CchRec* p = rec + (idx < e ? idx : 0);
     asm volatile("global_load_dwordx4 %0, %1, off" : "=v"(v.r[k]) : "v"(p));
   }
   return v;
@@ -33,22 +37,25 @@
 template <int NEWER>
 __device__ __forceinline__ void sweep_wait(SweepRecs& q) {
   static_assert(NEWER * SWEEP_RECS <= 63, "vmcnt range");
-  asm volatile("s_waitcnt vmcnt(%4)" : "+v"(q.r[0]), "+v"(q.r[1]), "+v"(q.r[2]), "+v"(q.r[3]) : "n"(NEWER * SWEEP_RECS));
-}
-
-__device__ __forceinline__ void sweep_relax(float* sd, int32_t* sp, float dx, int w, int hd, int arc) {
+  static_assert(SWEEP_RECS == 2, "the operand list below");
+  asm volatile("s_waitcnt vmcnt(%2)" : "+v"(q.r[0]), "+v"(q.r[1]) : "n"(NEWER * SWEEP_RECS));
+}
+
+__device__ __forceinline__ void sweep_relax(float* sd, int32_t* sp, float dx, int w, int wo, int ab) {
   const float nd = dx + __int_as_float(w);
+  const int hd = wo & 0xFFFF;
   if (nd < sd[hd]) {
     sd[hd] = nd;
-    sp[hd] = arc;
+    sp[hd] = ab + (int)((unsigned)wo >> 16);
   }
 }
 
 __global__ __launch_bounds__(64) void sweep_kernel(const int32_t* __restrict__ jobs, int J,
                                                    const int32_t* __restrict__ parent,
                                                    const int32_t* __restrict__ depth, int N,
-                                                   const int32_t* __restrict__ f_ptr, const int4* __restrict__ f_rec,
-                                                   const int32_t* __restrict__ b_ptr, const int4* __restrict__ b_rec,
+                                                   const int32_t* __restrict__ up_ptr,
+                                                   const int32_t* __restrict__ f_ptr, const CchRec* __restrict__ f_rec,
+                                                   const int32_t* __restrict__ b_ptr, const CchRec* __restrict__ b_rec,
                                                    int stride, float* __restrict__ out_dist,
                                                    int32_t* __restrict__ out_pred, int32_t* __restrict__ out_node,
                                                    const CchMView* __restrict__ mv, const int32_t* __restrict__ grp,
@@ -71,7 +78,7 @@
     b_rec = v.b_rec;
   }
   const int32_t* __restrict__ ptr = fwd ? f_ptr : b_ptr;
-  const int4* __restrict__ rec = fwd ? f_rec : b_rec;
+  const CchRec* __restrict__ rec = fwd ? f_rec : b_rec;
   const int D = depth[r];
   for (int d = lane; d <= D; d += 64) {
     sd[d] = F_INF;
@@ -86,6 +93,7 @@
   int par = cand < N ? parent[cand] : -2;
   int pb = cand < N ? ptr[cand] : 0;
   int pe = cand < N ? ptr[cand + 1] : 0;
+  int pa = cand < N ? up_ptr[cand] : 0;
   while (x >= 0 && d >= 0) {
     const unsigned long long cont = __ballot(cand < N && par == cand + 1);
     int L = (~cont == 0ull) ? 64 : (__builtin_ctzll(~cont) + 1);
@@ -97,47 +105,47 @@
     const int npar = nin ? parent[ncand] : -2;
     const int npb = nin ? ptr[ncand] : 0;
     const int npe = nin ? ptr[ncand + 1] : 0;
+    const int npa = nin ? up_ptr[ncand] : 0;
     auto node = [&](int i, const SweepRecs& q) {
       if (i >= L) return;
       const float dx = sd[d - i];
       if (dx < F_INF) {
-        const int b = __shfl(pb, i), e = __shfl(pe, i);
+        const int b = __shfl(pb, i), e = __shfl(pe, i), ab = __shfl(pa, i);
 #pragma unroll
-        for (int k = 0; k < SWEEP_RECS; ++k)
-          if (b + lane + 64 * k < e) sweep_relax(sd, sp, dx, q.r[k].x, q.r[k].y, q.r[k].z);
-        for (int k = b + 64 * SWEEP_RECS + lane; k < e; k += 64) {
-          const int4 rc = rec[k];
-          sweep_relax(sd, sp, dx, rc.x, rc.y, rc.z);
+        for (int k = 0; k < SWEEP_RECS; ++k) {
+          if (k > 0 && __builtin_amdgcn_readfirstlane(e - b) <= SWEEP_BLOCK * k) break;
+          const int idx = b + SWEEP_PER * lane + SWEEP_BLOCK * k;
+#pragma unroll
+          for (int t = 0; t < SWEEP_PER; ++t)
+            if (idx + t < e) sweep_relax(sd, sp, dx, q.r[k][2 * t], q.r[k][2 * t + 1], ab);
+        }
+        for (int k = b + SWEEP_BLOCK * SWEEP_RECS + lane; k < e; k += 64) {
+          const CchRec rc = rec[k];
+          sweep_relax(sd, sp, dx, rc.x, rc.y, ab);
         }
         __syncthreads();
       }
     };
-    SweepRecs qa = sweep_fetch(rec, pb, pe, 0, L, lane);
-    SweepRecs qb = sweep_fetch(rec, pb, pe, 1, L, lane);
-    SweepRecs qc = sweep_fetch(rec, pb, pe, 2, L, lane);
-    for (int i = 0; i < L; i += 4) {
-      SweepRecs qd = sweep_fetch(rec, pb, pe, i + 3, L, lane);
-      sweep_wait<3>(qa);
-      node(i, qa);
-      qa = sweep_fetch(rec, pb, pe, i + 4, L, lane);
-      sweep_wait<3>(qb);
-      node(i + 1, qb);
-      qb = sweep_fetch(rec, pb, pe, i + 5, L, lane);
-      sweep_wait<3>(qc);
-      node(i + 2, qc);
-      qc = sweep_fetch(rec, pb, pe, i + 6, L, lane);
-      sweep_wait<3>(qd);
-      node(i + 3, qd);
-    }
-    sweep_wait<0>(qa);
-    sweep_wait<0>(qb);
-    sweep_wait<0>(qc);
+    SweepRecs q[SWEEP_NBUF];
+#pragma unroll
+    for (int u = 0; u < SWEEP_AHEAD; ++u) q[u] = sweep_fetch(rec, pb, pe, u, L, lane);
+    for (int i = 0; i < L; i += SWEEP_NBUF) {
+#pragma unroll
+      for (int u = 0; u < SWEEP_NBUF; ++u) {
+        q[(u + SWEEP_AHEAD) % SWEEP_NBUF] = sweep_fetch(rec, pb, pe, i + u + SWEEP_AHEAD, L, lane);
+        sweep_wait<SWEEP_AHEAD>(q[u]);
+        node(i + u, q[u]);
+      }
+    }
+#pragma unroll
+    for (int u = 0; u < SWEEP_NBUF; ++u) sweep_wait<0>(q[u]);
     x = next;
     d -= L;
     cand = ncand;
     par = npar;
     pb = npb;
     pe = npe;
+    pa = npa;
   }
   __syncthreads();
   for (int dd = lane; dd <= D; dd += 64) {
@@ -725,8 +733,8 @@
   hipLaunchKernelGGL(route_jobs_kernel, dim3(blocks_for(Q, 256)), dim3(256), 0, s, d_src, d_dst, Q, d_rank, T_.N,
                      sc.jobs);
   hipLaunchKernelGGL(sweep_kernel, dim3(2 * Q), dim3(64), (size_t)S * 8, s, sc.jobs, 2 * Q, d_parent, d_depth, T_.N,
-                     m ? m->f_ptr : nullptr, m ? m->f_rec : nullptr, m ? m->b_ptr : nullptr, m ? m->b_rec : nullptr, S,
-                     sc.dist, sc.pred, sc.node, mv, grp, 2);
+                     d_up_ptr, m ? m->f_ptr : nullptr, m ? m->f_rec : nullptr, m ? m->b_ptr : nullptr,
+                     m ? m->b_rec : nullptr, S, sc.dist, sc.pred, sc.node, mv, grp, 2);
   if ((e = hipGetLastError()) != hipSuccess) return e;
   hipLaunchKernelGGL(meet_kernel, dim3(Q), dim3(64), 0, s, Q, nullptr, nullptr, 0, 1, sc.jobs, S, sc.dist, sc.pred,
                      sc.node, d_depth, d_arc_lo, m ? m->len_up : nullptr, m ? m->len_dn : nullptr, o.sec, o.metres,
@@ -765,7 +773,7 @@
                      d_rank, T_.N, sc.jobs);
   hipLaunchKernelGGL(matrix_pairs_kernel, dim3(blocks_for((long long)P, 256)), dim3(256), 0, s, d_npts, R, NM, pjf, pjb);
   hipLaunchKernelGGL(sweep_kernel, dim3((unsigned)J), dim3(64), (size_t)S * 8, s, sc.jobs, (int)J, d_parent, d_depth,
-                     T_.N, m ? m->f_ptr : nullptr, m ? m->f_rec : nullptr, m ? m->b_ptr : nullptr,
+                     T_.N, d_up_ptr, m ? m->f_ptr : nullptr, m ? m->f_rec : nullptr, m ? m->b_ptr : nullptr,
                      m ? m->b_rec : nullptr, S, sc.dist, sc.pred, sc.node, mv, grp, 2 * NM);
   if ((e = hipGetLastError()) != hipSuccess) return e;
   hipLaunchKernelGGL(meet_kernel, dim3((unsigned)P), dim3(64), 0, s, (int)P, pjf, pjb, 0, 0, sc.jobs, S, sc.dist,
@@ -811,7 +819,8 @@
   hipLaunchKernelGGL(rect_jobs_kernel, dim3(blocks_for((long long)J, 256)), dim3(256), 0, s, d_src, d_nsrc, d_dst,
                      d_ndst, R, SM, DM, d_rank, T_.N, sc.jobs);
   hipLaunchKernelGGL(sweep_kernel, dim3((unsigned)J), dim3(64), (size_t)S * 8, s, sc.jobs, (int)J, d_parent, d_depth,
-                     T_.N, m.f_ptr, m.f_rec, m.b_ptr, m.b_rec, S, sc.dist, sc.pred, sc.node, nullptr, nullptr, 1);
+                     T_.N, d_up_ptr, m.f_ptr, m.f_rec, m.b_ptr, m.b_rec, S, sc.dist, sc.pred, sc.node, nullptr, nullptr,
+                     1);
   if ((e = hipGetLastError()) != hipSuccess) return e;
   if (meet == MEET_RECT) {
     const size_t blocks = (size_t)R * SM * ((DM + MEET_TILE - 1) / MEET_TILE);
```
